# nwihardjo/SpaghettiSearch

Measured on AMD Instinct MI355X. Metric: pagerank_iters_per_sec, higher is better.
Workload: dtype f64

## Files before the change

include/spaghetti_rank.h:

```cpp
#ifndef SPAGHETTI_RANK_H
#define SPAGHETTI_RANK_H

#include <stdint.h>

#ifdef __cplusplus
extern "C" {
#endif

#define SS_ABI_VERSION 4

enum {
    SS_OK = 0,
    SS_ERR_INVALID = 1,
    SS_ERR_NO_DEVICE = 2,
    SS_ERR_HIP = 3,
    SS_ERR_OOM = 4,
    SS_ERR_UNSORTED = 5,
    SS_ERR_STATE = 6,
    SS_ERR_UNSUPPORTED = 7,
    SS_ERR_COMM = 8
};

#define SS_MAX_TOPK 1024
#define SS_MAX_TOPICS 64
#define SS_MAX_QUERY_TERMS 64
#define SS_MAX_CONSTRAINT_TERMS 16
#define SS_UNKNOWN_TERM 0xFFFFFFFFu

typedef struct ss_ctx ss_ctx;
typedef struct ss_graph ss_graph;
typedef struct ss_pr ss_pr;
typedef struct ss_index ss_index;
typedef struct ss_scorer ss_scorer;

typedef struct ss_hit {
    uint32_t doc;
    uint32_t _pad;
    double title;
    double body;
    double pagerank;
    double final;
} ss_hit;

typedef struct ss_graph_info {
    uint64_t n_nodes, n_edges;
    uint64_t n_nondangling;
    uint64_t n_rows_local;
    uint64_t n_edges_local;
    uint32_t max_indeg;
    int32_t rank, world;
} ss_graph_info;

int32_t ss_abi_version(void);
int32_t ss_init(int32_t device_id, ss_ctx** out);
int32_t ss_shutdown(ss_ctx* ctx);
int32_t ss_set_stream(ss_ctx* ctx, void* hip_stream);
int32_t ss_synchronize(ss_ctx* ctx);
#define SS_OPTION_DEFAULT INT64_MIN
int32_t ss_set_option(ss_ctx* ctx, const char* name, int64_t value);
const char* ss_last_error(ss_ctx* ctx);

#define SS_COMM_ID_BYTES 128
int32_t ss_comm_unique_id(void* id_out );
int32_t ss_comm_init(ss_ctx* ctx, const void* id , int32_t rank, int32_t world);
int32_t ss_comm_split(ss_ctx* ctx, int32_t color, int32_t key);
int32_t ss_comm_destroy(ss_ctx* ctx);
int32_t ss_comm_info(ss_ctx* ctx, int32_t* rank_out , int32_t* world_out);
int32_t ss_comm_allreduce_u64(ss_ctx* ctx, uint64_t* buf, uint64_t n);
int32_t ss_comm_allgather(ss_ctx* ctx, const void* send, void* recv, uint64_t bytes_per_rank);

int32_t ss_graph_create(ss_ctx* ctx, uint64_t n_nodes, uint64_t n_edges,
                        const uint64_t* out_ptr , const uint32_t* out_dst ,
                        int32_t rank, int32_t world, ss_graph** out);
int32_t ss_graph_apply_delta(ss_graph* g, uint64_t n_nodes_new, uint64_t n_changed, const uint32_t* changed ,
                             const uint64_t* new_ptr , const uint32_t* new_children);
int32_t ss_graph_get_info(const ss_graph* g, ss_graph_info* info);
int32_t ss_graph_destroy(ss_graph* g);

#define SS_MAX_LINKS      64
#define SS_LINKS_PARENTS  0
#define SS_LINKS_CHILDREN 1
int32_t ss_graph_set_link_key(ss_graph* g, const double* key );
int32_t ss_graph_top_links(ss_graph* g, int32_t dir, uint64_t n, const uint32_t* nodes , int32_t m,
                           uint32_t* links_out , int32_t* n_out , uint32_t* degree_out );
int32_t ss_graph_hit_links(ss_graph* g, int32_t dir, int32_t n_q, int32_t k,
                           const ss_hit* hits , const int32_t* n_hits , int32_t m,
                           uint32_t* links_out , int32_t* n_out ,
                           uint32_t* degree_out );

int32_t ss_pagerank_run(ss_graph* g, double damping, double eps, int32_t max_iter,
                        int32_t k_topics, const int32_t* n_topic,
                        double* rank_out, int32_t* iters_out);

int32_t ss_pr_create(ss_graph* g, double damping, double eps, int32_t max_iter,
                     int32_t k_topics, const int32_t* n_topic, ss_pr** out);
int32_t ss_pr_destroy(ss_pr* pr);
int32_t ss_pr_set_teleport(ss_pr* pr, const uint64_t* set_ptr , const uint32_t* set_nodes);
int32_t ss_pr_begin(ss_pr* pr);
int32_t ss_pr_step(ss_pr* pr, int32_t n_steps);
int32_t ss_pr_finalize(ss_pr* pr);
int32_t ss_pr_exchange_buffers(ss_pr* pr, void** send_dev, uint64_t* send_bytes,
                               void** recv_dev, uint64_t* recv_bytes);
int32_t ss_pr_exchange(ss_pr* pr, int32_t allreduce);
int32_t ss_pagerank_run_sharded(ss_graph* g, double damping, double eps, int32_t max_iter, int32_t k_topics,
                                const int32_t* n_topic, int32_t allreduce, uint32_t* ids_out, double* rank_out, int32_t* iters_out);
int32_t ss_pagerank_run_group(ss_graph* const* shards, int32_t world, double damping, double eps, int32_t max_iter, int32_t k_topics,
                              const int32_t* n_topic, double* rank_out, int32_t* iters_out);
int32_t ss_pr_status(ss_pr* pr, int32_t* iters_out, int32_t* n_active, int32_t* sweeps,
                     double* last_delta_out , double* last_total_out );
int32_t ss_pr_read_local(ss_pr* pr, uint32_t* ids_out, double* rank_out);
int32_t ss_pr_read(ss_pr* pr, double* rank_out);

int32_t ss_pr_probe(ss_pr* pr, int32_t mode, int32_t n_reps, float* ms_out);

int32_t ss_index_create(ss_ctx* ctx, uint64_t n_docs, uint64_t n_terms,
                        const uint64_t* term_ptr , const uint32_t* post_doc,
                        const float* post_tf, ss_index** out);
int32_t ss_index_destroy(ss_index* idx);
int32_t ss_tfidf_build(ss_index* idx, uint64_t total_docs,
                       float* w_out, double* mag_out, float* idf_out);
int32_t ss_index_set_doc_freq(ss_index* idx, const uint64_t* df );
int32_t ss_index_set_weighted(ss_index* idx, const double* mag );
int32_t ss_index_set_positions(ss_index* idx, const uint64_t* pos_ptr, const float* pos);

int32_t ss_index_apply_delta(ss_index* idx, uint64_t n_del_docs, const uint32_t* del_docs,
                             uint64_t n_del, const uint32_t* del_term, const uint32_t* del_doc,
                             uint64_t n_add, const uint32_t* add_term, const uint32_t* add_doc, const float* add_w);
int32_t ss_index_apply_delta_pos(ss_index* idx, uint64_t n_del_docs, const uint32_t* del_docs,
                                 uint64_t n_del, const uint32_t* del_term, const uint32_t* del_doc,
                                 uint64_t n_add, const uint32_t* add_term, const uint32_t* add_doc, const float* add_w,
                                 const uint64_t* add_pos_ptr , const float* add_pos);
int32_t ss_index_resize(ss_index* idx, uint64_t n_docs_new, uint64_t n_terms_new);
int32_t ss_index_read_magnitudes(ss_index* idx, uint64_t n, const uint32_t* docs, double* mag_out);
int32_t ss_index_refresh_magnitudes(ss_index* idx, double* mag_out);
int32_t ss_index_get_info(const ss_index* idx, uint64_t* n_docs, uint64_t* n_terms, uint64_t* n_post);
int32_t ss_index_read(ss_index* idx, uint64_t* term_ptr_out , uint32_t* post_doc_out, float* post_w_out);
int32_t ss_index_read_positions(ss_index* idx, uint64_t* pos_ptr_out, float* pos_out);

int32_t ss_index_build_doc_view(ss_index* idx);
int32_t ss_index_drop_doc_view(ss_index* idx);
int32_t ss_index_read_doc_view(ss_index* idx, uint64_t* doc_ptr_out, uint32_t* doc_term_out, float* doc_w_out);
int32_t ss_index_doc_top_terms(ss_index* idx, uint64_t n, const uint32_t* docs , int32_t m,
                               uint32_t* terms_out , float* w_out , int32_t* n_out );

int32_t ss_scorer_create(ss_ctx* ctx, ss_index* title, ss_index* body, ss_scorer** out);
int32_t ss_scorer_destroy(ss_scorer* s);
int32_t ss_scorer_set_prior(ss_scorer* s, int32_t k_topics, const double* rank);
int32_t ss_score_topk(ss_scorer* s, int32_t n_q, const uint32_t* q_ptr, const uint32_t* q_terms,
                      const int32_t* query_len, const double* topic_probs, int32_t k,
                      ss_hit* hits_out, int32_t* n_hits_out);

#define SS_SCORE_INFLIGHT 3
int32_t ss_score_topk_submit(ss_scorer* s, int32_t n_q, const uint32_t* q_ptr, const uint32_t* q_terms,
                             const uint32_t* p_ptr ,
                             const uint32_t* p_terms, const int32_t* query_len, const double* topic_probs, int32_t k,
                             uint64_t* ticket_out);
int32_t ss_score_topk_collect(ss_scorer* s, uint64_t ticket, ss_hit* hits_out, int32_t* n_hits_out);

#define SS_MAX_PHRASE_TERMS 16
int32_t ss_score_topk_phrase(ss_scorer* s, int32_t n_q, const uint32_t* q_ptr, const uint32_t* q_terms,
                             const uint32_t* p_ptr, const uint32_t* p_terms, const int32_t* query_len,
                             const double* topic_probs, int32_t k, ss_hit* hits_out, int32_t* n_hits_out);

int32_t ss_scorer_set_doc_masks(ss_scorer* s, int32_t n_masks, const uint32_t* words);

int32_t ss_score_topk_masked(ss_scorer* s, int32_t n_q, const uint32_t* q_ptr, const uint32_t* q_terms,
                             const uint32_t* p_ptr, const uint32_t* p_terms, const int32_t* query_len,
                             const double* topic_probs, const int32_t* mask_id, int32_t k,
                             ss_hit* hits_out, int32_t* n_hits_out);

int32_t ss_score_topk_constrained(ss_scorer* s, int32_t n_q, const uint32_t* q_ptr, const uint32_t* q_terms,
                                  const uint32_t* p_ptr, const uint32_t* p_terms, const int32_t* query_len,
                                  const double* topic_probs, const int32_t* mask_id,
                                  const uint32_t* req_ptr , const uint32_t* req_terms,
                                  const uint32_t* exc_ptr , const uint32_t* exc_terms,
                                  int32_t k, ss_hit* hits_out, int32_t* n_hits_out);

int32_t ss_similar_topk(ss_scorer* s, int32_t n_q, const uint32_t* seeds , int32_t m,
                        const double* topic_probs, const int32_t* mask_id , int32_t k,
                        ss_hit* hits_out, int32_t* n_hits_out);

#define SS_MAX_FEEDBACK_DOCS 64
int32_t ss_related_terms(ss_scorer* s, int32_t n_q, const uint32_t* q_ptr, const uint32_t* q_terms,
                         const int32_t* query_len, const double* topic_probs, const int32_t* mask_id ,
                         int32_t k_fb, int32_t m_doc, int32_t m,
                         uint32_t* terms_out , double* score_out , int32_t* n_out );

typedef struct ss_term_match {
    float    title_w;
    float    body_w;
    uint32_t flags;
    float    body_pos;
} ss_term_match;
int32_t ss_explain_hits(ss_scorer* s, int32_t n_q, const uint32_t* q_ptr, const uint32_t* q_terms,
                        int32_t k, const ss_hit* hits , const int32_t* n_hits ,
                        int32_t t_stride, ss_term_match* out );

typedef struct ss_passage {
    float    start;
    float    last;
    uint32_t n_distinct;
    uint32_t n_occ;
    uint64_t token_mask;
} ss_passage;
int32_t ss_best_passages(ss_scorer* s, int32_t n_q, const uint32_t* q_ptr, const uint32_t* q_terms,
                         int32_t k, const ss_hit* hits , const int32_t* n_hits ,
                         int32_t width, ss_passage* out );

#define SS_NO_GROUP 0xFFFFFFFFu
int32_t ss_scorer_set_doc_groups(ss_scorer* s, const uint32_t* group );

int32_t ss_collapse_hits(ss_scorer* s, int32_t n_q, int32_t k_in, const ss_hit* hits ,
                         const int32_t* n_hits , int32_t g, int32_t first, int32_t k,
                         ss_hit* hits_out , int32_t* n_hits_out ,
                         uint32_t* same_out , int32_t* n_kept_out );

int32_t ss_score_topk_collapsed(ss_scorer* s, int32_t n_q, const uint32_t* q_ptr, const uint32_t* q_terms,
                                const int32_t* query_len, const double* topic_probs, const int32_t* mask_id ,
                                int32_t k_window, int32_t g, int32_t first, int32_t k,
                                ss_hit* hits_out , int32_t* n_hits_out ,
                                uint32_t* same_out , int32_t* n_kept_out );

#define SS_MAX_SIG_SLOTS 32
#define SS_SIG_EMPTY 0xFFFFFFFFu
int32_t ss_index_build_signatures(ss_index* idx, int32_t n_slots);
int32_t ss_index_drop_signatures(ss_index* idx);
int32_t ss_index_read_signatures(ss_index* idx, uint64_t n, const uint32_t* docs ,
                                 uint32_t* sig_out , int32_t* n_slots_out );

int32_t ss_dedup_hits(ss_scorer* s, int32_t n_q, int32_t k_in, const ss_hit* hits , const int32_t* n_hits ,
                      int32_t min_match, int32_t first, int32_t k,
                      ss_hit* hits_out , int32_t* n_hits_out ,
                      uint32_t* similar_out , int32_t* n_kept_out );

#define SS_MAX_DOC_FIELDS 4
#define SS_MAX_RANGE_CLAUSES 4
#define SS_NO_FIELD_VALUE INT64_MIN
typedef struct ss_doc_range {
    int32_t field;
    int32_t _pad;
    int64_t lo, hi;
} ss_doc_range;
int32_t ss_scorer_set_doc_fields(ss_scorer* s, int32_t n_fields, const int64_t* values );

int32_t ss_doc_field_masks(ss_scorer* s, int32_t n_sets, const uint32_t* rng_ptr , const ss_doc_range* rng,
                           const int32_t* mask_id ,
                           uint32_t* words_out );

int32_t ss_score_topk_filtered(ss_scorer* s, int32_t n_q, const uint32_t* q_ptr, const uint32_t* q_terms,
                               const uint32_t* p_ptr, const uint32_t* p_terms, const int32_t* query_len,
                               const double* topic_probs, const int32_t* mask_id,
                               const uint32_t* req_ptr , const uint32_t* req_terms,
                               const uint32_t* exc_ptr , const uint32_t* exc_terms,
                               const uint32_t* rng_ptr , const ss_doc_range* rng,
                               int32_t k, ss_hit* hits_out, int32_t* n_hits_out);

int32_t ss_sort_hits_by_field(ss_scorer* s, int32_t n_q, int32_t k_in, const ss_hit* hits ,
                              const int32_t* n_hits , int32_t field, int32_t descending, int32_t first, int32_t k,
                              ss_hit* hits_out , int32_t* n_hits_out , int64_t* values_out );
int32_t ss_hit_fields(ss_scorer* s, int32_t n_q, int32_t k_in, const ss_hit* hits , const int32_t* n_hits ,
                      int64_t* values_out );

#define SS_MAX_VEC_DIM   1024
#define SS_NO_VEC_SCORE  INT32_MIN
typedef struct ss_vec_hit { uint32_t doc; int32_t score; } ss_vec_hit;
int32_t ss_scorer_set_doc_vectors(ss_scorer* s, int32_t dim, const int8_t* vec );

int32_t ss_vector_topk(ss_scorer* s, int32_t n_q, const int8_t* qvec , const int32_t* mask_id ,
                       int32_t k, ss_vec_hit* hits_out , int32_t* n_hits_out );

int32_t ss_hit_vector_scores(ss_scorer* s, int32_t n_q, const int8_t* qvec , int32_t k_in, const ss_hit* hits ,
                             const int32_t* n_hits , int32_t* scores_out );
int32_t ss_rerank_hits_by_vector(ss_scorer* s, int32_t n_q, const int8_t* qvec , int32_t k_in,
                                 const ss_hit* hits , const int32_t* n_hits , int32_t first, int32_t k,
                                 ss_hit* hits_out , int32_t* n_hits_out , int32_t* scores_out );

#define SS_MAX_VEC_LISTS 65536
#define SS_NO_LIST       0xFFFFFFFFu
int32_t ss_scorer_set_vector_lists(ss_scorer* s, int32_t n_lists, const int8_t* centroids ,
                                   const uint32_t* list_of_doc );
int32_t ss_vector_assign_lists(ss_scorer* s, int32_t n_lists, const int8_t* centroids , uint32_t* list_out ,
                               int32_t* score_out );
int32_t ss_vector_topk_probed(ss_scorer* s, int32_t n_q, const int8_t* qvec , const int32_t* mask_id ,
                              int32_t k, int32_t n_probe, ss_vec_hit* hits_out , int32_t* n_hits_out ,
                              uint32_t* probes_out );

int32_t ss_score_docs(ss_scorer* s, int32_t n_q, const uint32_t* q_ptr, const uint32_t* q_terms, const int32_t* query_len,
                      const double* topic_probs, int32_t k_in, const uint32_t* docs , const int32_t* n_in ,
                      ss_hit* hits_out );

#define SS_FUSE_RRF      0
#define SS_FUSE_WEIGHTED 1
typedef struct ss_fuse_params { int32_t mode; int32_t rrf_c; double w_lex; double w_vec; } ss_fuse_params;
typedef struct ss_fused { double score; int32_t vec_score; uint16_t lex_rank; uint16_t vec_rank; } ss_fused;
int32_t ss_fuse_hits(ss_scorer* s, int32_t n_q, const uint32_t* q_ptr, const uint32_t* q_terms, const int32_t* query_len,
                     const double* topic_probs, const int8_t* qvec ,
                     int32_t k_lex, const ss_hit* lex , const int32_t* n_lex ,
                     int32_t k_vec, const ss_vec_hit* vec , const int32_t* n_vec ,
                     const ss_fuse_params* fp, int32_t first, int32_t k,
                     ss_hit* hits_out , int32_t* n_hits_out ,
                     ss_fused* fused_out , int32_t* n_union_out );
int32_t ss_hybrid_topk(ss_scorer* s, int32_t n_q, const uint32_t* q_ptr, const uint32_t* q_terms, const int32_t* query_len,
                       const double* topic_probs, const int8_t* qvec , const int32_t* mask_id ,
                       int32_t k_window, const ss_fuse_params* fp, int32_t first, int32_t k,
                       ss_hit* hits_out , int32_t* n_hits_out ,
                       ss_fused* fused_out , int32_t* n_union_out );

#define SS_MAX_WORD_BYTES 64
#define SS_MAX_EDIT_DIST  3
#define SS_MAX_SUGGEST    64
typedef struct ss_lexicon ss_lexicon;

int32_t ss_lexicon_create(ss_ctx* ctx, uint64_t n_terms, const uint64_t* word_ptr , const uint8_t* bytes,
                          const uint32_t* freq , ss_lexicon** out);
int32_t ss_lexicon_set_freq(ss_lexicon* lx, const uint32_t* freq );
int32_t ss_lexicon_get_info(const ss_lexicon* lx, uint64_t* n_terms, uint64_t* n_bytes);
int32_t ss_lexicon_read_order(ss_lexicon* lx, uint32_t* order_out );
int32_t ss_lexicon_destroy(ss_lexicon* lx);

int32_t ss_lexicon_prefix(ss_lexicon* lx, int32_t n_q, const uint32_t* p_ptr , const uint8_t* p_bytes,
                          int64_t first, int32_t k, uint32_t* terms_out , int32_t* n_out ,
                          uint64_t* n_match_out );

int32_t ss_lexicon_suggest(ss_lexicon* lx, int32_t n_q, const uint32_t* w_ptr , const uint8_t* w_bytes,
                           int32_t max_dist, uint32_t min_freq, int32_t m,
                           uint32_t* terms_out , int32_t* dist_out , int32_t* n_out );

#define SS_MAX_SHARDS 64
int32_t ss_merge_hits(ss_ctx* ctx, int32_t n_q, int32_t n_parts, int32_t k, const ss_hit* parts,
                      const int32_t* n_hits, const uint32_t* doc_base, ss_hit* hits_out, int32_t* n_hits_out);

int32_t ss_last_kernel_ms(ss_ctx* ctx, int32_t kind, float* ms_out);

#ifdef __cplusplus
}
#endif
#endif
```

spaghettisearch_amd/_lib.py:

```python
from __future__ import annotations

import ctypes as C
import os

_HERE = os.path.dirname(os.path.abspath(__file__))
LIB_PATH = os.environ.get("SS_LIB_PATH") or os.path.join(_HERE, "libspaghetti_rank.so")

SS_OK = 0
SS_MAX_TOPK = 1024
SS_MAX_TOPICS = 64
SS_MAX_QUERY_TERMS = 64
SS_MAX_FEEDBACK_DOCS = 64
SS_UNKNOWN_TERM = 0xFFFFFFFF
SS_NO_GROUP = 0xFFFFFFFF
SS_MAX_WORD_BYTES = 64
SS_MAX_EDIT_DIST = 3
SS_MAX_SUGGEST = 64
SS_MAX_SIG_SLOTS = 32
SS_SIG_EMPTY = 0xFFFFFFFF
SS_MAX_LINKS = 64
SS_LINKS_PARENTS = 0
SS_LINKS_CHILDREN = 1
SS_MAX_DOC_FIELDS = 4
SS_MAX_RANGE_CLAUSES = 4
SS_NO_FIELD_VALUE = -(2 ** 63)
SS_MAX_VEC_DIM = 1024
SS_NO_VEC_SCORE = -(2 ** 31)
SS_MAX_VEC_LISTS = 65536
SS_NO_LIST = 0xFFFFFFFF
SS_FUSE_RRF = 0
SS_FUSE_WEIGHTED = 1

ERR_NAMES = {0: "SS_OK", 1: "SS_ERR_INVALID", 2: "SS_ERR_NO_DEVICE", 3: "SS_ERR_HIP", 4: "SS_ERR_OOM",
             5: "SS_ERR_UNSORTED", 6: "SS_ERR_STATE", 7: "SS_ERR_UNSUPPORTED", 8: "SS_ERR_COMM"}
SS_COMM_ID_BYTES = 128


class SpaghettiError(RuntimeError):
    def __init__(self, code: int, msg: str):
        super().__init__(f"{ERR_NAMES.get(code, code)}: {msg}")
        self.code = code


class SsHit(C.Structure):
    _fields_ = [("doc", C.c_uint32), ("_pad", C.c_uint32), ("title", C.c_double), ("body", C.c_double),
                ("pagerank", C.c_double), ("final", C.c_double)]


class SsTermMatch(C.Structure):
    _fields_ = [("title_w", C.c_float), ("body_w", C.c_float), ("flags", C.c_uint32), ("body_pos", C.c_float)]


class SsPassage(C.Structure):
    _fields_ = [("start", C.c_float), ("last", C.c_float), ("n_distinct", C.c_uint32), ("n_occ", C.c_uint32), ("token_mask", C.c_uint64)]


class SsDocRange(C.Structure):
    _fields_ = [("field", C.c_int32), ("_pad", C.c_int32), ("lo", C.c_int64), ("hi", C.c_int64)]


class SsVecHit(C.Structure):
    _fields_ = [("doc", C.c_uint32), ("score", C.c_int32)]


class SsFuseParams(C.Structure):
    _fields_ = [("mode", C.c_int32), ("rrf_c", C.c_int32), ("w_lex", C.c_double), ("w_vec", C.c_double)]


class SsFused(C.Structure):
    _fields_ = [("score", C.c_double), ("vec_score", C.c_int32), ("lex_rank", C.c_uint16), ("vec_rank", C.c_uint16)]


class SsGraphInfo(C.Structure):
    _fields_ = [("n_nodes", C.c_uint64), ("n_edges", C.c_uint64), ("n_nondangling", C.c_uint64),
                ("n_rows_local", C.c_uint64), ("n_edges_local", C.c_uint64), ("max_indeg", C.c_uint32),
                ("rank", C.c_int32), ("world", C.c_int32)]


_vp = C.c_void_p
_i32 = C.c_int32
_u64 = C.c_uint64
_f64 = C.c_double

PROTOTYPES = {
    "ss_abi_version": (_i32, []),
    "ss_init": (_i32, [_i32, C.POINTER(_vp)]),
    "ss_shutdown": (_i32, [_vp]),
    "ss_set_stream": (_i32, [_vp, _vp]),
    "ss_synchronize": (_i32, [_vp]),
    "ss_set_option": (_i32, [_vp, C.c_char_p, C.c_int64]),
    "ss_last_error": (C.c_char_p, [_vp]),
    "ss_comm_unique_id": (_i32, [_vp]),
    "ss_comm_init": (_i32, [_vp, _vp, _i32, _i32]),
    "ss_comm_split": (_i32, [_vp, _i32, _i32]),
    "ss_comm_destroy": (_i32, [_vp]),
    "ss_comm_info": (_i32, [_vp, C.POINTER(_i32), C.POINTER(_i32)]),
    "ss_comm_allreduce_u64": (_i32, [_vp, _vp, _u64]),
    "ss_comm_allgather": (_i32, [_vp, _vp, _vp, _u64]),
    "ss_graph_create": (_i32, [_vp, _u64, _u64, _vp, _vp, _i32, _i32, C.POINTER(_vp)]),
    "ss_graph_apply_delta": (_i32, [_vp, _u64, _u64, _vp, _vp, _vp]),
    "ss_graph_get_info": (_i32, [_vp, C.POINTER(SsGraphInfo)]),
    "ss_graph_destroy": (_i32, [_vp]),
    "ss_graph_set_link_key": (_i32, [_vp, _vp]),
    "ss_graph_top_links": (_i32, [_vp, _i32, _u64, _vp, _i32, _vp, _vp, _vp]),
    "ss_graph_hit_links": (_i32, [_vp, _i32, _i32, _i32, _vp, _vp, _i32, _vp, _vp, _vp]),
    "ss_pagerank_run": (_i32, [_vp, _f64, _f64, _i32, _i32, _vp, _vp, _vp]),
    "ss_pr_create": (_i32, [_vp, _f64, _f64, _i32, _i32, _vp, C.POINTER(_vp)]),
    "ss_pr_destroy": (_i32, [_vp]),
    "ss_pr_set_teleport": (_i32, [_vp, _vp, _vp]),
    "ss_pr_begin": (_i32, [_vp]),
    "ss_pr_step": (_i32, [_vp, _i32]),
    "ss_pr_finalize": (_i32, [_vp]),
    "ss_pr_exchange_buffers": (_i32, [_vp, C.POINTER(_vp), C.POINTER(_u64), C.POINTER(_vp), C.POINTER(_u64)]),
    "ss_pr_exchange": (_i32, [_vp, _i32]),
    "ss_pagerank_run_sharded": (_i32, [_vp, _f64, _f64, _i32, _i32, _vp, _i32, _vp, _vp, _vp]),
    "ss_pagerank_run_group": (_i32, [_vp, _i32, _f64, _f64, _i32, _i32, _vp, _vp, _vp]),
    "ss_pr_status": (_i32, [_vp, _vp, C.POINTER(_i32), C.POINTER(_i32), _vp, _vp]),
    "ss_pr_read_local": (_i32, [_vp, _vp, _vp]),
    "ss_pr_read": (_i32, [_vp, _vp]),
    "ss_pr_probe": (_i32, [_vp, _i32, _i32, C.POINTER(C.c_float)]),
    "ss_index_create": (_i32, [_vp, _u64, _u64, _vp, _vp, _vp, C.POINTER(_vp)]),
    "ss_index_destroy": (_i32, [_vp]),
    "ss_tfidf_build": (_i32, [_vp, _u64, _vp, _vp, _vp]),
    "ss_index_apply_delta": (_i32, [_vp, _u64, _vp, _u64, _vp, _vp, _u64, _vp, _vp, _vp]),
    "ss_index_apply_delta_pos": (_i32, [_vp, _u64, _vp, _u64, _vp, _vp, _u64, _vp, _vp, _vp, _vp, _vp]),
    "ss_index_resize": (_i32, [_vp, _u64, _u64]),
    "ss_index_read_magnitudes": (_i32, [_vp, _u64, _vp, _vp]),
    "ss_index_refresh_magnitudes": (_i32, [_vp, _vp]),
    "ss_index_get_info": (_i32, [_vp, C.POINTER(_u64), C.POINTER(_u64), C.POINTER(_u64)]),
    "ss_index_read": (_i32, [_vp, _vp, _vp, _vp]),
    "ss_index_read_positions": (_i32, [_vp, _vp, _vp]),
    "ss_index_set_doc_freq": (_i32, [_vp, _vp]),
    "ss_index_set_weighted": (_i32, [_vp, _vp]),
    "ss_index_set_positions": (_i32, [_vp, _vp, _vp]),
    "ss_index_build_doc_view": (_i32, [_vp]),
    "ss_index_drop_doc_view": (_i32, [_vp]),
    "ss_index_read_doc_view": (_i32, [_vp, _vp, _vp, _vp]),
    "ss_index_doc_top_terms": (_i32, [_vp, _u64, _vp, _i32, _vp, _vp, _vp]),
    "ss_scorer_create": (_i32, [_vp, _vp, _vp, C.POINTER(_vp)]),
    "ss_scorer_destroy": (_i32, [_vp]),
    "ss_scorer_set_prior": (_i32, [_vp, _i32, _vp]),
    "ss_score_topk": (_i32, [_vp, _i32, _vp, _vp, _vp, _vp, _i32, _vp, _vp]),
    "ss_score_topk_phrase": (_i32, [_vp, _i32, _vp, _vp, _vp, _vp, _vp, _vp, _i32, _vp, _vp]),
    "ss_score_topk_submit": (_i32, [_vp, _i32, _vp, _vp, _vp, _vp, _vp, _vp, _i32, _vp]),
    "ss_score_topk_collect": (_i32, [_vp, C.c_uint64, _vp, _vp]),
    "ss_scorer_set_doc_masks": (_i32, [_vp, _i32, _vp]),
    "ss_score_topk_masked": (_i32, [_vp, _i32, _vp, _vp, _vp, _vp, _vp, _vp, _vp, _i32, _vp, _vp]),
    "ss_score_topk_constrained": (_i32, [_vp, _i32, _vp, _vp, _vp, _vp, _vp, _vp, _vp, _vp, _vp, _vp, _vp, _i32, _vp, _vp]),
    "ss_similar_topk": (_i32, [_vp, _i32, _vp, _i32, _vp, _vp, _i32, _vp, _vp]),
    "ss_related_terms": (_i32, [_vp, _i32, _vp, _vp, _vp, _vp, _vp, _i32, _i32, _i32, _vp, _vp, _vp]),
    "ss_explain_hits": (_i32, [_vp, _i32, _vp, _vp, _i32, _vp, _vp, _i32, _vp]),
    "ss_best_passages": (_i32, [_vp, _i32, _vp, _vp, _i32, _vp, _vp, _i32, _vp]),
    "ss_scorer_set_doc_groups": (_i32, [_vp, _vp]),
    "ss_collapse_hits": (_i32, [_vp, _i32, _i32, _vp, _vp, _i32, _i32, _i32, _vp, _vp, _vp, _vp]),
    "ss_score_topk_collapsed": (_i32, [_vp, _i32, _vp, _vp, _vp, _vp, _vp, _i32, _i32, _i32, _i32, _vp, _vp, _vp, _vp]),
    "ss_index_build_signatures": (_i32, [_vp, _i32]),
    "ss_index_drop_signatures": (_i32, [_vp]),
    "ss_index_read_signatures": (_i32, [_vp, _u64, _vp, _vp, C.POINTER(_i32)]),
    "ss_dedup_hits": (_i32, [_vp, _i32, _i32, _vp, _vp, _i32, _i32, _i32, _vp, _vp, _vp, _vp]),
    "ss_scorer_set_doc_fields": (_i32, [_vp, _i32, _vp]),
    "ss_doc_field_masks": (_i32, [_vp, _i32, _vp, _vp, _vp, _vp]),
    "ss_score_topk_filtered": (_i32, [_vp, _i32, _vp, _vp, _vp, _vp, _vp, _vp, _vp, _vp, _vp, _vp, _vp, _vp, _vp, _i32, _vp, _vp]),
    "ss_sort_hits_by_field": (_i32, [_vp, _i32, _i32, _vp, _vp, _i32, _i32, _i32, _i32, _vp, _vp, _vp]),
    "ss_hit_fields": (_i32, [_vp, _i32, _i32, _vp, _vp, _vp]),
    "ss_scorer_set_doc_vectors": (_i32, [_vp, _i32, _vp]),
    "ss_vector_topk": (_i32, [_vp, _i32, _vp, _vp, _i32, _vp, _vp]),
    "ss_hit_vector_scores": (_i32, [_vp, _i32, _vp, _i32, _vp, _vp, _vp]),
    "ss_rerank_hits_by_vector": (_i32, [_vp, _i32, _vp, _i32, _vp, _vp, _i32, _i32, _vp, _vp, _vp]),
    "ss_scorer_set_vector_lists": (_i32, [_vp, _i32, _vp, _vp]),
    "ss_vector_assign_lists": (_i32, [_vp, _i32, _vp, _vp, _vp]),
    "ss_vector_topk_probed": (_i32, [_vp, _i32, _vp, _vp, _i32, _i32, _vp, _vp, _vp]),
    "ss_score_docs": (_i32, [_vp, _i32, _vp, _vp, _vp, _vp, _i32, _vp, _vp, _vp]),
    "ss_fuse_hits": (_i32, [_vp, _i32, _vp, _vp, _vp, _vp, _vp, _i32, _vp, _vp, _i32, _vp, _vp, _vp, _i32, _i32, _vp, _vp, _vp, _vp]),
    "ss_hybrid_topk": (_i32, [_vp, _i32, _vp, _vp, _vp, _vp, _vp, _vp, _i32, _vp, _i32, _i32, _vp, _vp, _vp, _vp]),
    "ss_lexicon_create": (_i32, [_vp, _u64, _vp, _vp, _vp, C.POINTER(_vp)]),
    "ss_lexicon_set_freq": (_i32, [_vp, _vp]),
    "ss_lexicon_get_info": (_i32, [_vp, C.POINTER(_u64), C.POINTER(_u64)]),
    "ss_lexicon_read_order": (_i32, [_vp, _vp]),
    "ss_lexicon_destroy": (_i32, [_vp]),
    "ss_lexicon_prefix": (_i32, [_vp, _i32, _vp, _vp, C.c_int64, _i32, _vp, _vp, _vp]),
    "ss_lexicon_suggest": (_i32, [_vp, _i32, _vp, _vp, _i32, C.c_uint32, _i32, _vp, _vp, _vp]),
    "ss_merge_hits": (_i32, [_vp, _i32, _i32, _i32, _vp, _vp, _vp, _vp, _vp]),
    "ss_last_kernel_ms": (_i32, [_vp, _i32, C.POINTER(C.c_float)]),
}

ABI_VERSION = 4
_lib = None


def load() -> C.CDLL:
    global _lib
    if _lib is not None:
        return _lib
    if not os.path.exists(LIB_PATH):
        raise ImportError(
            f"{LIB_PATH} not found: build it with `python -c 'import __graft_entry__ as g; g.build()'` "
            "(make -C spaghettisearch_amd/csrc). There is no CPU fallback.")
    try:
        import torch
    except ImportError:
        pass
    lib = C.CDLL(LIB_PATH)
    for name, (res, args) in PROTOTYPES.items():
        fn = getattr(lib, name)
        fn.restype = res
        fn.argtypes = args
    if lib.ss_abi_version() != ABI_VERSION:
        raise ImportError(f"{LIB_PATH}: ABI version {lib.ss_abi_version()}, this binding was written for {ABI_VERSION} "
                          "(include/spaghetti_rank.h: SS_ABI_VERSION) - rebuild the library")
    _lib = lib
    return lib


def check(rc: int, ctx=None) -> None:
    if rc != SS_OK:
        msg = load().ss_last_error(ctx)
        raise SpaghettiError(rc, msg.decode("utf-8", "replace") if msg else "")
```

spaghettisearch_amd/csrc/ctx.hip:

```cpp
#include "common.hpp"
#include <chrono>

#include <unordered_map>

namespace ss {

namespace {
struct Pool {
    std::mutex mu;
    std::multimap<std::pair<int, size_t>, void*> free_blocks;
    std::unordered_map<void*, std::pair<int, size_t>> live;
    size_t held = 0, limit = (size_t)64 << 30;
    double miss_ms = 0.0;
    uint64_t misses = 0;
    int contexts = 0;
};
Pool& pool() { static Pool* p = new Pool(); return *p; }
size_t size_class(size_t b) {
    if (b <= 4096) return 4096;
    size_t p2 = 4096;
    while (p2 < b) p2 <<= 1;
    if (p2 <= ((size_t)1 << 20)) return p2;
    const size_t step = p2 >> 4;
    return (b + step - 1) / step * step;
}
}

hipError_t pool_alloc(void** out, size_t bytes) {
    Pool& P = pool();
    const size_t cls = size_class(bytes);
    int dev = 0;
    (void)hipGetDevice(&dev);
    {
        std::lock_guard<std::mutex> lk(P.mu);
        auto it = P.free_blocks.find({dev, cls});
        if (it != P.free_blocks.end()) {
            *out = it->second;
            P.free_blocks.erase(it);
            P.held -= cls;
            P.live[*out] = {dev, cls};
            return hipSuccess;
        }
    }
    const auto tm0 = std::chrono::steady_clock::now();
    hipError_t e = hipMalloc(out, cls);
    {
        std::lock_guard<std::mutex> lk(P.mu);
        P.miss_ms += std::chrono::duration<double, std::milli>(std::chrono::steady_clock::now() - tm0).count();
        P.misses++;
    }
    if (e != hipSuccess) {
        (void)hipGetLastError();
        pool_trim();
        e = hipMalloc(out, cls);
    }
    if (e == hipSuccess) {
        std::lock_guard<std::mutex> lk(P.mu);
        P.live[*out] = {dev, cls};
    }
    return e;
}

static thread_local bool t_device_idle = false;

void pool_free_batch(void* const* blocks, size_t count) {
    if (!count) return;
    {
        int cur = 0;
        (void)hipGetDevice(&cur);
        if (device_wedged(cur)) return;
    }
    (void)hipDeviceSynchronize();
    t_device_idle = true;
    for (size_t i = 0; i < count; i++) pool_free(blocks[i]);
    t_device_idle = false;
}

void pool_free(void* p) {
    if (!p) return;
    Pool& P = pool();
    size_t cls = 0, limit = 0;
    int dev = 0;
    {
        std::lock_guard<std::mutex> lk(P.mu);
        auto it = P.live.find(p);
        if (it != P.live.end()) { dev = it->second.first; cls = it->second.second; P.live.erase(it); }
        limit = P.limit;
    }
    if (device_wedged(dev)) return;
    if (cls && cls <= limit / 2) {
        int cur = 0;
        (void)hipGetDevice(&cur);
        if (cur != dev || !t_device_idle) {
            if (cur != dev) (void)hipSetDevice(dev);
            (void)hipDeviceSynchronize();
            if (cur != dev) (void)hipSetDevice(cur);
        }
        std::vector<void*> evict;
        {
            std::lock_guard<std::mutex> lk(P.mu);
            while (P.held + cls > P.limit && !P.free_blocks.empty()) {
                auto last = std::prev(P.free_blocks.end());
                if (last->first.second <= cls) break;
                evict.push_back(last->second);
                P.held -= last->first.second;
                P.free_blocks.erase(last);
            }
            if (P.held + cls <= P.limit) {
                P.free_blocks.emplace(std::make_pair(dev, cls), p);
                P.held += cls;
                p = nullptr;
            }
        }
        for (void* q : evict) (void)hipFree(q);
        if (!p) return;
    }
    (void)hipFree(p);
}

void pool_stats(uint64_t* misses, double* miss_ms) {
    std::lock_guard<std::mutex> lk(pool().mu);
    *misses = pool().misses;
    *miss_ms = pool().miss_ms;
}
void pool_context_count(int delta) {
    bool last = false;
    {
        std::lock_guard<std::mutex> lk(pool().mu);
        pool().contexts += delta;
        last = delta < 0 && pool().contexts <= 0;
    }
    if (last) pool_trim();
}

void pool_trim() {
    Pool& P = pool();
    std::multimap<std::pair<int, size_t>, void*> take;
    {
        std::lock_guard<std::mutex> lk(P.mu);
        take.swap(P.free_blocks);
        P.held = 0;
    }
    for (auto& kv : take) (void)hipFree(kv.second);
}

void pool_set_limit(size_t bytes) {
    {
        std::lock_guard<std::mutex> lk(pool().mu);
        pool().limit = bytes;
    }
    pool_trim();
}

static std::mutex g_err_mu;
static std::string g_err;
void set_global_error(const std::string& msg) {
    std::lock_guard<std::mutex> lk(g_err_mu);
    g_err = msg;
}
}

extern "C" {

int32_t ss_abi_version(void) { return SS_ABI_VERSION; }

int32_t ss_init(int32_t device_id, ss_ctx** out) {
    if (!out) {
        ss::set_global_error("ss_init: out is NULL");
        return SS_ERR_INVALID;
    }
    *out = nullptr;
    int n_dev = 0;
    hipError_t e = hipGetDeviceCount(&n_dev);
    if (e != hipSuccess || n_dev <= 0) {
        ss::set_global_error(std::string("ss_init: no HIP device (") + hipGetErrorString(e) + ")");
        return SS_ERR_NO_DEVICE;
    }
    if (device_id < 0 || device_id >= n_dev) {
        ss::set_global_error("ss_init: device_id out of range");
        return SS_ERR_INVALID;
    }
    ss_ctx* ctx = new (std::nothrow) ss_ctx();
    if (!ctx) return SS_ERR_OOM;
    ctx->device = device_id;
    if ((e = hipSetDevice(device_id)) != hipSuccess) {
        ss::set_global_error(std::string("ss_init: hipSetDevice: ") + hipGetErrorString(e));
        delete ctx;
        return SS_ERR_NO_DEVICE;
    }
    hipDeviceProp_t prop;
    if ((e = hipGetDeviceProperties(&prop, device_id)) != hipSuccess) {
        ss::set_global_error(std::string("ss_init: hipGetDeviceProperties: ") + hipGetErrorString(e));
        delete ctx;
        return SS_ERR_NO_DEVICE;
    }
    if (std::strncmp(prop.gcnArchName, "gfx950", 6) != 0) {
        ss::set_global_error(std::string("ss_init: device is ") + prop.gcnArchName +
                             ", this library is built for gfx950 (MI355X) only");
        delete ctx;
        return SS_ERR_NO_DEVICE;
    }
    ctx->cu_count = prop.multiProcessorCount;
    ctx->total_mem = prop.totalGlobalMem;
    if ((e = hipStreamCreateWithFlags(&ctx->own_stream, hipStreamNonBlocking)) != hipSuccess) {
        ss::set_global_error(std::string("ss_init: hipStreamCreate: ") + hipGetErrorString(e));
        delete ctx;
        return SS_ERR_HIP;
    }
    ctx->stream = ctx->own_stream;
    int prio_lo = 0, prio_hi = 0;
    (void)hipDeviceGetStreamPriorityRange(&prio_lo, &prio_hi);
    if ((e = hipStreamCreateWithPriority(&ctx->comm_stream, hipStreamNonBlocking, prio_hi)) != hipSuccess) {
        ss::set_global_error(std::string("ss_init: hipStreamCreate (comm): ") + hipGetErrorString(e));
        (void)hipStreamDestroy(ctx->own_stream);
        delete ctx;
        return SS_ERR_HIP;
    }
    for (int k = 0; k < 3; k++)
        for (int j = 0; j < 2; j++)
            if ((e = hipEventCreate(&ctx->ev[k][j])) != hipSuccess) {
                ss::set_global_error(std::string("ss_init: hipEventCreate: ") + hipGetErrorString(e));
                delete ctx;
                return SS_ERR_HIP;
            }
    if ((e = hipHostMalloc(reinterpret_cast<void**>(&ctx->h_pin), ss_ctx::PIN_SCRATCH, hipHostMallocDefault)) != hipSuccess) {
        ss::set_global_error(std::string("ss_init: hipHostMalloc: ") + hipGetErrorString(e));
        delete ctx;
        return SS_ERR_HIP;
    }
    ss::pool_context_count(+1);
    *out = ctx;
    return SS_OK;
}

int32_t ss_shutdown(ss_ctx* ctx) {
    if (!ctx) return SS_ERR_INVALID;
    (void)hipSetDevice(ctx->device);
    const bool stuck = !ss::try_unwedge(ctx);
    (void)ss_comm_destroy(ctx);
    if (!stuck) (void)hipStreamSynchronize(ctx->stream);
    for (int k = 0; k < 3; k++)
        for (int j = 0; j < 2; j++)
            if (ctx->ev[k][j]) (void)hipEventDestroy(ctx->ev[k][j]);
    if (ctx->comm_stream && !stuck) { (void)hipStreamSynchronize(ctx->comm_stream); (void)hipStreamDestroy(ctx->comm_stream); }
    for (hipStream_t ws : ctx->wave_stream)
        if (ws && !stuck) { (void)hipStreamSynchronize(ws); (void)hipStreamDestroy(ws); }
    if (ctx->own_stream && !stuck) (void)hipStreamDestroy(ctx->own_stream);
    if (ctx->h_pin) (void)hipHostFree(ctx->h_pin);
    for (auto& b : ctx->pin_cache) (void)hipHostFree(b.p);
    delete ctx;
    ss::pool_context_count(-1);
    return SS_OK;
}

int32_t ss_set_stream(ss_ctx* ctx, void* hip_stream) {
    if (!ctx) return SS_ERR_INVALID;
    std::lock_guard<std::recursive_mutex> lk(ctx->mu);
    SS_HIP(ctx, hipStreamSynchronize(ctx->stream));
    ctx->stream = hip_stream ? reinterpret_cast<hipStream_t>(hip_stream) : ctx->own_stream;
    return SS_OK;
}

static const char* const k_option_names[] = {
    "comm.timeout_ms",
    "pr.force_narrow",
    "pr.wire_f32",
    "pr.narrow_wave",
    "pr.t_quad",
    "pr.blocks_per_cu",
    "mem.pool_mb",
    "pr.deal_snake",
    "pr.affine_lag",
    "pr.affine",
    "pr.items_per_wave",
    "pr.persistent",
    "pr.persistent_blocks",
    "pr.n_class_order",
    "pr.class_order",
    "pr.stagger",
    "pr.deal_global",
    "pr.share_zero_rows",
    "pr.item_turns",
    "graph.late_free",
    "graph.readback_runs",
    "pr.trace",
    "score.collect_pinned",
    "score.pipeline_slices",
    "score.timing",
    "score.trace",
    "pr.probe_hot",
    "pr.topic_blocks",
    "tfidf.blocks",
    "tfidf.bucket_shift",
    "tfidf.head_min_run",
    "tfidf.bucket_min",
    "score.wave",
    "score.wave_max_terms",
    "score.wave_min_list",
    "score.wave_share_pct",
    "score.wave_slice_target",
    "score.wave_big_pct",
    "score.wave_big_x100",
    "score.small",
    "score.small_max_batch",
    "score.small_batch",
    "score.small_cap",
    "score.pipeline",
    "score.grade_slices",
    "score.wave_small_x100",
    "score.exact_all",
    "score.slice_target",
    "score.separate_merge",
    "passage.lds_events",
    "lexicon.chunk_terms",
    "links.wave_max",
    "links.chunk_edges",
    "vec.chunk_docs",
    "vec.list_seg_rows",
    "vec.list_batch_q",
    "vec.assign_batch",
};

int32_t ss_set_option(ss_ctx* ctx, const char* name, int64_t value) {
    if (!ctx || !name) return SS_ERR_INVALID;
    std::lock_guard<std::recursive_mutex> lk(ctx->mu);
    for (const char* n : k_option_names)
        if (std::strcmp(n, name) == 0) {
            if (value == SS_OPTION_DEFAULT) ctx->options.erase(name);
            else ctx->options[name] = value;
            if (std::strcmp(name, "mem.pool_mb") == 0) ss::pool_set_limit(value == SS_OPTION_DEFAULT ? (size_t)64 << 30 : (size_t)std::max<int64_t>(0, value) << 20);
            return SS_OK;
        }
    return ctx->fail(SS_ERR_INVALID, "ss_set_option: unknown option '%s'", name);
}

int32_t ss_synchronize(ss_ctx* ctx) {
    if (!ctx) return SS_ERR_INVALID;
    std::lock_guard<std::recursive_mutex> lk(ctx->mu);
    SS_HIP(ctx, hipSetDevice(ctx->device));
    SS_TRY(ss::sync_bounded(ctx, ctx->stream, "ss_synchronize"));
    return SS_OK;
}

const char* ss_last_error(ss_ctx* ctx) {
    if (ctx) return ctx->last_error.c_str();
    static thread_local std::string tl;
    {
        std::lock_guard<std::mutex> lk(ss::g_err_mu);
        tl = ss::g_err;
    }
    return tl.c_str();
}

int32_t ss_last_kernel_ms(ss_ctx* ctx, int32_t kind, float* ms_out) {
    if (!ctx || !ms_out || kind < 0 || kind > 2) return SS_ERR_INVALID;
    std::lock_guard<std::recursive_mutex> lk(ctx->mu);
    if (!ctx->ev_valid[kind]) return ctx->fail(SS_ERR_STATE, "ss_last_kernel_ms: no timed call of kind %d yet", kind);
    SS_HIP(ctx, hipEventSynchronize(ctx->ev[kind][1]));
    SS_HIP(ctx, hipEventElapsedTime(ms_out, ctx->ev[kind][0], ctx->ev[kind][1]));
    return SS_OK;
}

}
```

spaghettisearch_amd/csrc/pagerank.hip:

```cpp
#include "pr_device.hpp"

#include <algorithm>
#include <chrono>
#include <cmath>
#include <memory>

namespace {

__global__ void k_pr_item_ranges(WorkItem* __restrict__ work, uint32_t n_items, const uint32_t* __restrict__ in_ptr) {
    const uint32_t i = blockIdx.x * blockDim.x + threadIdx.x;
    if (i >= n_items) return;
    WorkItem w = work[i];
    switch (w.kind) {
        case V_ROWW: w.beg = in_ptr[w.row]; w.end = in_ptr[w.row + 1]; break;
        case V_SEG:
            w.beg = in_ptr[w.row] + w.count * SEGW;
            w.end = min(in_ptr[w.row + 1], w.beg + SEGW);
            break;
        case V_QUAD:
        case V_DEG: w.beg = in_ptr[w.row]; w.end = in_ptr[w.row + w.count]; break;
        default: return;
    }
    work[i] = w;
}

__global__ __launch_bounds__(TPB) void k_pr_remap_src(const uint32_t* __restrict__ in_src, uint32_t* __restrict__ out, size_t n_edges, uint32_t pos_nd,
                                                      uint32_t cnt_nd, const uint32_t* __restrict__ outdeg, const uint32_t* __restrict__ sh_deg,
                                                      uint32_t n_shared, uint32_t zrow) {
    for (size_t e = (size_t)blockIdx.x * TPB + threadIdx.x; e < n_edges; e += (size_t)gridDim.x * TPB) {
        uint32_t w = NT_LOAD(&in_src[e]);
        const uint32_t s = w & SRC_MASK;
        if (s >= pos_nd) {
            uint32_t row = zrow;
            if (s < cnt_nd && n_shared) {
                const uint32_t od = outdeg[s];
                uint32_t lo = 0, hi = n_shared;
                while (lo < hi) {
                    const uint32_t mid = (lo + hi) >> 1;
                    if (sh_deg[mid] < od) lo = mid + 1; else hi = mid;
                }
                if (lo < n_shared && sh_deg[lo] == od) row = zrow + 1 + lo;
            }
            w = (w & ~SRC_MASK) | row;
        }
        NT_STORE(w, &out[e]);
    }
}

template <int GW>
__global__ __launch_bounds__(TPB) void k_pr_begin(PrParams p) {
    const int lane = threadIdx.x & 63;
    const int t = lane % GW;
    const double x0 = p.x0[t];
    double* __restrict__ Tw = p.tab_wr[1];
    double csum = 0.0;
    for (uint32_t i = blockIdx.x * TPB + threadIdx.x; i < p.n_shared * (uint32_t)GW; i += gridDim.x * TPB)
        Tw[(size_t)(p.zrow + 1) * GW + i] = p.d * x0 / (double)p.sh_deg[i / GW];
    const size_t n_el = ((size_t)p.sl_nd + p.sl_d) * GW;
    for (size_t i = (size_t)blockIdx.x * TPB + threadIdx.x; i < n_el; i += (size_t)gridDim.x * TPB) {
        const uint32_t lrow = (uint32_t)(i / GW);
        const bool real = lrow < p.sl_nd ? lrow < p.cnt_nd : (lrow - p.sl_nd) < p.cnt_d;
        p.x[i] = real ? x0 : 0.0;
        if (lrow < p.sl_nd) {
            double c = 0.0;
            if (real) c = p.d * x0 / (double)p.outdeg[lrow];
            if ((p.world == 1 || lrow + 2 < p.sl_nd) && lrow < p.tab_rows) Tw[i] = c;
            csum += c;
        }
    }
    block_reduce_and_publish<GW>(p, 0.0, csum, Tw, true);
}

template <int GW>
__global__ void k_pr_finalize(PrParams p, const double* __restrict__ table, int is_begin) {
    if (threadIdx.x != 0 || blockIdx.x != 0) return;
    if (!is_begin && p.ctl->n_active == 0) return;
    double dl[MAXK], cs[MAXK];
    for (int k = 0; k < MAXK; k++) { dl[k] = 0.0; cs[k] = 0.0; }
    for (int r = 0; r < p.world; r++) {
        const size_t base = ((size_t)r * p.sl_nd + (p.sl_nd - 2)) * GW;
        for (int k = 0; k < GW; k++) {
            cs[k] += table[base + k];
            dl[k] += table[base + GW + k];
        }
    }
    finalize_ctl(p, dl, cs, is_begin != 0);
}

template <int GW>
__global__ void k_pr_read(const double* __restrict__ x, const PrCtl* __restrict__ ctl, const uint32_t* __restrict__ old_id,
                          uint32_t sl_nd, uint32_t cnt_nd, uint32_t pos_nd, uint32_t sl_d, uint32_t cnt_d, uint32_t pos_d,
                          uint64_t id0_nd, uint64_t id0_d, int k_topics, uint64_t out_stride,
                          int by_original_id, uint32_t* __restrict__ ids_out, double* __restrict__ out,
                          const uint32_t* __restrict__ memb, uint32_t ts_mask) {
    const size_t n_rows = (size_t)cnt_nd + cnt_d;
    size_t i = (size_t)blockIdx.x * blockDim.x + threadIdx.x;
    if (i >= n_rows) return;
    const uint32_t lrow = i < cnt_nd ? (uint32_t)i : sl_nd + (uint32_t)(i - cnt_nd);
    const uint64_t iid = lrow < sl_nd ? id0_nd + lrow : id0_d + (lrow - sl_nd);
    const uint32_t orig = old_id[iid];
    const size_t o = by_original_id ? (size_t)orig : i;
    if (ids_out) ids_out[i] = orig;
    const bool zero = lrow < sl_nd ? lrow >= pos_nd : (lrow - sl_nd) >= pos_d;
    const uint32_t mb = memb ? memb[lrow] & ts_mask : 0u;
    for (int k = 0; k < k_topics; k++)
        out[(size_t)k * out_stride + o] = zero ? (((mb >> k) & 1u) ? ctl->xz_in[k] : ctl->xz[k]) : x[(size_t)lrow * GW + k];
}

__global__ void k_pr_memb(const uint64_t* __restrict__ set_ptr, const uint32_t* __restrict__ set_nodes, int k_topics, uint64_t n_nodes,
                          const uint32_t* __restrict__ new_id, uint64_t nd_int, uint32_t sl_nd, uint32_t sl_d, int rank,
                          uint32_t* __restrict__ memb, uint32_t* __restrict__ seen, uint32_t* __restrict__ err) {
    const uint64_t total = set_ptr[k_topics];
    for (uint64_t i = (uint64_t)blockIdx.x * blockDim.x + threadIdx.x; i < total; i += (uint64_t)gridDim.x * blockDim.x) {
        int k = 0;
        while (k + 1 < k_topics && set_ptr[k + 1] <= i) k++;
        const uint32_t v = set_nodes[i];
        if ((uint64_t)v >= n_nodes) { atomicOr(err, 1u); continue; }
        if (atomicOr(&seen[v], 1u << k) & (1u << k)) { atomicOr(err, 2u); continue; }
        const uint64_t iid = new_id[v];
        uint32_t lrow;
        int owner;
        if (iid < nd_int) { owner = (int)(iid / sl_nd); lrow = (uint32_t)(iid % sl_nd); }
        else { owner = (int)((iid - nd_int) / sl_d); lrow = sl_nd + (uint32_t)((iid - nd_int) % sl_d); }
        if (owner == rank) atomicOr(&memb[lrow], 1u << k);
    }
}
__global__ void k_pr_memb_zero_count(const uint32_t* __restrict__ memb, uint32_t sl_nd, uint32_t cnt_nd, uint32_t pos_nd, uint32_t cnt_d,
                                     uint32_t pos_d, int k_topics, unsigned long long* __restrict__ cnt) {
    const uint32_t z_nd = cnt_nd - pos_nd, n_zero = z_nd + (cnt_d - pos_d);
    for (uint32_t i = blockIdx.x * blockDim.x + threadIdx.x; i < n_zero; i += gridDim.x * blockDim.x) {
        const uint32_t lrow = i < z_nd ? pos_nd + i : sl_nd + pos_d + (i - z_nd);
        const uint32_t mb = memb[lrow];
        for (int k = 0; k < k_topics; k++)
            if ((mb >> k) & 1u) atomicAdd(&cnt[k], 1ull);
    }
}

template <int GW, int POL>
__global__ __launch_bounds__(TPB) void k_pr_probe(const double* __restrict__ T, const uint32_t* __restrict__ in_src, size_t n_edges,
                                                  uint32_t n_rows, int mode, double* __restrict__ sink, uint32_t hot) {
    if constexpr (GW >= 8) {
        constexpr int NSLOT = 64 / GW;
        const int lane = threadIdx.x & 63, wave = threadIdx.x >> 6;
        const int t = lane % GW, slot = lane / GW, gbase = lane - t;
        const size_t groups = (size_t)gridDim.x * WAVES * NSLOT;
        const size_t gi = ((size_t)blockIdx.x * WAVES + wave) * NSLOT + slot;
        const size_t n_chunks = n_edges / CH;
        const size_t per = (n_chunks + groups - 1) / groups;
        size_t c = min(gi * per, n_chunks);
        const size_t c_hi = min(c + per, n_chunks);
        double acc = 0.0;
        for (; c < c_hi; c++) {
            constexpr int R = CH / GW;
            uint32_t src[R];
#pragma unroll
            for (int r = 0; r < R; r++) {
                const size_t e = c * CH + (size_t)(r * GW + t);
                uint32_t v = NT_LOAD(&in_src[e]) & SRC_MASK;
                if (mode == 1) v = (uint32_t)(((uint64_t)(v * 2654435761u + (uint32_t)e * 40503u) * n_rows) >> 32);
                if (mode == 2) v = (uint32_t)(e % n_rows);
                src[r] = v;
            }
            double v[CH];
#pragma unroll
            for (int j = 0; j < CH; j++) {
                const uint32_t sj = (uint32_t)__shfl((int)src[j / GW], gbase + (j % GW), 64);
                const double* a = &T[(size_t)sj * GW + t];
                if constexpr (POL == 0) v[j] = *a;
                else if constexpr (POL == 1) v[j] = __builtin_nontemporal_load(a);
                else if constexpr (POL == 2) v[j] = __hip_atomic_load(a, __ATOMIC_RELAXED, __HIP_MEMORY_SCOPE_AGENT);
                else if constexpr (POL == 3) v[j] = sj < hot ? *a : __builtin_nontemporal_load(a);
                else v[j] = sj < hot ? *a : __hip_atomic_load(a, __ATOMIC_RELAXED, __HIP_MEMORY_SCOPE_AGENT);
            }
#pragma unroll
            for (int j = 0; j < CH; j++) acc += v[j];
        }
        sink[((size_t)blockIdx.x * TPB + threadIdx.x)] = acc;
    }
}

}

namespace {

void pick_kernel(const ss_ctx* ctx, ss_pr* pr, int k, uint64_t table_rows) {
    const bool force_narrow = ctx->opt("pr.force_narrow", 0) != 0, narrow_wave = ctx->opt("pr.narrow_wave", 1) != 0;
    if (k > 2) {
        pr->kernel = PR_SWEEP;
        pr->gw = k <= 8 ? 8 : 16;
    } else if (force_narrow) {
        pr->kernel = PR_STEP;
        pr->gw = k;
    } else if (narrow_wave) {
        pr->kernel = PR_SWEEP_N;
        pr->gw = k;
    } else if (table_rows * 64 <= (64ull << 20)) {
        pr->kernel = PR_SWEEP;
        pr->gw = 8;
    } else {
        pr->kernel = PR_STEP;
        pr->gw = k;
    }
    pr->nwave = pr->kernel == PR_SWEEP_N;
    const int64_t want = ctx->opt("pr.persistent", 0);
    pr->persist_mode = want == 2 ? 2 : 1;
    pr->persist = pr->nwave && pr->g->world == 1 && !ctx->opt("pr.affine", 0) && want > 0;
}

template <int GW>
void launch_begin(ss_pr* pr, hipStream_t st, unsigned nb) {
    hipLaunchKernelGGL(k_pr_begin<GW>, dim3(nb), dim3(TPB), 0, st, pr->prm);
}
template <int GW>
void launch_finalize(ss_pr* pr, hipStream_t st, int is_begin) {
    hipLaunchKernelGGL(k_pr_finalize<GW>, dim3(1), dim3(64), 0, st, pr->prm, (const double*)pr->tab0.p, is_begin);
}
template <int GW>
__global__ __launch_bounds__(TPB) void k_pr_read_orig(const double* __restrict__ x, const PrCtl* __restrict__ ctl, const uint32_t* __restrict__ new_id,
                                                      uint64_t n, uint32_t sl_nd, uint32_t pos_nd, uint32_t pos_d, int k_topics,
                                                      double* __restrict__ out, const uint32_t* __restrict__ memb, uint32_t ts_mask) {
    const uint64_t v = (uint64_t)blockIdx.x * blockDim.x + threadIdx.x;
    if (v >= n) return;
    const uint32_t lrow = new_id[v];
    const bool zero = lrow < sl_nd ? lrow >= pos_nd : (lrow - sl_nd) >= pos_d;
    double r[GW];
    if (!zero) {
        if constexpr (GW >= 2) {
            const double2* const row = reinterpret_cast<const double2*>(x + (size_t)lrow * GW);
#pragma unroll
            for (int j = 0; j < GW / 2; j++) { const double2 t = row[j]; r[2 * j] = t.x; r[2 * j + 1] = t.y; }
        } else {
            r[0] = x[lrow];
        }
    } else {
        const uint32_t mb = memb ? memb[lrow] & ts_mask : 0u;
#pragma unroll
        for (int k = 0; k < GW; k++) r[k] = ((mb >> k) & 1u) ? ctl->xz_in[k] : ctl->xz[k];
    }
#pragma unroll
    for (int k = 0; k < GW; k++)
        if (k < k_topics) out[(size_t)k * n + v] = r[k];
}

template <int GW>
void launch_read(ss_pr* pr, hipStream_t st, int by_orig, uint64_t stride, uint32_t* ids, double* out) {
    const ss_graph* g = pr->g;
    const size_t n_rows = (size_t)g->cnt_nd + g->cnt_d;
    if (!n_rows) return;
    if (by_orig && g->world == 1 && !ids && stride == g->n) {
        hipLaunchKernelGGL(k_pr_read_orig<GW>, dim3(ss::div_up(g->n, TPB)), dim3(TPB), 0, st, (const double*)pr->x.p, (const PrCtl*)pr->ctl.p,
                           (const uint32_t*)g->new_id.p, g->n, g->sl_nd, pr->prm.pos_nd, pr->prm.pos_d, pr->k, out, pr->prm.memb, pr->prm.ts_mask);
        return;
    }
    hipLaunchKernelGGL(k_pr_read<GW>, dim3(ss::div_up(n_rows, TPB)), dim3(TPB), 0, st, (const double*)pr->x.p,
                       (const PrCtl*)pr->ctl.p, (const uint32_t*)g->old_id.p, g->sl_nd, g->cnt_nd, pr->prm.pos_nd, g->sl_d, g->cnt_d,
                       pr->prm.pos_d,
                       (uint64_t)g->rank * g->sl_nd, g->nd_int + (uint64_t)g->rank * g->sl_d, pr->k, stride, by_orig, ids, out,
                       pr->prm.memb, pr->prm.ts_mask);
}

#define SS_GW_DISPATCH(gw, fn, ...)          \
    switch (gw) {                            \
        case 1: fn<1>(__VA_ARGS__); break;   \
        case 2: fn<2>(__VA_ARGS__); break;   \
        case 8: fn<8>(__VA_ARGS__); break;   \
        default: fn<16>(__VA_ARGS__); break; \
    }

}

namespace ss {
unsigned begin_blocks(const ss_pr* pr) { return std::max(1u, std::min(2048u, ss::div_up((size_t)pr->g->n_local() * pr->gw, TPB))); }
void pr_launch_begin(ss_pr* pr, hipStream_t st, unsigned nb) { SS_GW_DISPATCH(pr->gw, launch_begin, pr, st, nb); }
void pr_launch_step(ss_pr* pr, hipStream_t st) {
    switch (pr->kernel) {
        case PR_STEP: pr_step_launch(pr, st); break;
        case PR_SWEEP: pr_sweep_launch(pr, st); break;
        case PR_SWEEP_N: pr_sweep_n_launch(pr, st); break;
    }
}
void pr_launch_finalize(ss_pr* pr, hipStream_t st, int is_begin) { SS_GW_DISPATCH(pr->gw, launch_finalize, pr, st, is_begin); }
}

namespace {

PlanOptions plan_options(const ss_ctx* ctx, const ss_pr* pr, size_t n_local) {
    const bool small = n_local <= ((size_t)4 << 20);
    PlanOptions o;
    o.t_quad = (uint32_t)ctx->opt("pr.t_quad", pr->nwave ? 256 : 128);
    o.item_turns = (uint32_t)std::max<int64_t>(1, std::min<int64_t>(64, ctx->opt("pr.item_turns", pr->nwave ? (small ? 1 : 4) : (small ? 4 : 8))));
    o.items_per_wave = pr->nwave ? (size_t)std::max<int64_t>(1, ctx->opt("pr.items_per_wave", 4)) : 1;
    o.deal_snake = ctx->opt("pr.deal_snake", PlanOptions::AUTO);
    o.deal_global = ctx->opt("pr.deal_global", pr->nwave && pr->gw == 1 ? 1 : 2);
    o.blocks_per_cu = ctx->opt("pr.blocks_per_cu", PlanOptions::AUTO);
    o.class_order = ctx->opt("pr.class_order", 235401);
    o.n_class_order = ctx->opt("pr.n_class_order", small ? 2310 : 123);
    o.stagger = ctx->opt("pr.stagger", 0);
    return o;
}

constexpr int OCC_MULTI_N = 3;
int blocks_per_cu(int row, int gw) {
    static std::mutex occ_mu;
    static int occ_cache[4][MAXK + 1] = {};
    std::lock_guard<std::mutex> lk_occ(occ_mu);
    int& occ = occ_cache[row][gw];
    if (!occ) {
        int per_cu = 0;
        switch (row) {
            case PR_STEP: per_cu = ss::pr_step_occupancy(gw); break;
            case PR_SWEEP: per_cu = ss::pr_sweep_occupancy(gw); break;
            case PR_SWEEP_N: per_cu = ss::pr_sweep_n_occupancy(gw); break;
            default: per_cu = ss::pr_multi_n_occupancy(gw); break;
        }
        occ = std::max(per_cu, 1);
    }
    return occ;
}
unsigned grid_for(const ss_ctx* ctx, const ss_pr* pr, const PlanOptions& opt, int per_cu, size_t n_items) {
    per_cu = (int)std::max<int64_t>(1, opt.blocks_per_cu == PlanOptions::AUTO ? per_cu : opt.blocks_per_cu);
    if (pr->persist) {
        const int admit = std::max(1, blocks_per_cu(OCC_MULTI_N, pr->gw) - 2);
        per_cu = (int)std::max<int64_t>(1, std::min<int64_t>(std::min(admit, std::max(1, per_cu / 2)), ctx->opt("pr.persistent_blocks", 4)));
    }
    return pr->kernel != PR_STEP ? (unsigned)std::min<size_t>(std::max<size_t>(1, ss::div_up(n_items, (size_t)WAVES * opt.items_per_wave)), (size_t)ctx->cu_count * per_cu)
                                 : (unsigned)std::min<size_t>(n_items, (size_t)ctx->cu_count * 8);
}

void fill_params(ss_pr* pr, const Cut& cut, const PlanOptions& opt, double damping, double eps, int32_t max_iter, int32_t k_topics) {
    const ss_graph* g = pr->g;
    PrParams& p = pr->prm;
    p.in_ptr = g->in_ptr.p;
    p.in_src = g->in_src.p;
    p.outdeg = g->outdeg.p;
    p.x = pr->x.p;
    if (g->world == 1) {
        p.tab_rd[0] = pr->tab0.p; p.tab_wr[0] = pr->tab1.p;
        p.tab_rd[1] = pr->tab1.p; p.tab_wr[1] = pr->tab0.p;
    } else {
        p.tab_rd[0] = p.tab_rd[1] = pr->tab0.p;
        p.tab_wr[0] = p.tab_wr[1] = pr->send.p;
    }
    p.work = pr->work.p;
    p.partials = pr->partials.p;
    p.segpart = pr->segpart.p;
    p.rowticket = pr->rowticket.p;
    p.hubsum = pr->hubsum.p;
    p.nmulti = cut.nmulti;
    p.ctl = pr->ctl.p;
    p.x0 = pr->x0.p;
    p.d = damping;
    p.teleport = 1.0 - damping;
    p.eps = eps;
    p.tele_n = p.teleport * (double)g->n;
    p.max_iter = max_iter;
    p.k_topics = k_topics;
    p.world = g->world;
    p.sl_nd = g->sl_nd;
    p.cnt_nd = g->cnt_nd;
    p.sl_d = g->sl_d;
    p.cnt_d = g->cnt_d;
    p.seg_edges = cut.seg_edges;
    p.n_items = (uint32_t)cut.items.size();
    p.pos_nd = cut.pos_nd;
    p.pos_d = cut.pos_d;
    p.zrow = (uint32_t)g->nd_int;
    p.tab_rows = g->sl_nd;
    p.woff = pr->woff.p;
    p.stagger_div = opt.stagger != 0 ? (uint32_t)std::max(g->ctx->cu_count, 1) : 0u;
    p.stagger_code = opt.stagger >= 10 ? (uint32_t)(opt.stagger - 10) : 0u;
    p.class_order = pack_class_order(opt.class_order);
    p.n_order = pack_n_order(opt.n_class_order);
}

uint64_t fnv1a(const void* q, size_t n, uint64_t h = 0xcbf29ce484222325ull) {
    const unsigned char* b = static_cast<const unsigned char*>(q);
    for (size_t i = 0; i < n; i++) { h ^= b[i]; h *= 0x100000001b3ull; }
    return h;
}
void trace_plan(const ss_pr* pr, const std::vector<WorkItem>& work, const std::vector<uint32_t>& woff) {
    const PrParams& p = pr->prm;
    const double sd[] = {p.d, p.teleport, p.eps, p.tele_n};
    const uint32_t su[] = {(uint32_t)p.max_iter, (uint32_t)p.k_topics, (uint32_t)p.world, p.sl_nd, p.cnt_nd, p.sl_d, p.cnt_d, p.seg_edges, p.n_items,
                           p.pos_nd, p.pos_d, p.ts_mask, p.zrow, p.stagger_div, p.stagger_code, p.class_order, p.n_order};
    fprintf(stderr, "[pr trace] plan: work %016llx (%zu items)  woff %016llx  params %016llx  nblocks %u\n",
            (unsigned long long)fnv1a(work.data(), work.size() * sizeof(WorkItem)), work.size(),
            (unsigned long long)fnv1a(woff.data(), woff.size() * sizeof(uint32_t)),
            (unsigned long long)fnv1a(su, sizeof(su), fnv1a(sd, sizeof(sd))), pr->nblocks);
}

int32_t alloc_tables(ss_pr* pr, hipStream_t st, size_t rows) {
    const ss_graph* g = pr->g;
    ss_ctx* ctx = g->ctx;
    const size_t GW = (size_t)pr->gw;
    SS_HIP(ctx, pr->tab0.alloc(rows * GW));
    SS_HIP(ctx, hipMemsetAsync(pr->tab0.p, 0, std::max<size_t>(pr->tab0.bytes(), 8), st));
    if (g->world == 1) {
        SS_HIP(ctx, pr->tab1.alloc(rows * GW));
        SS_HIP(ctx, hipMemsetAsync(pr->tab1.p, 0, std::max<size_t>(pr->tab1.bytes(), 8), st));
    } else {
        SS_HIP(ctx, pr->send.alloc((size_t)g->sl_nd * GW));
        SS_HIP(ctx, hipMemsetAsync(pr->send.p, 0, std::max<size_t>(pr->send.bytes(), 8), st));
    }
    return SS_OK;
}
int32_t unshare_rows(ss_pr* pr, hipStream_t st) {
    if (!pr->prm.share) return SS_OK;
    const ss_graph* g = pr->g;
    SS_HIP(g->ctx, hipStreamSynchronize(st));
    SS_TRY(alloc_tables(pr, st, (size_t)g->nd_int + 1));
    pr->src_shared.release();
    pr->sh_deg.release();
    PrParams& p = pr->prm;
    p.tab_rd[0] = pr->tab0.p; p.tab_wr[0] = pr->tab1.p;
    p.tab_rd[1] = pr->tab1.p; p.tab_wr[1] = pr->tab0.p;
    p.in_src = g->in_src.p;
    p.sh_deg = nullptr;
    p.n_shared = 0;
    p.share = 0;
    p.zrow = (uint32_t)g->nd_int;
    p.tab_rows = g->sl_nd;
    return SS_OK;
}

#ifdef SS_PR_WAVETIME
void dump_wave_loads(const Cut& cut, const std::vector<double>& cost, const std::vector<uint32_t>& owner, uint32_t nw) {
    FILE* f = open_dump("pr_load.csv");
    if (!f) return;
    std::vector<double> wl(nw, 0.0), wcls((size_t)nw * 6, 0.0);
    for (size_t i = 0; i < cut.items.size(); i++) {
        int kc = 0; while (kc < 5 && i >= cut.vbeg[kc + 1]) kc++;
        wl[owner[i]] += cost[i]; wcls[(size_t)owner[i] * 6 + kc] += cost[i];
    }
    fprintf(f, "wave,load,c0,c1,c2,c3,c4,c5\n");
    for (uint32_t w = 0; w < nw; w++) fprintf(f, "%u,%.2f,%.2f,%.2f,%.2f,%.2f,%.2f,%.2f\n", w, wl[w], wcls[(size_t)w * 6], wcls[(size_t)w * 6 + 1], wcls[(size_t)w * 6 + 2], wcls[(size_t)w * 6 + 3], wcls[(size_t)w * 6 + 4], wcls[(size_t)w * 6 + 5]);
    fclose(f);
}
#endif

}

extern "C" {

int32_t ss_pr_create(ss_graph* g, double damping, double eps, int32_t max_iter, int32_t k_topics,
                     const int32_t* n_topic, ss_pr** out) {
    if (!g) return SS_ERR_INVALID;
    ss_ctx* ctx = g->ctx;
    std::lock_guard<std::recursive_mutex> lk(ctx->mu);
    if (!out) return ctx->fail(SS_ERR_INVALID, "ss_pr_create: out is NULL");
    *out = nullptr;
    if (k_topics < 1 || !n_topic) return ctx->fail(SS_ERR_INVALID, "ss_pr_create: k_topics < 1 or n_topic NULL");
    if (k_topics > MAXK) return ctx->fail(SS_ERR_UNSUPPORTED, "ss_pr_create: k_topics %d > %d per state (ss_pagerank_run splits larger K)", k_topics, MAXK);
    SS_HIP(ctx, hipSetDevice(ctx->device));
    hipStream_t st = ctx->stream;

    ss_pr* pr = new (std::nothrow) ss_pr();
    if (!pr) return ctx->fail(SS_ERR_OOM, "ss_pr_create: host OOM");
    std::unique_ptr<ss_pr> guard(pr);
    pr->g = g;
    pr->k = k_topics;
    pick_kernel(ctx, pr, k_topics, g->nd_int);
    const int GW = pr->gw;
    const bool vitems = pr->kernel != PR_STEP;
    const int GI = pr->nwave ? 8 : GW;
    const size_t n_local = g->n_local();
    if (((uint64_t)g->nd_int + 1) * GW * 8 >= (1ull << 32))
        return ctx->fail(SS_ERR_UNSUPPORTED, "ss_pr_create: contribution table of %llu rows x %d topics exceeds 4 GiB (shard the graph over more ranks)",
                         (unsigned long long)g->nd_int, GW);

    const bool trace = ctx->opt("pr.trace", 0) != 0;
    auto t_now = [] { return std::chrono::steady_clock::now(); };
    auto t_ms = [](std::chrono::steady_clock::time_point a, std::chrono::steady_clock::time_point b) { return std::chrono::duration<double, std::milli>(b - a).count(); };
    SS_HIP(ctx, pr->x.alloc(n_local * GW));
    bool share = GW >= 8 && g->world == 1 && ctx->opt("pr.affine", 0) == 0 && ctx->opt("pr.share_zero_rows", 1) != 0;
    if (!share) SS_TRY(alloc_tables(pr, st, (size_t)g->nd_int + 1));

    const auto tc0 = t_now();
    const PlanOptions opt = plan_options(ctx, pr, n_local);
    Cut cut = cut_items(g->h_indeg_nd, g->h_indeg_d, g->sl_nd, GI, pr->nwave, opt);
    const uint32_t n_tail = g->cnt_nd - cut.pos_nd;
    struct PinGuard { ss_ctx* c; void* p = nullptr; size_t cap = 0; ~PinGuard() { c->pin_free(p, cap); } } tail_od{ctx};
    if (share && n_tail == 0) {
        share = false;
        SS_TRY(alloc_tables(pr, st, (size_t)g->nd_int + 1));
    }
    if (share) {
        tail_od.p = ctx->pin_alloc((size_t)n_tail * sizeof(uint32_t), &tail_od.cap);
        if (!tail_od.p) return ctx->fail(SS_ERR_OOM, "ss_pr_create: no pinned host memory for %u out-degrees", n_tail);
        SS_HIP(ctx, hipMemcpyAsync(tail_od.p, g->outdeg.p + cut.pos_nd, (size_t)n_tail * sizeof(uint32_t), hipMemcpyDeviceToHost, st));
    }
    const auto tc1 = t_now();
    const int per_cu = blocks_per_cu(pr->kernel, GW);
    const auto tc1a = t_now();
    pr->nblocks = grid_for(ctx, pr, opt, per_cu, cut.items.size());
    static const std::vector<uint32_t> no_woff;
    const std::vector<uint32_t>* woff = &no_woff;
    if (vitems) {
        const uint32_t nw = pr->nblocks * WAVES;
        const auto td0 = t_now();
        const std::vector<double>& cost = item_costs(cut, g->h_indeg_nd, g->h_indeg_d, g->sl_nd, GI, pr->nwave);
        const auto td0a = t_now();
        std::vector<uint32_t>& owner = deal_items(cut, cost, nw, pr->nwave, opt);
#ifdef SS_PR_WAVETIME
        dump_wave_loads(cut, cost, owner, nw);
#endif
        const auto td1 = t_now();
        if (trace) fprintf(stderr, "[pr trace]   deal: occupancy query %.2f ms, costs %.3f ms, owners %.3f ms\n", t_ms(tc1, tc1a), t_ms(td0, td0a), t_ms(td0a, td1));
        woff = &place_items(cut, owner, nw);
        if (trace) fprintf(stderr, "[pr trace]   deal: placement %.3f ms\n", t_ms(td1, t_now()));
    }
    const std::vector<WorkItem>& items = cut.items;

    g->settle();
    const auto tc2 = t_now();
    SharedRows sh;
    if (share) {
        SS_HIP(ctx, hipStreamSynchronize(st));
        const auto ts0 = t_now();
        sh = plan_shared_rows(static_cast<const uint32_t*>(tail_od.p), n_tail, cut.pos_nd);
        const auto ts1 = t_now();
        SS_TRY(alloc_tables(pr, st, (size_t)sh.table_rows));
        SS_HIP(ctx, pr->sh_deg.alloc(sh.deg.size()));
        SS_HIP(ctx, hipMemcpyAsync(pr->sh_deg.p, sh.deg.data(), sh.deg.size() * sizeof(uint32_t), hipMemcpyHostToDevice, st));
        SS_HIP(ctx, pr->src_shared.alloc(g->e_local));
        if (g->e_local)
            hipLaunchKernelGGL(k_pr_remap_src, dim3((unsigned)std::min<uint64_t>(ss::div_up(g->e_local, TPB), (uint64_t)ctx->cu_count * 16)), dim3(TPB), 0, st,
                               (const uint32_t*)g->in_src.p, pr->src_shared.p, (size_t)g->e_local, cut.pos_nd, g->cnt_nd, (const uint32_t*)g->outdeg.p,
                               (const uint32_t*)pr->sh_deg.p, (uint32_t)sh.deg.size(), sh.zrow);
        if (trace) fprintf(stderr, "[pr trace]   shared rows: %u rows without in-edges -> %zu shared rows (host %.3f ms), table %llu rows\n", n_tail, sh.deg.size(),
                           t_ms(ts0, ts1), (unsigned long long)sh.table_rows);
    }
    SS_HIP(ctx, pr->partials.alloc(((size_t)std::max(pr->nblocks, ss::begin_blocks(pr)) + 8) * 2 * GW));
    SS_HIP(ctx, pr->segpart.alloc((size_t)std::max(cut.nsegs, 1u) * GW));
    SS_HIP(ctx, pr->rowticket.alloc(std::max(cut.nmulti, 1u)));
    SS_HIP(ctx, pr->hubsum.alloc((size_t)std::max(cut.nmulti, 1u) * 2 * GW));
    SS_HIP(ctx, hipMemsetAsync(pr->hubsum.p, 0, pr->hubsum.bytes(), st));
    SS_HIP(ctx, hipMemsetAsync(pr->rowticket.p, 0, pr->rowticket.bytes(), st));
    SS_HIP(ctx, pr->woff.alloc(std::max<size_t>(woff->size(), 8)));
    if (!woff->empty()) SS_HIP(ctx, hipMemcpyAsync(pr->woff.p, woff->data(), woff->size() * sizeof(uint32_t), hipMemcpyHostToDevice, st));
    SS_HIP(ctx, pr->work.alloc(items.size()));
    SS_HIP(ctx, hipMemcpyAsync(pr->work.p, items.data(), items.size() * sizeof(WorkItem), hipMemcpyHostToDevice, st));
    if (vitems)
        hipLaunchKernelGGL(k_pr_item_ranges, dim3(ss::div_up(items.size(), TPB)), dim3(TPB), 0, st, pr->work.p, (uint32_t)items.size(), (const uint32_t*)g->in_ptr.p);
    SS_HIP(ctx, pr->ctl.alloc(1));
    SS_HIP(ctx, hipMemsetAsync(pr->ctl.p, 0, sizeof(PrCtl), st));
    double h_x0[MAXK];
    for (int k = 0; k < MAXK; k++) h_x0[k] = k < k_topics ? 1.0 / (double)n_topic[k] : 0.0;
    SS_HIP(ctx, pr->x0.alloc(MAXK));
    SS_HIP(ctx, hipMemcpyAsync(pr->x0.p, h_x0, sizeof(h_x0), hipMemcpyHostToDevice, st));
    SS_HIP(ctx, hipStreamSynchronize(st));
    if (trace) fprintf(stderr, "[pr trace] ss_pr_create: build_work %.2f ms (%zu items), edge ranges + deal %.2f ms, alloc + upload %.2f ms\n", t_ms(tc0, tc1), items.size(), t_ms(tc1, tc2), t_ms(tc2, t_now()));
    if (trace) fprintf(stderr, "[pr trace] where the state lives: x %p  tab0 %p  tab1 %p  in_src %p  in_ptr %p  outdeg %p  work %p  woff %p\n", (void*)pr->x.p, (void*)pr->tab0.p,
                       (void*)pr->tab1.p, (void*)g->in_src.p, (void*)g->in_ptr.p, (void*)g->outdeg.p, (void*)pr->work.p, (void*)pr->woff.p);

    fill_params(pr, cut, opt, damping, eps, max_iter, k_topics);
    if (share) {
        PrParams& p = pr->prm;
        p.in_src = pr->src_shared.p;
        p.sh_deg = pr->sh_deg.p;
        p.n_shared = (uint32_t)sh.deg.size();
        p.share = 1;
        p.zrow = sh.zrow;
        p.tab_rows = cut.pos_nd;
    }
    if (trace) trace_plan(pr, items, *woff);
    g->users++;
    *out = guard.release();
    return SS_OK;
}

int32_t ss_pr_set_teleport(ss_pr* pr, const uint64_t* set_ptr, const uint32_t* set_nodes) {
    if (!pr) return SS_ERR_INVALID;
    ss_ctx* ctx = pr->g->ctx;
    std::lock_guard<std::recursive_mutex> lk(ctx->mu);
    SS_HIP(ctx, hipSetDevice(ctx->device));
    if (pr->begun) return ctx->fail(SS_ERR_STATE, "ss_pr_set_teleport: call before ss_pr_begin");
    hipStream_t st = ctx->stream;
    PrParams& p = pr->prm;
    if (!set_ptr) {
        p.memb = nullptr; p.tin = nullptr; p.nz_in = nullptr; p.ts_mask = 0;
        return SS_OK;
    }
    const ss_graph* g = pr->g;
    const int K = pr->k;
    SS_TRY(unshare_rows(pr, st));
    std::vector<uint64_t> h_ptr(K + 1);
    SS_HIP(ctx, ss::copy_in(ctx->stream, h_ptr.data(), set_ptr, (K + 1) * sizeof(uint64_t)));
    if (h_ptr[0] != 0) return ctx->fail(SS_ERR_INVALID, "ss_pr_set_teleport: set_ptr[0] != 0");
    for (int k = 0; k < K; k++)
        if (h_ptr[k + 1] < h_ptr[k]) return ctx->fail(SS_ERR_INVALID, "ss_pr_set_teleport: set_ptr not non-decreasing");
    const uint64_t total = h_ptr[K];
    if (total && !set_nodes) return ctx->fail(SS_ERR_INVALID, "ss_pr_set_teleport: set_nodes is NULL");
    double h_tin[MAXK];
    uint32_t mask = 0;
    for (int k = 0; k < MAXK; k++) {
        h_tin[k] = 0.0;
        if (k < K && h_ptr[k + 1] > h_ptr[k]) {
            mask |= 1u << k;
            h_tin[k] = p.teleport * (double)g->n / (double)(h_ptr[k + 1] - h_ptr[k]);
        }
    }
    const size_t n_local = g->n_local();
    ss::DevBuf<uint64_t> d_ptr;
    ss::DevBuf<uint32_t> d_nodes, d_err, d_seen;
    ss::DevBuf<unsigned long long> d_cnt;
    SS_HIP(ctx, d_ptr.alloc(K + 1));
    SS_HIP(ctx, d_seen.alloc(g->n));
    SS_HIP(ctx, hipMemsetAsync(d_seen.p, 0, std::max<size_t>(d_seen.bytes(), 4), st));
    SS_HIP(ctx, d_nodes.alloc(total));
    SS_HIP(ctx, d_err.alloc(1));
    SS_HIP(ctx, d_cnt.alloc(MAXK));
    SS_HIP(ctx, pr->memb.alloc(n_local));
    SS_HIP(ctx, pr->tin.alloc(MAXK));
    SS_HIP(ctx, pr->nz_in.alloc(MAXK));
    SS_HIP(ctx, hipMemcpyAsync(d_ptr.p, h_ptr.data(), (K + 1) * sizeof(uint64_t), hipMemcpyHostToDevice, st));
    if (total) SS_HIP(ctx, hipMemcpyAsync(d_nodes.p, set_nodes, total * sizeof(uint32_t), hipMemcpyDefault, st));
    SS_HIP(ctx, hipMemsetAsync(pr->memb.p, 0, std::max<size_t>(pr->memb.bytes(), 4), st));
    SS_HIP(ctx, hipMemsetAsync(d_err.p, 0, sizeof(uint32_t), st));
    SS_HIP(ctx, hipMemsetAsync(d_cnt.p, 0, MAXK * sizeof(unsigned long long), st));
    if (total)
        hipLaunchKernelGGL(k_pr_memb, dim3(std::min<unsigned>(ss::div_up(total, TPB), 4096u)), dim3(TPB), 0, st, (const uint64_t*)d_ptr.p,
                           (const uint32_t*)d_nodes.p, K, g->n, (const uint32_t*)g->new_id.p, g->nd_int, std::max(g->sl_nd, 1u), std::max(g->sl_d, 1u),
                           g->rank, pr->memb.p, d_seen.p, d_err.p);
    const uint32_t n_zero = (g->cnt_nd - p.pos_nd) + (g->cnt_d - p.pos_d);
    if (n_zero)
        hipLaunchKernelGGL(k_pr_memb_zero_count, dim3(std::min<unsigned>(ss::div_up(n_zero, TPB), 4096u)), dim3(TPB), 0, st,
                           (const uint32_t*)pr->memb.p, g->sl_nd, g->cnt_nd, p.pos_nd, g->cnt_d, p.pos_d, K, d_cnt.p);
    SS_HIP(ctx, hipGetLastError());
    uint32_t h_err = 0;
    unsigned long long h_cnt[MAXK];
    SS_HIP(ctx, ss::fetch(ctx, st, &h_err, d_err.p, sizeof(h_err), h_cnt, d_cnt.p, sizeof(h_cnt)));
    if (h_err & 1u) return ctx->fail(SS_ERR_INVALID, "ss_pr_set_teleport: a teleport set holds a node id >= n_nodes");
    if (h_err & 2u) return ctx->fail(SS_ERR_INVALID, "ss_pr_set_teleport: a teleport set lists a node twice (the ids of a set must be distinct)");
    double h_nz[MAXK];
    for (int k = 0; k < MAXK; k++) h_nz[k] = (double)h_cnt[k];
    SS_HIP(ctx, hipMemcpyAsync(pr->tin.p, h_tin, sizeof(h_tin), hipMemcpyHostToDevice, st));
    SS_HIP(ctx, hipMemcpyAsync(pr->nz_in.p, h_nz, sizeof(h_nz), hipMemcpyHostToDevice, st));
    SS_HIP(ctx, hipStreamSynchronize(st));
    p.memb = pr->memb.p;
    p.tin = pr->tin.p;
    p.nz_in = pr->nz_in.p;
    p.ts_mask = mask;
    return SS_OK;
}

int32_t ss_pr_destroy(ss_pr* pr) {
#ifdef SS_PR_WAVETIME
    if (pr) ss::pr_dump_wave_times(pr);
#endif

    if (!pr) return SS_ERR_INVALID;
    ss_ctx* ctx = pr->g->ctx;
    std::lock_guard<std::recursive_mutex> lk(ctx->mu);
    (void)hipSetDevice(ctx->device);
    if (!ss::device_wedged(ctx->device)) {
        (void)hipStreamSynchronize(ctx->stream);
        (void)hipStreamSynchronize(ctx->comm_stream);
    }
    pr->g->users--;
    delete pr;
    return SS_OK;
}

int32_t ss_pr_begin(ss_pr* pr) {
    if (!pr) return SS_ERR_INVALID;
    ss_ctx* ctx = pr->g->ctx;
    std::lock_guard<std::recursive_mutex> lk(ctx->mu);
    SS_HIP(ctx, hipSetDevice(ctx->device));
    if (pr->need_finalize) return ctx->fail(SS_ERR_STATE, "ss_pr_begin: pending exchange/finalize");
    SS_HIP(ctx, hipMemsetAsync(&pr->ctl.p->ticket, 0, sizeof(uint32_t), ctx->stream));
    ss::pr_launch_begin(pr, ctx->stream, ss::begin_blocks(pr));
    SS_HIP(ctx, hipGetLastError());
    pr->begun = true;
    if (pr->g->world > 1) {
        pr->need_finalize = true;
        pr->finalize_is_begin = true;
    }
    return SS_OK;
}

int32_t ss_pr_step(ss_pr* pr, int32_t n_steps) {
    if (!pr) return SS_ERR_INVALID;
    ss_ctx* ctx = pr->g->ctx;
    std::lock_guard<std::recursive_mutex> lk(ctx->mu);
    SS_HIP(ctx, hipSetDevice(ctx->device));
    if (!pr->begun) return ctx->fail(SS_ERR_STATE, "ss_pr_step: ss_pr_begin not called");
    if (pr->need_finalize) return ctx->fail(SS_ERR_STATE, "ss_pr_step: pending exchange/finalize");
    if (n_steps < 1) return ctx->fail(SS_ERR_INVALID, "ss_pr_step: n_steps < 1");
    if (pr->g->world > 1 && n_steps != 1) return ctx->fail(SS_ERR_INVALID, "ss_pr_step: world>1 needs an exchange after every step");
    SS_HIP(ctx, hipEventRecord(ctx->ev[0][0], ctx->stream));
    if (pr->persist && !pr->prm.memb && !pr->prm.aff) {
        ss::pr_multi_n_launch(pr, ctx->stream, (int)n_steps);
    } else {
        for (int i = 0; i < n_steps; i++) ss::pr_launch_step(pr, ctx->stream);
    }
    SS_HIP(ctx, hipEventRecord(ctx->ev[0][1], ctx->stream));
    ctx->ev_valid[0] = true;
    SS_HIP(ctx, hipGetLastError());
    if (pr->g->world > 1) {
        pr->need_finalize = true;
        pr->finalize_is_begin = false;
    }
    return SS_OK;
}

int32_t ss_pr_finalize(ss_pr* pr) {
    if (!pr) return SS_ERR_INVALID;
    ss_ctx* ctx = pr->g->ctx;
    std::lock_guard<std::recursive_mutex> lk(ctx->mu);
    SS_HIP(ctx, hipSetDevice(ctx->device));
    if (pr->g->world == 1) return ctx->fail(SS_ERR_STATE, "ss_pr_finalize: world==1 folds the finalize into the sweep");
    if (!pr->need_finalize) return ctx->fail(SS_ERR_STATE, "ss_pr_finalize: nothing to finalize");
    ss::pr_launch_finalize(pr, ctx->stream, pr->finalize_is_begin ? 1 : 0);
    SS_HIP(ctx, hipGetLastError());
    pr->need_finalize = false;
    return SS_OK;
}

int32_t ss_pr_exchange_buffers(ss_pr* pr, void** send_dev, uint64_t* send_bytes, void** recv_dev, uint64_t* recv_bytes) {
    if (!pr) return SS_ERR_INVALID;
    ss_ctx* ctx = pr->g->ctx;
    if (pr->g->world == 1) return ctx->fail(SS_ERR_STATE, "ss_pr_exchange_buffers: world==1 has no exchange");
    if (send_dev) *send_dev = pr->send.p;
    if (send_bytes) *send_bytes = pr->send.bytes();
    if (recv_dev) *recv_dev = pr->tab0.p;
    if (recv_bytes) *recv_bytes = (uint64_t)pr->g->nd_int * pr->gw * sizeof(double);
    return SS_OK;
}

int32_t ss_pr_exchange(ss_pr* pr, int32_t allreduce) {
    if (!pr) return SS_ERR_INVALID;
    ss_ctx* ctx = pr->g->ctx;
    std::lock_guard<std::recursive_mutex> lk(ctx->mu);
    SS_HIP(ctx, hipSetDevice(ctx->device));
    const ss_graph* g = pr->g;
    if (g->world == 1) return ctx->fail(SS_ERR_STATE, "ss_pr_exchange: world==1 has no exchange");
    if (!pr->need_finalize) return ctx->fail(SS_ERR_STATE, "ss_pr_exchange: nothing to exchange (call after ss_pr_begin / ss_pr_step)");
    if (!ctx->comm || ctx->comm_world != g->world || ctx->comm_rank != g->rank)
        return ctx->fail(SS_ERR_STATE, "ss_pr_exchange: the context's communicator (rank %d of %d) does not match the graph's shard (rank %d of %d)",
                         ctx->comm ? ctx->comm_rank : -1, ctx->comm ? ctx->comm_world : 0, g->rank, g->world);
    const size_t slice = (size_t)g->sl_nd * pr->gw;
    if (!allreduce && ctx->opt("pr.wire_f32", 0) != 0) {
        SS_HIP(ctx, ss::pr_wire_alloc(pr));
        ss::pr_wire_pack(pr, ctx->stream);
        SS_TRY(ss::comm_allgather(ctx, pr->wire_send.p, pr->wire_recv.p, ss::pr_wire_floats(pr) * sizeof(float)));
        ss::pr_wire_unpack(pr, ctx->stream);
        return SS_OK;
    }
    if (!allreduce) return ss::comm_allgather(ctx, pr->send.p, pr->tab0.p, slice * sizeof(double));
    SS_HIP(ctx, hipMemsetAsync(pr->tab0.p, 0, pr->tab0.bytes(), ctx->stream));
    SS_HIP(ctx, hipMemcpyAsync(pr->tab0.p + (size_t)g->rank * slice, pr->send.p, slice * sizeof(double), hipMemcpyDeviceToDevice, ctx->stream));
    return ss::comm_allreduce_f64(ctx, pr->tab0.p, pr->tab0.p, slice * (size_t)g->world);
}

int32_t ss_pr_status(ss_pr* pr, int32_t* iters_out, int32_t* n_active, int32_t* sweeps, double* last_delta_out,
                     double* last_total_out) {
    if (!pr) return SS_ERR_INVALID;
    ss_ctx* ctx = pr->g->ctx;
    std::lock_guard<std::recursive_mutex> lk(ctx->mu);
    SS_HIP(ctx, hipSetDevice(ctx->device));
    const PrCtl* hp = nullptr;
    SS_TRY(read_ctl(ctx, pr, ctx->stream, "ss_pr_status", &hp));
    const PrCtl h = *hp;
    if (h.stuck) return ctx->fail(SS_ERR_STATE, "ss_pr_status: the multi-sweep kernel gave up waiting between two sweeps (its grid of %u blocks was not resident: "
                                  "other kernels held the CUs for seconds); the state is void — set option pr.persistent = 0 and run again", pr->nblocks);
    for (int k = 0; k < pr->k; k++) {
        if (iters_out) iters_out[k] = h.iters[k];
        if (last_delta_out) last_delta_out[k] = h.delta[k];
        if (last_total_out) last_total_out[k] = h.S[k];
    }
    if (n_active) *n_active = h.n_active;
    if (sweeps) *sweeps = h.sweep;
    return SS_OK;
}

int32_t ss_pr_read_local(ss_pr* pr, uint32_t* ids_out, double* rank_out) {
    if (!pr || !rank_out) return SS_ERR_INVALID;
    ss_ctx* ctx = pr->g->ctx;
    std::lock_guard<std::recursive_mutex> lk(ctx->mu);
    SS_HIP(ctx, hipSetDevice(ctx->device));
    const ss_graph* g = pr->g;
    const size_t n_rows = (size_t)g->cnt_nd + g->cnt_d;
    ss::DevBuf<uint32_t> d_ids;
    ss::DevBuf<double> d_out;
    SS_HIP(ctx, d_ids.alloc(n_rows));
    SS_HIP(ctx, d_out.alloc(n_rows * pr->k));
    SS_GW_DISPATCH(pr->gw, launch_read, pr, ctx->stream, 0, (uint64_t)n_rows, d_ids.p, d_out.p);
    SS_HIP(ctx, hipGetLastError());
    if (ids_out && n_rows) SS_HIP(ctx, hipMemcpyAsync(ids_out, d_ids.p, n_rows * sizeof(uint32_t), hipMemcpyDefault, ctx->stream));
    if (n_rows) SS_HIP(ctx, hipMemcpyAsync(rank_out, d_out.p, n_rows * pr->k * sizeof(double), hipMemcpyDefault, ctx->stream));
    SS_HIP(ctx, hipStreamSynchronize(ctx->stream));
    return SS_OK;
}

int32_t ss_pr_read(ss_pr* pr, double* rank_out) {
    if (!pr || !rank_out) return SS_ERR_INVALID;
    ss_ctx* ctx = pr->g->ctx;
    std::lock_guard<std::recursive_mutex> lk(ctx->mu);
    SS_HIP(ctx, hipSetDevice(ctx->device));
    const ss_graph* g = pr->g;
    if (g->world != 1) return ctx->fail(SS_ERR_STATE, "ss_pr_read: world>1, use ss_pr_read_local");
    hipPointerAttribute_t pa{};
    const bool dev_out = hipPointerGetAttributes(&pa, rank_out) == hipSuccess && pa.type == hipMemoryTypeDevice;
    (void)hipGetLastError();
    ss::DevBuf<double> d_out;
    if (!dev_out) SS_HIP(ctx, d_out.alloc((size_t)g->n * pr->k));
    SS_GW_DISPATCH(pr->gw, launch_read, pr, ctx->stream, 1, (uint64_t)g->n, (uint32_t*)nullptr, dev_out ? rank_out : d_out.p);
    SS_HIP(ctx, hipGetLastError());
    if (!dev_out) SS_HIP(ctx, hipMemcpyAsync(rank_out, d_out.p, (size_t)g->n * pr->k * sizeof(double), hipMemcpyDefault, ctx->stream));
    SS_HIP(ctx, hipStreamSynchronize(ctx->stream));
    return SS_OK;
}

int32_t ss_pr_probe(ss_pr* pr, int32_t mode, int32_t n_reps, float* ms_out) {
    if (!pr || !ms_out) return SS_ERR_INVALID;
    ss_ctx* ctx = pr->g->ctx;
    std::lock_guard<std::recursive_mutex> lk(ctx->mu);
    SS_HIP(ctx, hipSetDevice(ctx->device));
    if (pr->gw < 8) return ctx->fail(SS_ERR_UNSUPPORTED, "ss_pr_probe: the probe mirrors the chunked gather of the K >= 5 kernels");
    if (mode < 0 || (mode & 7) > 2 || (mode >> 3) > 4 || n_reps < 1) return ctx->fail(SS_ERR_INVALID, "ss_pr_probe: mode 0..2 (+ 8 * gather cache policy 0..4), n_reps >= 1");
    const int pol = mode >> 3;
    mode &= 7;
    const uint32_t hot = (uint32_t)ctx->opt("pr.probe_hot", 24576);
    const ss_graph* g = pr->g;
    const unsigned nb = (unsigned)ctx->cu_count * 8;
    ss::DevBuf<double> sink;
    SS_HIP(ctx, sink.alloc((size_t)nb * TPB));
    hipEvent_t e0, e1;
    SS_HIP(ctx, hipEventCreate(&e0));
    SS_HIP(ctx, hipEventCreate(&e1));
    hipStream_t st = ctx->stream;
    ss::DevBuf<double> full;
    if (pr->prm.share) {
        SS_HIP(ctx, full.alloc(((size_t)g->nd_int + 1) * pr->gw));
        SS_HIP(ctx, hipMemsetAsync(full.p, 0, full.bytes(), ctx->stream));
    }
    const double* T = pr->prm.share ? full.p : pr->tab0.p;
    for (int r = 0; r < n_reps + 1; r++) {
        if (r == 1) SS_HIP(ctx, hipEventRecord(e0, st));
#define SS_PROBE_LAUNCH(GWV, POLV) hipLaunchKernelGGL((k_pr_probe<GWV, POLV>), dim3(nb), dim3(TPB), 0, st, T, (const uint32_t*)g->in_src.p, (size_t)g->e_local, (uint32_t)g->nd_int, mode, sink.p, hot)
        if (pr->gw == 8) SS_PROBE_LAUNCH(8, 0);
        else switch (pol) {
            case 0: SS_PROBE_LAUNCH(16, 0); break;
            case 1: SS_PROBE_LAUNCH(16, 1); break;
            case 2: SS_PROBE_LAUNCH(16, 2); break;
            case 3: SS_PROBE_LAUNCH(16, 3); break;
            default: SS_PROBE_LAUNCH(16, 4); break;
        }
    }
    SS_HIP(ctx, hipEventRecord(e1, st));
    SS_HIP(ctx, hipEventSynchronize(e1));
    float ms = 0.f;
    SS_HIP(ctx, hipEventElapsedTime(&ms, e0, e1));
    (void)hipEventDestroy(e0);
    (void)hipEventDestroy(e1);
    SS_HIP(ctx, hipGetLastError());
    *ms_out = ms / (float)n_reps;
    return SS_OK;
}

}
```

spaghettisearch_amd/csrc/pagerank_run.hip:

```cpp
#include "pr_state.hpp"

#include <algorithm>

namespace {

constexpr int AFF_KC = 16;
__global__ __launch_bounds__(TPB) void k_aff_delta(const double2* __restrict__ xp, const double2* __restrict__ xn, const AffCtl* __restrict__ a,
                                                   uint32_t sl_nd, uint32_t pos_nd, uint32_t pos_d, double* __restrict__ partials) {
    __shared__ double red[WAVES][AFF_KC];
    if (a->n_active == 0) return;
    const int k_real = a->k_real;
    const double r_old = a->r_prev, r_new = a->r_x, s_old = a->s_prev, s_new = a->s_x;
    const uint32_t n_rows = pos_nd + pos_d;
    const int lane = threadIdx.x & 63, wave = threadIdx.x >> 6;
    for (int k0 = 0; k0 < k_real; k0 += AFF_KC) {
        double u[AFF_KC], d_old[AFF_KC], d_new[AFF_KC], acc[AFF_KC];
        bool any = false;
#pragma unroll
        for (int j = 0; j < AFF_KC; j++) {
            const bool on = k0 + j < k_real && a->active[k0 + j] != 0;
            any = any || on;
            u[j] = on ? a->u[k0 + j] : 0.0;
            d_old[j] = on ? r_old * u[j] + s_old : 1.0;
            d_new[j] = on ? r_new * u[j] + s_new : 1.0;
// ... 366 lines not shown
                for (int s = 0; s < S; s++) ctl_and_emit(s, A[s].gath.p, (size_t)AFF_MAXK, 0);
            }
            it++;
            if (max_iter > 0 && it >= max_iter) break;
        }
        SS_HIP(ctx, hipGetLastError());
        ctx->pin_used = 0;
        int32_t* const hn = ctx->pin<int32_t>();
        SS_HIP(ctx, hipMemcpyAsync(hn, &A[0].aff.p->n_active, sizeof(int32_t), hipMemcpyDeviceToHost, st));
        SS_TRY(ss::sync_bounded(ctx, st, "sharded two-vector sweep (waiting for the exchange)"));
        n_active = *hn;
        if (max_iter > 0 && it >= max_iter) break;
    }
    if (lag && max_iter > 0 && it >= max_iter && n_active > 0) {
        it--;
        for (int s = 0; s < S; s++) {
            ss_pr* pr = sh[s].blk[0];
            hipLaunchKernelGGL(k_aff_local, dim3(1), dim3(AFF_MAXK), 0, st, (const AffCtl*)A[s].aff.p, (const PrCtl*)pr->ctl.p, (const double*)A[s].partials.p,
                               AFF_NB, A[s].n_zero, A[s].loc.p);
        }
        SS_TRY(exchange_sums(st));
        for (int s = 0; s < S; s++) ctl_and_emit(s, A[s].gath.p, (size_t)AFF_MAXK, 0);
        it++;
        SS_HIP(ctx, hipGetLastError());
    }
    for (int s = 0; s < S; s++) sh[s].blk[0]->need_finalize = false;
    if (iters_out) {
        std::vector<AffCtl> h(1);
        SS_HIP(ctx, hipMemcpyAsync(h.data(), A[0].aff.p, sizeof(AffCtl), hipMemcpyDeviceToHost, st));
        SS_TRY(ss::sync_bounded(ctx, st, "sharded two-vector sweep (status)"));
        for (int k = 0; k < k_topics; k++) iters_out[k] = h[0].iters[k];
    }
    return SS_OK;
}
int32_t local_ids(ss_pr* pr, uint32_t* ids_out) {
    const size_t n_rows = (size_t)pr->g->cnt_nd + pr->g->cnt_d;
    std::vector<double> scratch(std::max<size_t>(1, n_rows * (size_t)pr->k));
    return ss_pr_read_local(pr, ids_out, scratch.data());
}

int32_t check_eps(ss_ctx* ctx, const char* who, double eps, int32_t max_iter) {
    if (!(eps >= 0.0) && max_iter <= 0 && !(eps != eps)) return ctx->fail(SS_ERR_INVALID, "%s: eps < 0 (never converges) needs max_iter > 0", who);
    return SS_OK;
}

int32_t make_topic_blocks(ss_ctx* ctx, const char* who, ss_graph* const* shards, int n_shards, bool affine, bool check_first, double damping, double eps,
                          int32_t max_iter, int32_t k_topics, const int32_t* n_topic, std::vector<ShardBlocks>& sh, std::vector<AffShard>& aff, std::vector<int>& k0) {
    const int B = affine ? 1 : topic_blocks_for(ctx, k_topics);
    sh.resize(n_shards);
    aff.resize(affine ? n_shards : 0);
    k0.resize(B + 1);
    for (int b = 0; b <= B; b++) k0[b] = (int)((int64_t)k_topics * b / B);
    auto check_sizes = [&]() -> int32_t {
        for (int k = 0; k < k_topics; k++)
            if (n_topic[k] < 1) return ctx->fail(SS_ERR_INVALID, "%s: n_topic[%d] < 1", who, k);
        return SS_OK;
    };
    if (affine && check_first) SS_TRY(check_sizes());
    const int32_t two[2] = {1, 1};
    for (int s = 0; s < n_shards; s++) {
        for (int b = 0; b < B; b++) {
            ss_pr* pr = nullptr;
            SS_TRY(affine ? ss_pr_create(shards[s], damping, -1.0, 0, 2, two, &pr)
                          : ss_pr_create(shards[s], damping, eps, max_iter, k0[b + 1] - k0[b], n_topic + k0[b], &pr));
            sh[s].blk.push_back(pr);
        }
        if (affine && !check_first && s == 0) SS_TRY(check_sizes());
        if (affine) SS_TRY(aff_attach(sh[s].blk[0], aff[s], k_topics, n_topic, shards[s]->world));
    }
    return SS_OK;
}

int32_t run_affine(ss_graph* g, double damping, double eps, int32_t max_iter, int32_t k_topics, const int32_t* n_topic,
                   double* rank_out, int32_t* iters_out) {
    ss_ctx* ctx = g->ctx;
    hipStream_t st = ctx->stream;
    if (k_topics > AFF_MAXK) return ctx->fail(SS_ERR_UNSUPPORTED, "ss_pagerank_run (pr.affine): at most %d topics", AFF_MAXK);
    for (int k = 0; k < k_topics; k++)
        if (n_topic[k] < 1) return ctx->fail(SS_ERR_INVALID, "ss_pagerank_run: n_topic[%d] < 1", k);
    const int32_t two[2] = {1, 1};
    ss_pr* pr = nullptr;
    SS_TRY(ss_pr_create(g, damping, -1.0, 0, 2, two, &pr));
    struct Guard { ss_pr* p; ~Guard() { ss_pr_destroy(p); } } guard{pr};
    if (!pr->nwave || pr->gw != 2) return ctx->fail(SS_ERR_UNSUPPORTED, "ss_pagerank_run (pr.affine): needs the wave-item K = 2 sweep (pr.narrow_wave / pr.force_narrow at their defaults)");
    const uint32_t n_local = g->n_local();
    ss::DevBuf<AffCtl> aff;
    ss::DevBuf<double> x_prev, partials, d_out;
    SS_HIP(ctx, aff.alloc(1));
    SS_HIP(ctx, x_prev.alloc((size_t)n_local * 2));
    SS_HIP(ctx, partials.alloc((size_t)AFF_NB * AFF_MAXK));
    SS_TRY(aff_init(pr, k_topics, n_topic, aff.p, x_prev.p));
    hipPointerAttribute_t at{};
    const bool dev_out = hipPointerGetAttributes(&at, rank_out) == hipSuccess && at.type == hipMemoryTypeDevice;
    (void)hipGetLastError();
    double* out = rank_out;
    if (!dev_out) {
        SS_HIP(ctx, d_out.alloc((size_t)k_topics * g->n));
        out = d_out.p;
    }
    SS_TRY(ss_pr_begin(pr));
    const double n_zero = (double)((g->cnt_nd - pr->prm.pos_nd) + (g->cnt_d - pr->prm.pos_d));
    int32_t n_active = k_topics, it = 0;
    const int BATCH = 4;
    while (n_active > 0) {
        for (int b = 0; b < BATCH; b++) {
            const double2* const x_old = reinterpret_cast<const double2*>((it & 1) ? x_prev.p : pr->x.p);
            const double2* const x_new = reinterpret_cast<const double2*>((it & 1) ? pr->x.p : x_prev.p);
            ss::pr_launch_step(pr, st);
            hipLaunchKernelGGL(k_aff_delta, dim3(AFF_NB), dim3(TPB), 0, st, x_old, x_new, (const AffCtl*)aff.p, g->sl_nd, pr->prm.pos_nd, pr->prm.pos_d, partials.p);
            hipLaunchKernelGGL(k_aff_ctl, dim3(1), dim3(AFF_MAXK), 0, st, aff.p, pr->ctl.p, (const double*)partials.p, AFF_NB, n_zero, eps, max_iter, (size_t)AFF_MAXK);
            hipLaunchKernelGGL(k_aff_emit, dim3((unsigned)std::min<uint64_t>(4096, ss::div_up(g->n, TPB))), dim3(TPB), 0, st, x_new, (const PrCtl*)pr->ctl.p,
                               (const AffCtl*)aff.p, (const uint32_t*)g->new_id.p, g->n, g->sl_nd, pr->prm.pos_nd, pr->prm.pos_d, out);
            it++;
            if (max_iter > 0 && it >= max_iter) break;
        }
        SS_HIP(ctx, hipGetLastError());
        SS_HIP(ctx, ss::fetch(ctx, st, &n_active, &aff.p->n_active, sizeof(int32_t)));
        if (max_iter > 0 && it >= max_iter) break;
    }
    std::vector<AffCtl> h(1);
    SS_HIP(ctx, hipMemcpyAsync(h.data(), aff.p, sizeof(AffCtl), hipMemcpyDeviceToHost, st));
    if (!dev_out) SS_HIP(ctx, hipMemcpyAsync(rank_out, d_out.p, (size_t)k_topics * g->n * sizeof(double), hipMemcpyDeviceToHost, st));
    SS_HIP(ctx, hipStreamSynchronize(st));
    if (iters_out)
        for (int k = 0; k < k_topics; k++) iters_out[k] = h[0].iters[k];
    return SS_OK;
}

}

extern "C" {

int32_t ss_pagerank_run_sharded(ss_graph* g, double damping, double eps, int32_t max_iter, int32_t k_topics,
                                const int32_t* n_topic, int32_t allreduce, uint32_t* ids_out, double* rank_out, int32_t* iters_out) {
    if (!g) return SS_ERR_INVALID;
    ss_ctx* ctx = g->ctx;
    std::lock_guard<std::recursive_mutex> lk(ctx->mu);
    if (g->world < 2) return ctx->fail(SS_ERR_STATE, "ss_pagerank_run_sharded: needs a sharded graph (world > 1); use ss_pagerank_run");
    const bool affine = ctx->opt("pr.affine", 0) != 0 && !allreduce;
    const int k_max = affine ? AFF_MAXK : MAXK;
    if (k_topics < 1 || k_topics > k_max || !n_topic || !rank_out)
        return ctx->fail(SS_ERR_INVALID, "ss_pagerank_run_sharded: k_topics must be 1..%d, n_topic/rank_out not NULL", k_max);
    SS_TRY(check_eps(ctx, "ss_pagerank_run_sharded", eps, max_iter));
    if (!ctx->comm || ctx->comm_world != g->world || ctx->comm_rank != g->rank)
        return ctx->fail(SS_ERR_STATE, "ss_pagerank_run_sharded: the context's communicator (rank %d of %d) does not match the graph's shard (rank %d of %d)",
                         ctx->comm ? ctx->comm_rank : -1, ctx->comm ? ctx->comm_world : 0, g->rank, g->world);
    SS_HIP(ctx, hipSetDevice(ctx->device));
    std::vector<ShardBlocks> sh;
    std::vector<AffShard> aff;
    std::vector<int> k0;
    int32_t rc = make_topic_blocks(ctx, "ss_pagerank_run_sharded", &g, 1, affine, false, damping, eps, max_iter, k_topics, n_topic, sh, aff, k0);
    const bool wire_f32 = ctx->opt("pr.wire_f32", 0) != 0;
    if (rc == SS_OK) {
        auto exchange = [&](int b, hipStream_t xs) -> int32_t {
            ss_pr* pr = sh[0].blk[b];
            const size_t slice = (size_t)g->sl_nd * pr->gw;
            if (!allreduce && wire_f32) {
                SS_HIP(ctx, ss::pr_wire_alloc(pr));
                ss::pr_wire_pack(pr, xs);
                SS_TRY(ss::comm_allgather_on(ctx, pr->wire_send.p, pr->wire_recv.p, ss::pr_wire_floats(pr) * sizeof(float), xs));
                ss::pr_wire_unpack(pr, xs);
                return SS_OK;
            }
            if (!allreduce) return ss::comm_allgather_on(ctx, pr->send.p, pr->tab0.p, slice * sizeof(double), xs);
            SS_HIP(ctx, hipMemsetAsync(pr->tab0.p, 0, pr->tab0.bytes(), xs));
            SS_HIP(ctx, hipMemcpyAsync(pr->tab0.p + (size_t)g->rank * slice, pr->send.p, slice * sizeof(double), hipMemcpyDeviceToDevice, xs));
            return ss::comm_allreduce_f64_on(ctx, pr->tab0.p, pr->tab0.p, slice * (size_t)g->world, xs);
        };
        if (affine) {
            auto exchange_sums = [&](hipStream_t xs) -> int32_t {
                return ss::comm_allgather_on(ctx, aff[0].loc.p, aff[0].gath.p, (size_t)AFF_MAXK * sizeof(double), xs);
            };
            rc = run_affine_sharded(ctx, sh, aff, g->world, eps, max_iter, k_topics, exchange, exchange_sums, iters_out);
        } else {
            rc = run_pipelined(ctx, sh, max_iter, exchange, iters_out, k0);
        }
    }
    const size_t n_rows = (size_t)g->cnt_nd + g->cnt_d;
    if (affine) {
        if (rc == SS_OK && ids_out) rc = local_ids(sh[0].blk[0], ids_out);
        if (rc == SS_OK && n_rows) {
            if (hipMemcpyAsync(rank_out, aff[0].out.p, (size_t)k_topics * n_rows * sizeof(double), hipMemcpyDefault, ctx->stream) != hipSuccess ||
                hipStreamSynchronize(ctx->stream) != hipSuccess)
                rc = ctx->fail(SS_ERR_HIP, "ss_pagerank_run_sharded: copy of the ranks failed");
        }
    } else
    for (int b = 0; b < (int)sh[0].blk.size() && rc == SS_OK; b++)
        rc = ss_pr_read_local(sh[0].blk[b], b == 0 ? ids_out : nullptr, rank_out + (size_t)k0[b] * n_rows);
    for (ss_pr* pr : sh[0].blk) ss_pr_destroy(pr);
    return rc;
}

int32_t ss_pagerank_run_group(ss_graph* const* shards, int32_t world, double damping, double eps, int32_t max_iter, int32_t k_topics,
                              const int32_t* n_topic, double* rank_out, int32_t* iters_out) {
    if (!shards || world < 2 || !shards[0]) return SS_ERR_INVALID;
    ss_ctx* ctx = shards[0]->ctx;
    std::lock_guard<std::recursive_mutex> lk(ctx->mu);
    const bool affine = ctx->opt("pr.affine", 0) != 0;
    const int k_max = affine ? AFF_MAXK : MAXK;
    if (k_topics < 1 || k_topics > k_max || !n_topic || !rank_out)
        return ctx->fail(SS_ERR_INVALID, "ss_pagerank_run_group: k_topics must be 1..%d, n_topic/rank_out not NULL", k_max);
    SS_TRY(check_eps(ctx, "ss_pagerank_run_group", eps, max_iter));
    for (int s = 0; s < world; s++)
        if (!shards[s] || shards[s]->ctx != ctx || shards[s]->world != world || shards[s]->rank != s || shards[s]->n != shards[0]->n)
            return ctx->fail(SS_ERR_INVALID, "ss_pagerank_run_group: shards[%d] is not shard %d of %d of the same graph on this context", s, s, world);
    SS_HIP(ctx, hipSetDevice(ctx->device));
    std::vector<ShardBlocks> sh;
    std::vector<AffShard> aff;
    std::vector<int> k0;
    int32_t rc = make_topic_blocks(ctx, "ss_pagerank_run_group", shards, world, affine, true, damping, eps, max_iter, k_topics, n_topic, sh, aff, k0);
    const int B = (int)k0.size() - 1;
    if (rc == SS_OK) {
        const bool wire_f32 = ctx->opt("pr.wire_f32", 0) != 0;
        auto exchange = [&](int b, hipStream_t xs) -> int32_t {
            if (wire_f32) {
                for (int src = 0; src < world; src++) {
                    SS_HIP(ctx, ss::pr_wire_alloc(sh[src].blk[b]));
                    ss::pr_wire_pack(sh[src].blk[b], xs);
                }
                for (int dst = 0; dst < world; dst++) {
                    ss_pr* to = sh[dst].blk[b];
                    for (int src = 0; src < world; src++) {
                        ss_pr* from = sh[src].blk[b];
                        SS_HIP(ctx, hipMemcpyAsync(to->wire_recv.p + (size_t)src * ss::pr_wire_floats(from), from->wire_send.p, ss::pr_wire_floats(from) * sizeof(float),
                                                   hipMemcpyDeviceToDevice, xs));
                    }
                    ss::pr_wire_unpack(to, xs);
                }
                return SS_OK;
            }
            for (int dst = 0; dst < world; dst++)
                for (int src = 0; src < world; src++) {
                    ss_pr* from = sh[src].blk[b];
                    ss_pr* to = sh[dst].blk[b];
                    const size_t slice = (size_t)shards[src]->sl_nd * from->gw;
                    SS_HIP(ctx, hipMemcpyAsync(to->tab0.p + (size_t)src * slice, from->send.p, slice * sizeof(double), hipMemcpyDeviceToDevice, xs));
                }
            return SS_OK;
        };
        if (affine) {
            auto exchange_sums = [&](hipStream_t xs) -> int32_t {
                for (int dst = 0; dst < world; dst++)
                    for (int src = 0; src < world; src++)
                        SS_HIP(ctx, hipMemcpyAsync(aff[dst].gath.p + (size_t)src * AFF_MAXK, aff[src].loc.p, (size_t)AFF_MAXK * sizeof(double),
                                                   hipMemcpyDeviceToDevice, xs));
                return SS_OK;
            };
            rc = run_affine_sharded(ctx, sh, aff, world, eps, max_iter, k_topics, exchange, exchange_sums, iters_out);
        } else {
            rc = run_pipelined(ctx, sh, max_iter, exchange, iters_out, k0);
        }
    }
    const uint64_t n = shards[0]->n;
    for (int s = 0; s < world && rc == SS_OK && affine; s++) {
        const size_t n_rows = (size_t)shards[s]->cnt_nd + shards[s]->cnt_d;
        std::vector<uint32_t> ids(n_rows);
        std::vector<double> part((size_t)k_topics * n_rows);
        rc = local_ids(sh[s].blk[0], ids.data());
        if (rc == SS_OK && n_rows) {
            if (hipMemcpyAsync(part.data(), aff[s].out.p, part.size() * sizeof(double), hipMemcpyDeviceToHost, ctx->stream) != hipSuccess ||
                hipStreamSynchronize(ctx->stream) != hipSuccess)
                rc = ctx->fail(SS_ERR_HIP, "ss_pagerank_run_group: copy of the ranks failed");
        }
        for (int k = 0; k < k_topics && rc == SS_OK; k++)
            for (size_t i = 0; i < n_rows; i++) rank_out[(size_t)k * n + ids[i]] = part[(size_t)k * n_rows + i];
    }
    for (int s = 0; s < world && rc == SS_OK && !affine; s++) {
        const size_t n_rows = (size_t)shards[s]->cnt_nd + shards[s]->cnt_d;
        std::vector<uint32_t> ids(n_rows);
        for (int b = 0; b < B && rc == SS_OK; b++) {
            const int kb = k0[b + 1] - k0[b];
            std::vector<double> part((size_t)kb * n_rows);
            rc = ss_pr_read_local(sh[s].blk[b], ids.data(), part.data());
            if (rc != SS_OK) break;
            for (int k = 0; k < kb; k++)
                for (size_t i = 0; i < n_rows; i++) rank_out[(size_t)(k0[b] + k) * n + ids[i]] = part[(size_t)k * n_rows + i];
        }
    }
    for (auto& s : sh)
        for (ss_pr* pr : s.blk) ss_pr_destroy(pr);
    return rc;
}

int32_t ss_pagerank_run(ss_graph* g, double damping, double eps, int32_t max_iter, int32_t k_topics,
                        const int32_t* n_topic, double* rank_out, int32_t* iters_out) {
    if (!g) return SS_ERR_INVALID;
    ss_ctx* ctx = g->ctx;
    std::lock_guard<std::recursive_mutex> lk(ctx->mu);
    if (g->world != 1) return ctx->fail(SS_ERR_STATE, "ss_pagerank_run: needs a (rank 0, world 1) graph");
    if (k_topics < 1 || k_topics > SS_MAX_TOPICS || !n_topic || !rank_out)
        return ctx->fail(SS_ERR_INVALID, "ss_pagerank_run: bad k_topics / NULL argument");
    SS_TRY(check_eps(ctx, "ss_pagerank_run", eps, max_iter));
    if (ctx->opt("pr.affine", 0) != 0) return run_affine(g, damping, eps, max_iter, k_topics, n_topic, rank_out, iters_out);
    for (int k0 = 0; k0 < k_topics; k0 += MAXK) {
        const int kk = std::min(MAXK, k_topics - k0);
        ss_pr* pr = nullptr;
        SS_TRY(ss_pr_create(g, damping, eps, max_iter, kk, n_topic + k0, &pr));
        int32_t rc = ss_pr_begin(pr);
        int32_t n_active = kk, sweeps = 0;
        const int BATCH = 8;
        while (rc == SS_OK && n_active > 0) {
            int todo = BATCH;
            if (max_iter > 0) todo = std::min(BATCH, std::max(1, max_iter - sweeps));
            rc = ss_pr_step(pr, todo);
            if (rc == SS_OK) rc = ss_pr_status(pr, iters_out ? iters_out + k0 : nullptr, &n_active, &sweeps, nullptr, nullptr);
        }
        if (rc == SS_OK) rc = ss_pr_read(pr, rank_out + (size_t)k0 * g->n);
        ss_pr_destroy(pr);
        if (rc != SS_OK) return rc;
    }
    return SS_OK;
}

}
```

spaghettisearch_amd/csrc/pr_plan.hpp:

```cpp
#pragma once
#include "sorted_degrees.hpp"

#include <algorithm>
#include <cstdint>
#include <utility>
#include <vector>

namespace {

constexpr int TPB = 256;
constexpr int WAVES = TPB / 64;
constexpr int CH = 16;
constexpr uint32_t SEGW = 2048;

enum : uint32_t { W_SEG = 0, W_WAVE = 1, W_GROUP = 2, W_ZERO = 3,
                  V_SEG = 8,
                  V_ROWW = 9,
                  V_QUAD = 10,
                  V_DEG = 11,
                  V_ZERO = 12 };

struct WorkItem {
    uint32_t kind;
    uint32_t row;
    uint32_t count;
    uint32_t nseg;
    uint32_t sbase;
    uint32_t tix;
    uint32_t beg, end;
};

constexpr uint32_t plan_div_up(uint64_t a, uint64_t b) { return (uint32_t)((a + b - 1) / b); }

struct PlanOptions {
    static constexpr int64_t AUTO = INT64_MIN;
    uint32_t t_quad = 128;
    uint32_t item_turns = 4;
    size_t items_per_wave = 1;
    int64_t deal_snake = AUTO;
    int64_t deal_global = 2;
    int64_t blocks_per_cu = AUTO;
    int64_t class_order = 235401;
    int64_t n_class_order = 2310;
    int64_t stagger = 0;
};

struct PlanScratch {
    std::vector<WorkItem> seg, rwg, wav, grp, zer;
    std::vector<WorkItem> vseg, vroww, vquad, vdeg[3], vzero;
    std::vector<WorkItem> items, dealt;
    std::vector<double> cost, load;
    std::vector<uint32_t> owner, by_load, idx, order, bucket, woff, cnt;
    std::vector<std::pair<double, uint32_t>> key;
};
inline PlanScratch& plan_scratch() {
    static thread_local PlanScratch s;
    return s;
}

struct Cut {
    std::vector<WorkItem>& items;
    uint32_t nsegs = 0, nmulti = 0;
    uint32_t seg_edges = 0;
    uint32_t pos_nd = 0, pos_d = 0;
    uint32_t vbeg[7] = {0};
};

inline Cut cut_items(const ss::SortedDegrees& nd, const ss::SortedDegrees& d, uint32_t sl_nd, int gw, bool lane_rows, const PlanOptions& opt) {
    PlanScratch& s = plan_scratch();
    Cut cut{s.items};
    uint32_t& nsegs = cut.nsegs;
    uint32_t& nmulti = cut.nmulti;
    const uint32_t NSLOT = 64 / gw;
    const uint32_t T_SEG = 32 * NSLOT;
    const uint32_t T_WAVE = 2 * NSLOT;
    const uint32_t seg_edges = cut.seg_edges = 128 * NSLOT;
    auto &seg = s.seg, &rwg = s.rwg, &wav = s.wav, &grp = s.grp, &zer = s.zer;
    auto &vseg = s.vseg, &vroww = s.vroww, &vquad = s.vquad, &vzero = s.vzero;
    auto& vdeg = s.vdeg;
    for (auto* v : {&seg, &rwg, &wav, &grp, &zer, &vseg, &vroww, &vquad, &vdeg[0], &vdeg[1], &vdeg[2], &vzero}) v->clear();
    auto emit_v = [&](const ss::SortedDegrees& deg, uint32_t row0, bool non_dangling, uint32_t& n_pos) {
        const uint32_t cnt = (uint32_t)deg.size();
        const uint32_t T_MULTI = 4096, T_DEG = 8;
        const uint32_t T_QUAD = opt.t_quad;
        const uint32_t item_turns = opt.item_turns;
        size_t j_at = 0, j_lim = 0;
        const size_t n_run = deg.val.size();
        auto deg_at = [&](uint32_t r) -> uint32_t {
            while (deg.start[j_at + 1] <= r) j_at++;
            return deg.val[j_at];
        };
        auto end_above = [&](uint32_t lim) -> uint32_t {
            while (j_lim < n_run && deg.val[j_lim] > lim) j_lim++;
            return deg.start[j_lim];
        };
        uint32_t r = 0;
        for (; r < cnt && deg_at(r) > T_MULTI; r++) {
            const uint32_t ns = (deg_at(r) + SEGW - 1) / SEGW;
            const uint32_t tix = nmulti++;
            for (uint32_t sg = 0; sg < ns; sg++) vseg.push_back({V_SEG, row0 + r, sg, ns, nsegs, tix});
            nsegs += ns;
        }
        {
            const uint32_t end = std::min(cnt, end_above(T_QUAD));
            for (; r < end; r++) vroww.push_back({V_ROWW, row0 + r, 0, 0, 0, 0});
        }
        while (r < cnt && deg_at(r) > T_DEG) {
            const uint32_t nch = (deg_at(r) + CH - 1) / CH;
            const uint32_t max_groups = std::min<uint32_t>((uint32_t)gw, std::max<uint32_t>(1u, 2u * item_turns / nch));
            const uint32_t lim = std::max<uint32_t>(T_DEG, (nch - 1) * CH);
            const uint32_t end = end_above(lim);
            const uint32_t same = end > r ? end - r : 0u;
            const uint32_t rows = std::min<uint32_t>(same, max_groups * NSLOT);
            vquad.push_back({V_QUAD, row0 + r, rows, nch, 0, 0});
            r += rows;
        }
        while (r < cnt && deg_at(r) > 0) {
            const uint32_t D = deg_at(r);
            const uint32_t run = deg.start[j_at + 1] - r;
            const uint32_t R = D <= 2 ? 8 : D <= 4 ? 4 : 2;
            const uint32_t per_item = lane_rows ? 64u * item_turns : NSLOT * R * item_turns;
            auto& out = vdeg[R == 2 ? 0 : R == 4 ? 1 : 2];
            for (uint32_t o = 0; o < run; o += per_item) out.push_back({V_DEG, row0 + r + o, std::min(per_item, run - o), D, 0, 0});
            r += run;
        }
        n_pos = r;
        const uint32_t ZERO_ROWS = 16 * NSLOT;
        if (non_dangling)
            for (uint32_t o = r; o < cnt; o += ZERO_ROWS) vzero.push_back({V_ZERO, row0 + o, std::min<uint32_t>(ZERO_ROWS, cnt - o), 0, 0, 0});
    };
    auto emit = [&](const ss::SortedDegrees& deg, uint32_t row0, bool non_dangling, uint32_t& n_pos) {
        if (gw >= 8) { emit_v(deg, row0, non_dangling, n_pos); return; }
        const uint32_t cnt = (uint32_t)deg.size();
        const uint32_t a = deg.first_at_most(T_SEG);
        const uint32_t c = std::max(a, deg.first_at_most(0));
        for (uint32_t r = 0; r < a; r++) {
            const uint32_t ns = (deg[r] + seg_edges - 1) / seg_edges;
            const uint32_t tix = ns > 1 ? nmulti++ : 0;
            for (uint32_t sg = 0; sg < ns; sg++) seg.push_back({W_SEG, row0 + r, sg, ns, nsegs, tix});
            nsegs += ns;
        }
        {
            const uint32_t b = std::min(c, std::max(a, deg.first_at_most(T_WAVE)));
            for (uint32_t r = a; r < b; r += WAVES) wav.push_back({W_WAVE, row0 + r, std::min<uint32_t>(WAVES, b - r), 0, 0, 0});
            const uint32_t GROUP_ROWS = WAVES * NSLOT * 4;
            for (uint32_t r = b; r < c; r += GROUP_ROWS) grp.push_back({W_GROUP, row0 + r, std::min<uint32_t>(GROUP_ROWS, c - r), 0, 0, 0});
        }
        n_pos = c;
        const uint32_t ZERO_ROWS = (TPB * 8) / gw;
        if (non_dangling)
            for (uint32_t r = c; r < cnt; r += ZERO_ROWS) zer.push_back({W_ZERO, row0 + r, std::min<uint32_t>(ZERO_ROWS, cnt - r), 0, 0, 0});
    };
    emit(nd, 0, true, cut.pos_nd);
    const size_t vquad_split = vquad.size();
    emit(d, sl_nd, false, cut.pos_d);
    auto& items = cut.items;
    auto& vbeg = cut.vbeg;
    items.clear();
    items.reserve(seg.size() + rwg.size() + wav.size() + grp.size() + zer.size());
    items.insert(items.end(), seg.begin(), seg.end());
    items.insert(items.end(), rwg.begin(), rwg.end());
    items.insert(items.end(), wav.begin(), wav.end());
    items.insert(items.end(), grp.begin(), grp.end());
    items.insert(items.end(), zer.begin(), zer.end());
    vbeg[0] = (uint32_t)items.size();
    items.insert(items.end(), vseg.begin(), vseg.end());
    items.insert(items.end(), vroww.begin(), vroww.end());
    vbeg[1] = (uint32_t)items.size();
    std::inplace_merge(vquad.begin(), vquad.begin() + (ptrdiff_t)vquad_split, vquad.end(),
                       [](const WorkItem& a, const WorkItem& b) { return a.nseg > b.nseg; });
    items.insert(items.end(), vquad.begin(), vquad.end());
    for (int k = 0; k < 3; k++) {
        vbeg[2 + k] = (uint32_t)items.size();
        items.insert(items.end(), vdeg[k].begin(), vdeg[k].end());
    }
    vbeg[5] = (uint32_t)items.size();
    items.insert(items.end(), vzero.begin(), vzero.end());
    vbeg[6] = (uint32_t)items.size();
    if (items.empty()) items.push_back({W_ZERO, 0, 0, 0, 0, 0});
    return cut;
}

inline const std::vector<double>& item_costs(const Cut& cut, const ss::SortedDegrees& nd, const ss::SortedDegrees& d, uint32_t sl_nd, int gw, bool lane_rows) {
    const std::vector<WorkItem>& items = cut.items;
    std::vector<double>& cost = plan_scratch().cost;
    const uint32_t NS = 64 / gw;
    struct DegCursor {
        const ss::SortedDegrees* d;
        size_t j = 0;
        uint32_t at(uint32_t r) {
            if (r >= d->size()) return 0u;
            if (d->start[j] > r) j = d->run_of(r);
            while (d->start[j + 1] <= r) j++;
            return d->val[j];
        }
    } cur_nd{&nd}, cur_d{&d};
    auto deg_of = [&](uint32_t lrow) -> uint32_t { return lrow < sl_nd ? cur_nd.at(lrow) : cur_d.at(lrow - sl_nd); };
    cost.assign(items.size(), 0.0);
    for (size_t i = 0; i < items.size(); i++) {
        const WorkItem& w = items[i];
        double turns = 1.0;
        switch (w.kind) {
            case V_ROWW: turns = plan_div_up(deg_of(w.row), NS * CH); break;
            case V_SEG: turns = plan_div_up(std::min<uint32_t>(SEGW, deg_of(w.row) - w.count * SEGW), NS * CH) + 2.0; break;
            case V_QUAD: turns = (double)plan_div_up(w.count, NS) * w.nseg; break;
            case V_DEG: {
                if (lane_rows) { turns = (double)plan_div_up(w.count, 64u) * (0.6 + 0.2 * (w.nseg <= 2 ? 2 : w.nseg <= 4 ? 4 : 8)); break; }
                const uint32_t R = w.nseg <= 2 ? 8 : w.nseg <= 4 ? 4 : 2;
                turns = (double)plan_div_up(w.count, NS * R) * (R == 8 ? 2.5 : R == 4 ? 1.7 : 1.3);
                break;
            }
            default: turns = 0.5; break;
        }
        cost[i] = turns + 1.0;
    }
    return cost;
}

inline std::vector<uint32_t>& deal_items(const Cut& cut, const std::vector<double>& cost, uint32_t nw, bool lane_rows, const PlanOptions& opt) {
    PlanScratch& s = plan_scratch();
    const size_t n_items = cut.items.size();
    auto &owner = s.owner, &by_load = s.by_load, &idx = s.idx, &order = s.order, &bucket = s.bucket;
    auto& load = s.load;
    auto& key = s.key;
    owner.assign(n_items, 0u);
    load.assign(nw, 0.0);
    by_load.resize(nw);
    for (uint32_t w = 0; w < nw; w++) by_load[w] = w;
    const bool snake = (opt.deal_snake == PlanOptions::AUTO ? (n_items >= (size_t)8 * nw || lane_rows ? 1 : 0) : opt.deal_snake) != 0;
    const int64_t deal_mode = opt.deal_global;
    const bool global_order = deal_mode != 0;
    if (global_order) {
        constexpr uint32_t NB = 1u << 14;
        const auto bkey = [&](size_t i) { return NB - 1 - (uint32_t)std::min<double>(cost[i] * 16.0, (double)(NB - 1)); };
        bucket.assign(NB + 1, 0u);
        order.resize(n_items);
        size_t c0 = 0;
        for (int kcls = 0; kcls < (deal_mode == 2 ? 6 : 1); kcls++) {
            const size_t c1 = deal_mode == 2 ? (kcls < 5 ? std::min<size_t>(cut.vbeg[kcls + 1], n_items) : n_items) : n_items;
            if (kcls) std::fill(bucket.begin(), bucket.end(), 0u);
            for (size_t i = c0; i < c1; i++) bucket[bkey(i) + 1]++;
            for (uint32_t b = 0; b < NB; b++) bucket[b + 1] += bucket[b];
            for (size_t i = c0; i < c1; i++) order[c0 + bucket[bkey(i)]++] = (uint32_t)i;
            c0 = c1;
        }
    }
    for (size_t i0 = 0; i0 < n_items; i0 += nw) {
        const size_t n_chunk = std::min<size_t>(nw, n_items - i0);
        if (i0 && snake) {
            std::reverse(by_load.begin(), by_load.end());
        } else if (i0) {
            key.resize(nw);
            for (uint32_t w = 0; w < nw; w++) key[w] = {load[w], w};
            std::sort(key.begin(), key.end());
            for (uint32_t w = 0; w < nw; w++) by_load[w] = key[w].second;
        }
        idx.resize(n_chunk);
        for (size_t j = 0; j < n_chunk; j++) idx[j] = global_order ? order[i0 + j] : (uint32_t)(i0 + j);
        const auto falling = [&](uint32_t a, uint32_t b) { return cost[a] > cost[b]; };
        size_t run_end = 0, n_merge = 0;
        for (size_t j = 1; j <= n_chunk && !global_order; j++) {
            if (j < n_chunk && !(cost[i0 + j] > cost[i0 + j - 1])) continue;
            if (run_end) {
                if (++n_merge > 8) { std::stable_sort(idx.begin(), idx.end(), falling); break; }
                std::inplace_merge(idx.begin(), idx.begin() + (ptrdiff_t)run_end, idx.begin() + (ptrdiff_t)j, falling);
            }
            run_end = j;
        }
        for (size_t j = 0; j < n_chunk; j++) {
            owner[idx[j]] = by_load[j];
            load[by_load[j]] += cost[idx[j]];
        }
    }
    return owner;
}

inline const std::vector<uint32_t>& place_items(Cut& cut, std::vector<uint32_t>& owner, uint32_t nw) {
    PlanScratch& s = plan_scratch();
    auto& items = cut.items;
    auto &woff = s.woff, &cnt = s.cnt;
    woff.assign((size_t)nw * 8, 0);
    cnt.assign((size_t)nw * 8, 0);
    for (int k = 0; k < 6; k++) {
        const size_t i1 = k < 5 ? std::min<size_t>(cut.vbeg[k + 1], items.size()) : items.size();
        for (size_t i = std::min<size_t>(cut.vbeg[k], i1); i < i1; i++) { owner[i] = owner[i] * 8 + (uint32_t)k; cnt[owner[i]]++; }
    }
    uint32_t run_off = 0;
    for (uint32_t w = 0; w < nw; w++) {
        for (int k = 0; k < 8; k++) {
            woff[(size_t)w * 8 + k] = run_off;
            run_off += cnt[(size_t)w * 8 + k];
            cnt[(size_t)w * 8 + k] = woff[(size_t)w * 8 + k];
        }
    }
    s.dealt.resize(items.size());
    for (size_t i = 0; i < items.size(); i++) s.dealt[cnt[owner[i]]++] = items[i];
    s.dealt.push_back({V_ZERO, 0, 0, 0, 0, 0, 0, 0});
    s.dealt.push_back({V_ZERO, 0, 0, 0, 0, 0, 0, 0});
    items.swap(s.dealt);
    return woff;
}

inline uint32_t pack_class_order(int64_t code) {
    uint32_t packed = 0, seen = 0;
    for (int pos = 5; pos >= 0; pos--) {
        const uint32_t c = (uint32_t)(code % 10);
        code /= 10;
        packed |= (c & 7u) << (3 * pos);
        if (c < 6) seen |= 1u << c;
    }
    return seen == 0x3Fu ? packed : (0u | 1u << 3 | 2u << 6 | 3u << 9 | 4u << 12 | 5u << 15);
}
inline uint32_t pack_n_order(int64_t code) {
    uint32_t packed = 0, seen = 0;
    for (int pos = 3; pos >= 0; pos--) {
        const uint32_t c = (uint32_t)(code % 10);
        code /= 10;
        packed |= (c & 3u) << (2 * pos);
        if (c < 4) seen |= 1u << c;
    }
    return seen == 0xFu ? packed : (0u | 1u << 2 | 2u << 4 | 3u << 6);
}

struct SharedRows {
    std::vector<uint32_t> deg;
    uint32_t zrow = 0;
    uint32_t base = 0;
    uint64_t table_rows = 0;
    uint32_t row_of(uint32_t od) const {
        const auto it = std::lower_bound(deg.begin(), deg.end(), od);
        return it != deg.end() && *it == od ? base + (uint32_t)(it - deg.begin()) : zrow;
    }
};
inline SharedRows plan_shared_rows(const uint32_t* od, size_t n, uint32_t pos_nd) {
    SharedRows sh;
    uint32_t hi = 0;
    for (size_t i = 0; i < n; i++) hi = std::max(hi, od[i]);
    if (n && (uint64_t)hi <= 4 * (uint64_t)n + 65536) {
        std::vector<unsigned char> seen((size_t)hi + 1, 0);
        for (size_t i = 0; i < n; i++) seen[od[i]] = 1;
        for (size_t v = 0; v <= hi; v++)
            if (seen[v]) sh.deg.push_back((uint32_t)v);
    } else if (n) {
        sh.deg.assign(od, od + n);
        std::sort(sh.deg.begin(), sh.deg.end());
        sh.deg.erase(std::unique(sh.deg.begin(), sh.deg.end()), sh.deg.end());
    }
    sh.zrow = pos_nd;
    sh.base = pos_nd + 1;
    sh.table_rows = (uint64_t)pos_nd + 1 + sh.deg.size();
    return sh;
}

}
```

spaghettisearch_amd/csrc/pr_state.hpp:

```cpp
#pragma once
#include "graph.hpp"
#include "pr_plan.hpp"

#ifdef SS_PR_WAVETIME
#include <cstdio>
#include <cstdlib>
#include <string>
#endif

namespace {

constexpr int MAXK = 16;

struct PrCtl {
    double S[MAXK];
    double delta[MAXK];
    double csum[MAXK];
    double xz[MAXK];
    double xz_in[MAXK];
    double tele[MAXK];
    int32_t active[MAXK];
    int32_t iters[MAXK];
    int32_t sweep;
    int32_t n_active;
    uint32_t ticket;
    uint32_t stuck;
    uint32_t gticket[8];
};

constexpr int AFF_MAXK = 256;
constexpr unsigned AFF_NB = 512;
struct AffCtl {
    double u[AFF_MAXK];
    double delta[AFF_MAXK];
    int32_t active[AFF_MAXK], iters[AFF_MAXK], just[AFF_MAXK];
    double r_x, r_prev, r_next;
    double s_x, s_prev, s_next;
    double xz_prev[2];
    int32_t n_active, n_just, k_real, it;
};

struct PrParams {
    const uint32_t* in_ptr;
    const uint32_t* in_src;
    const uint32_t* outdeg;
    double* x;
    const double* tab_rd[2];
    double* tab_wr[2];
    const WorkItem* work;
    double* partials;
    double* segpart;
    uint32_t* rowticket;
    double* hubsum;
    uint32_t nmulti;
    PrCtl* ctl;
    const double* x0;
    double d, teleport, eps, tele_n;
    int32_t max_iter, k_topics, world;
    uint32_t sl_nd, cnt_nd, sl_d, cnt_d, seg_edges, n_items;
    uint32_t pos_nd, pos_d;
    const uint32_t* memb;
    const double* tin;
    const double* nz_in;
    uint32_t ts_mask;
    uint32_t zrow;
    const uint32_t* woff;
    uint32_t stagger_div;
    uint32_t stagger_code;
    uint32_t class_order;
    uint32_t n_order;
    double* x_alt;
    AffCtl* aff;
    const double* tele_col;
    const uint32_t* sh_deg;
    uint32_t n_shared;
    uint32_t share;
    uint32_t tab_rows;
};

}

enum PrKernel : int {
    PR_STEP = 0,
    PR_SWEEP = 1,
    PR_SWEEP_N = 2,
};

struct ss_pr {
    ss_graph* g = nullptr;
    PrKernel kernel = PR_SWEEP;
    int gw = 1;
    ss::DevBuf<float> wire_send, wire_recv;
    bool nwave = false;
    int persist_mode = 1;
    bool persist = false;
    int k = 1;
    PrParams prm{};
    unsigned nblocks = 0;
    ss::DevBuf<double> x, tab0, tab1, send, partials, segpart, hubsum, x0;
    ss::DevBuf<uint32_t> rowticket;
    ss::DevBuf<uint32_t> memb;
    ss::DevBuf<double> tin, nz_in;
    ss::DevBuf<WorkItem> work;
    ss::DevBuf<uint32_t> woff;
    ss::DevBuf<uint32_t> src_shared;
    ss::DevBuf<uint32_t> sh_deg;
    ss::DevBuf<PrCtl> ctl;
    bool begun = false;
    bool need_finalize = false;
    bool finalize_is_begin = false;
};

#pragma GCC visibility push(hidden)
namespace ss {
unsigned begin_blocks(const ss_pr* pr);
void pr_launch_begin(ss_pr* pr, hipStream_t st, unsigned nb);
void pr_launch_step(ss_pr* pr, hipStream_t st);
void pr_launch_finalize(ss_pr* pr, hipStream_t st, int is_begin);
void pr_sweep_launch(ss_pr* pr, hipStream_t st);
int pr_sweep_occupancy(int gw);
void pr_sweep_n_launch(ss_pr* pr, hipStream_t st);
int pr_sweep_n_occupancy(int gw);
void pr_multi_n_launch(ss_pr* pr, hipStream_t st, int n_steps);
int pr_multi_n_occupancy(int gw);
void pr_step_launch(ss_pr* pr, hipStream_t st);
int pr_step_occupancy(int gw);
#ifdef SS_PR_WAVETIME
void pr_dump_wave_times(const ss_pr* pr);
#endif
size_t pr_wire_floats(const ss_pr* pr);
hipError_t pr_wire_alloc(ss_pr* pr);
void pr_wire_pack(ss_pr* pr, hipStream_t st);
void pr_wire_unpack(ss_pr* pr, hipStream_t st);
}
#pragma GCC visibility pop

namespace {
#ifdef SS_PR_WAVETIME
inline FILE* open_dump(const char* name) {
    const char* dir = getenv("SS_PR_WAVETIME_DIR");
    return fopen((std::string(dir && *dir ? dir : ".") + "/" + name).c_str(), "w");
}
#endif
inline int32_t read_ctl(ss_ctx* ctx, const ss_pr* pr, hipStream_t st, const char* what, const PrCtl** out) {
    ctx->pin_used = 0;
    PrCtl* const hp = ctx->pin<PrCtl>();
    if (hipMemcpyAsync(hp, pr->ctl.p, sizeof(PrCtl), hipMemcpyDeviceToHost, st) != hipSuccess) return ctx->fail(SS_ERR_HIP, "%s: status read failed", what);
    SS_TRY(ss::sync_bounded(ctx, st, what));
    *out = hp;
    return SS_OK;
}
}
```

spaghettisearch_amd/csrc/pr_sweep.hip:

```cpp
#include "pr_device.hpp"

#include <algorithm>

namespace {

template <int GW>
__device__ __forceinline__ double tab_at(const double* __restrict__ T, uint32_t row, int t) {
    return *reinterpret_cast<const double*>(reinterpret_cast<const char*>(T) + (size_t)((row * (uint32_t)GW + (uint32_t)t) * 8u));
}


template <int GW, bool TS>
struct SweepCtx {
    const PrParams& p;
    const double* __restrict__ T;
    double* __restrict__ Tw;
    double S, x0;
    bool act;
    int t, gbase, slot;
    double dsum, csum;
};

__device__ __forceinline__ uint32_t turn_fill(uint32_t epos, uint32_t lim) {
    return min((uint32_t)CH, __builtin_elementwise_sub_sat(lim, epos));
}

template <int GW>
__device__ __forceinline__ void idx_turn(const uint32_t* __restrict__ in_src, uint32_t epos, uint32_t n, uint32_t zrow, int t, uint32_t (&src)[CH / GW]) {
#pragma unroll
    for (int r = 0; r < CH / GW; r++) {
        const uint32_t j = (uint32_t)(r * GW + t);
        const uint32_t raw = NT_LOAD(&in_src[j < n ? epos + j : 0u]);
        src[r] = j < n ? (raw & SRC_MASK) : zrow;
    }
}
template <int GW>
__device__ __forceinline__ void gather_turn(const double* __restrict__ T, const uint32_t (&src)[CH / GW], int t, int gbase, double (&v)[CH]) {
#pragma unroll
    for (int j = 0; j < CH; j++) {
        const uint32_t sj = (uint32_t)__shfl((int)src[j / GW], gbase + (j % GW), 64);
        v[j] = tab_at<GW>(T, sj, t);
    }
}

template <int GW, bool TS>
__device__ __forceinline__ void finish_row(SweepCtx<GW, TS>& c, uint32_t lrow, double y, double xo, uint32_t od, double* hub = nullptr) {
    const PrParams& p = c.p;
    y += c.x0;
    const size_t xi = (size_t)lrow * GW + c.t;
    double tele = p.teleport;
    if constexpr (TS) tele = teleport_of(p, lrow, c.t);
    double xn = (y + tele) / c.S;
    if (c.act) {
        NT_STORE(xn, &p.x[xi]);
        if (!hub) c.dsum += fabs(xn - xo);
    } else {
        xn = xo;
    }
    double cc = 0.0;
    if (lrow < p.sl_nd) {
        cc = p.d * xn / (double)od;
        NT_STORE(cc, &c.Tw[xi]);
        if (!hub) c.csum += cc;
    }
    if (hub) {
        __hip_atomic_store(&hub[c.t], fabs(xn - xo), __ATOMIC_RELAXED, __HIP_MEMORY_SCOPE_AGENT);
        __hip_atomic_store(&hub[GW + c.t], cc, __ATOMIC_RELAXED, __HIP_MEMORY_SCOPE_AGENT);
    }
}

template <int GW, bool TS>
__device__ __forceinline__ void long_rows(SweepCtx<GW, TS>& c, const WorkItem* __restrict__ work, uint32_t i0, uint32_t i1, int lane) {
    constexpr int NS = 64 / GW;
    constexpr uint32_t TW = NS * CH;
    const PrParams& p = c.p;
    if (i0 >= i1) return;
    WorkItem cur = work[i0], nxt = work[i0 + 1];
    uint32_t src_n[CH / GW];
    {
        const uint32_t e0 = cur.beg + (uint32_t)c.slot * CH;
        idx_turn<GW>(p.in_src, e0, turn_fill(e0, cur.end), p.zrow, c.t, src_n);
    }
    for (uint32_t it = i0; it < i1; it++) {
        const WorkItem nn = work[it + 2];
        const uint32_t lrow = cur.row;
        const double xo = NT_LOAD(&p.x[(size_t)lrow * GW + c.t]);
        const uint32_t od = lrow < p.sl_nd ? NT_LOAD(&p.outdeg[lrow]) : 1u;
        const uint32_t turns = (cur.end - cur.beg + TW - 1) / TW;
        const bool more = it + 1 < i1;
        double acc = 0.0;
        for (uint32_t i = 0; i < turns; i++) {
            uint32_t src[CH / GW];
#pragma unroll
            for (int r = 0; r < CH / GW; r++) src[r] = src_n[r];
            const bool last = i + 1 == turns;
            const uint32_t e1 = (last ? nxt.beg : cur.beg + (i + 1) * TW) + (uint32_t)c.slot * CH;
            const uint32_t lim = last ? (more ? nxt.end : 0u) : cur.end;
            idx_turn<GW>(p.in_src, e1, turn_fill(e1, lim), p.zrow, c.t, src_n);
            double v[CH];
            gather_turn<GW>(c.T, src, c.t, c.gbase, v);
#pragma unroll
            for (int j = 0; j < CH; j++) acc += v[j];
        }
        const double y = wave_sum_topic<GW>(acc);
        if (cur.kind == V_ROWW) {
            if (lane < GW) finish_row<GW>(c, lrow, y, xo, od);
        } else {
            if (lane < GW) __hip_atomic_store(&p.segpart[(size_t)(cur.sbase + cur.count) * GW + c.t], y, __ATOMIC_RELAXED, __HIP_MEMORY_SCOPE_AGENT);
            asm volatile("s_waitcnt vmcnt(0)" ::: "memory");
            unsigned prev = 0;
            if (lane == 0) prev = __hip_atomic_fetch_add(&p.rowticket[cur.tix], 1u, __ATOMIC_RELAXED, __HIP_MEMORY_SCOPE_AGENT);
            prev = (unsigned)__builtin_amdgcn_readfirstlane((int)prev);
            if (prev == cur.nseg - 1) {
                if (lane == 0) __hip_atomic_store(&p.rowticket[cur.tix], 0u, __ATOMIC_RELAXED, __HIP_MEMORY_SCOPE_AGENT);
                if (lane < GW) {
                    double ys = 0.0;
                    for (uint32_t q = 0; q < cur.nseg; q++)
                        ys += __hip_atomic_load(&p.segpart[(size_t)(cur.sbase + q) * GW + c.t], __ATOMIC_RELAXED, __HIP_MEMORY_SCOPE_AGENT);
                    finish_row<GW>(c, lrow, ys, xo, od, p.hubsum + (size_t)cur.tix * 2 * GW);
                }
            }
        }
        cur = nxt;
        nxt = nn;
    }
}

template <int GW, bool TS>
__device__ __forceinline__ void quad_rows(SweepCtx<GW, TS>& c, const WorkItem* __restrict__ work, uint32_t i0, uint32_t i1) {
    constexpr int NS = 64 / GW;
    const PrParams& p = c.p;
    if (i0 >= i1) return;
    const uint32_t myq = (uint32_t)c.t * NS + (uint32_t)c.slot;
    auto bounds = [&](const WorkItem& w, bool live, uint32_t& bv, uint32_t& ev, uint32_t& ov) __attribute__((always_inline)) {
        const bool have = live && myq < w.count;
        const uint32_t rq = live ? w.row + (have ? myq : 0u) : 0u;
        const uint32_t b = p.in_ptr[rq], e = p.in_ptr[rq + 1];
        bv = b;
        ev = have ? e : b;
        ov = rq < p.sl_nd ? NT_LOAD(&p.outdeg[rq]) : 1u;
    };
    WorkItem cur = work[i0], nxt = work[i0 + 1];
    uint32_t cb, ce, co, nb, ne, no;
    bounds(cur, true, cb, ce, co);
    bounds(nxt, i0 + 1 < i1, nb, ne, no);
    uint32_t it = i0, q = 0, ch = 0;
    uint32_t nq = (cur.count + NS - 1) / NS, nch = cur.nseg;
    uint32_t src_n[CH / GW];
    {
        const uint32_t b0 = (uint32_t)__shfl((int)cb, c.gbase, 64), e0 = (uint32_t)__shfl((int)ce, c.gbase, 64);
        idx_turn<GW>(p.in_src, b0, turn_fill(b0, e0), p.zrow, c.t, src_n);
    }
    double acc = 0.0;
    while (it < i1) {
        uint32_t src[CH / GW];
#pragma unroll
        for (int r = 0; r < CH / GW; r++) src[r] = src_n[r];
        uint32_t qn = q, cn = ch + 1;
        bool cross = false;
        if (cn == nch) {
            cn = 0;
            qn = q + 1;
            if (qn == nq) { qn = 0; cross = true; }
        }
        const bool live_n = !cross || it + 1 < i1;
        {
            const uint32_t b_n = (uint32_t)__shfl((int)(cross ? nb : cb), c.gbase + (int)qn, 64);
            const uint32_t e_n = (uint32_t)__shfl((int)(cross ? ne : ce), c.gbase + (int)qn, 64);
            const uint32_t ep = b_n + cn * CH;
            idx_turn<GW>(p.in_src, ep, live_n ? turn_fill(ep, e_n) : 0u, p.zrow, c.t, src_n);
        }
        const bool ends = ch + 1 == nch;
        const uint32_t lrow = cur.row + q * NS + (uint32_t)c.slot;
        const bool valid = q * NS + (uint32_t)c.slot < cur.count;
        double xo = 0.0;
        if (ends) xo = NT_LOAD(&p.x[(size_t)(valid ? lrow : cur.row) * GW + c.t]);
        double v[CH];
        gather_turn<GW>(c.T, src, c.t, c.gbase, v);
#pragma unroll
        for (int j = 0; j < CH; j++) acc += v[j];
        if (ends) {
            const uint32_t od = (uint32_t)__shfl((int)co, c.gbase + (int)q, 64);
            if (valid) finish_row<GW>(c, lrow, acc, xo, od);
            acc = 0.0;
        }
        q = qn;
        ch = cn;
        if (cross) {
            it++;
            cur = nxt;
            cb = nb; ce = ne; co = no;
            nq = (cur.count + NS - 1) / NS;
            nch = cur.nseg;
            nxt = work[it + 1];
            bounds(nxt, it + 1 < i1, nb, ne, no);
        }
    }
}

template <int GW, int R, bool TS>
__device__ __forceinline__ void deg_rows(SweepCtx<GW, TS>& c, const WorkItem* __restrict__ work, uint32_t i0, uint32_t i1) {
    constexpr int NS = 64 / GW;
    constexpr int DM = CH / R;
    constexpr int IR = CH / GW;
    const PrParams& p = c.p;
    if (i0 >= i1) return;
    auto idx = [&](const WorkItem& w, bool live, uint32_t turn, uint32_t (&src)[IR]) __attribute__((always_inline)) {
        const uint32_t rb = (turn * NS + (uint32_t)c.slot) * R;
#pragma unroll
        for (int r = 0; r < IR; r++) {
            const uint32_t j = (uint32_t)(r * GW + c.t);
            const uint32_t rr = rb + j / DM, u = j % DM;
            const bool ok = live && u < w.nseg && rr < w.count;
            const uint32_t raw = NT_LOAD(&p.in_src[ok ? w.beg + rr * w.nseg + u : 0u]);
            src[r] = ok ? (raw & SRC_MASK) : p.zrow;
        }
    };
    WorkItem cur = work[i0], nxt = work[i0 + 1];
    uint32_t src_n[IR];
    idx(cur, true, 0, src_n);
    for (uint32_t it = i0; it < i1; it++) {
        const WorkItem nn = work[it + 2];
        const uint32_t row0 = cur.row, count = cur.count;
        const uint32_t turns = (count + NS * R - 1) / (NS * R);
        for (uint32_t i = 0; i < turns; i++) {
            uint32_t src[IR];
#pragma unroll
            for (int r = 0; r < IR; r++) src[r] = src_n[r];
            if (i + 1 < turns) idx(cur, true, i + 1, src_n);
            else idx(nxt, it + 1 < i1, 0, src_n);
            const uint32_t rb = (i * NS + (uint32_t)c.slot) * R;
            double xo[R];
#pragma unroll
            for (int r = 0; r < R; r++) xo[r] = NT_LOAD(&p.x[(size_t)(row0 + (rb + r < count ? rb + r : 0u)) * GW + c.t]);
            const uint32_t myr = row0 + (rb + (uint32_t)c.t < count ? rb + (uint32_t)c.t : 0u);
            const uint32_t odv = (c.t < R && myr < p.sl_nd) ? NT_LOAD(&p.outdeg[myr]) : 1u;
            double v[CH];
            gather_turn<GW>(c.T, src, c.t, c.gbase, v);
#pragma unroll
            for (int r = 0; r < R; r++) {
                double y = 0.0;
#pragma unroll
                for (int u = 0; u < DM; u++) y += v[r * DM + u];
                const uint32_t od = (uint32_t)__shfl((int)odv, c.gbase + r, 64);
                if (rb + r < count) finish_row<GW>(c, row0 + rb + r, y, xo[r], od);
            }
        }
        cur = nxt;
        nxt = nn;
    }
}

#ifndef SS_PR_MINW
#define SS_PR_MINW 1
#endif
#ifdef SS_PR_WAVETIME
__device__ unsigned long long g_pr_wt[65536][2];
#endif
template <int GW, bool TS>
__global__ __launch_bounds__(TPB, SS_PR_MINW) void k_pr_sweep(PrParams p) {
    constexpr int NS = 64 / GW;
    PrCtl* ctl = p.ctl;
    if (ctl->n_active == 0) return;
#ifdef SS_PR_WAVETIME
    unsigned long long wt0;
    asm volatile("s_memrealtime %0\n\ts_waitcnt lgkmcnt(0)" : "=s"(wt0));
#endif
    const int sweep = ctl->sweep;
    const int lane = threadIdx.x & 63;
    const uint32_t wave = (uint32_t)__builtin_amdgcn_readfirstlane((int)(threadIdx.x >> 6));
    SweepCtx<GW, TS> c{p, p.tab_rd[sweep & 1], p.tab_wr[sweep & 1], 0.0, 0.0, false, lane % GW, lane - lane % GW, lane / GW, 0.0, 0.0};
    c.S = ctl->S[c.t];
    c.act = ctl->active[c.t] != 0;
    c.x0 = sweep == 0 ? p.x0[c.t] : 0.0;

    if constexpr (!TS) {
        if (p.n_shared) {
            const double xz_out = c.act ? zero_row_rank(p, sweep, c.S, p.x0[c.t]) : ctl->xz[c.t];
            const uint32_t nel = p.n_shared * (uint32_t)GW;
            for (uint32_t i = blockIdx.x * TPB + threadIdx.x; i < nel; i += gridDim.x * TPB)
                c.Tw[(size_t)(p.zrow + 1) * GW + i] = p.d * xz_out / (double)p.sh_deg[i / GW];
        }
    }

    const uint32_t* __restrict__ off = p.woff + (size_t)(blockIdx.x * WAVES + wave) * 8;
    int rot = p.stagger_div ? (int)((blockIdx.x / p.stagger_div) % 6u) : 0;
    if (p.stagger_code) {
        uint32_t cdv = p.stagger_code;
        for (uint32_t r = blockIdx.x / p.stagger_div; r > 0; r--) cdv /= 6u;
        rot = (int)(cdv % 6u);
    }
    for (int s6 = 0; s6 < 6; s6++) {
    const int cls = (int)((p.class_order >> (3 * ((s6 + rot) % 6))) & 7u);
    {
        int ln = lane;
        asm volatile("" : "+v"(ln));
        c.t = ln % GW;
        c.gbase = ln - ln % GW;
        c.slot = ln / GW;
    }
    switch (cls) {
    case 0: long_rows<GW>(c, p.work, off[0], off[1], lane); break;
    case 1: quad_rows<GW>(c, p.work, off[1], off[2]); break;
    case 2: deg_rows<GW, 2>(c, p.work, off[2], off[3]); break;
    case 3: deg_rows<GW, 4>(c, p.work, off[3], off[4]); break;
    case 4: deg_rows<GW, 8>(c, p.work, off[4], off[5]); break;
    default:
    for (uint32_t item = off[5]; item < off[6]; item++) {
        const WorkItem w = p.work[item];
        const bool store = TS || !p.share;
        const bool ts = TS && p.memb && ((p.ts_mask >> c.t) & 1u);
        const double xz_out = c.act ? (ts ? zero_row_rank_ts(p, sweep, c.S, p.x0[c.t], 0.0) : zero_row_rank(p, sweep, c.S, p.x0[c.t])) : ctl->xz[c.t];
        const double xz_inn = ts ? (c.act ? zero_row_rank_ts(p, sweep, c.S, p.x0[c.t], p.tin[c.t]) : ctl->xz_in[c.t]) : xz_out;
        uint32_t od[16];
#pragma unroll
        for (int i = 0; i < 16; i++) {
            const uint32_t rr = (uint32_t)(i * NS + c.slot);
            od[i] = NT_LOAD(&p.outdeg[w.row + (rr < w.count ? rr : 0u)]);
        }
#pragma unroll
        for (int i = 0; i < 16; i++) {
            const uint32_t rr = (uint32_t)(i * NS + c.slot);
            if (rr < w.count) {
                const uint32_t lrow = w.row + rr;
                const double xz = ts && ((p.memb[lrow] >> c.t) & 1u) ? xz_inn : xz_out;
                const double cc = p.d * xz / (double)od[i];
                if (store) NT_STORE(cc, &c.Tw[(size_t)lrow * GW + c.t]);
                c.csum += cc;
            }
        }
    }
    break;
    }
    }
#ifdef SS_PR_WAVETIME
    {
        unsigned long long wt1;
        asm volatile("s_waitcnt vmcnt(0)\n\ts_memrealtime %0\n\ts_waitcnt lgkmcnt(0)" : "=s"(wt1));
        const uint32_t wid = (blockIdx.x * WAVES + wave) & 65535u;
        if (lane == 0) { g_pr_wt[wid][0] = wt0; g_pr_wt[wid][1] = wt1; }
    }
#endif
    block_reduce_and_publish<GW>(p, c.dsum, c.csum, c.Tw, false);
}

template __device__ void begin_caller_context<8, 16>(const PrParams&, double*);

}

namespace ss {
void pr_sweep_launch(ss_pr* pr, hipStream_t st) {
    const bool ts = pr->prm.memb != nullptr;
    if (pr->gw == 8) {
        if (ts) hipLaunchKernelGGL((k_pr_sweep<8, true>), dim3(pr->nblocks), dim3(TPB), 0, st, pr->prm);
        else hipLaunchKernelGGL((k_pr_sweep<8, false>), dim3(pr->nblocks), dim3(TPB), 0, st, pr->prm);
    } else {
        if (ts) hipLaunchKernelGGL((k_pr_sweep<16, true>), dim3(pr->nblocks), dim3(TPB), 0, st, pr->prm);
        else hipLaunchKernelGGL((k_pr_sweep<16, false>), dim3(pr->nblocks), dim3(TPB), 0, st, pr->prm);
    }
}
int pr_sweep_occupancy(int gw) {
    int per_cu = 8;
    if (gw == 8) (void)hipOccupancyMaxActiveBlocksPerMultiprocessor(&per_cu, k_pr_sweep<8, false>, TPB, 0);
    else (void)hipOccupancyMaxActiveBlocksPerMultiprocessor(&per_cu, k_pr_sweep<16, false>, TPB, 0);
    return per_cu;
}

#ifdef SS_PR_WAVETIME
void pr_dump_wave_times(const ss_pr* pr) {
    if (pr->gw < 8) return;
    (void)hipDeviceSynchronize();
    const uint32_t nwv = std::min<uint32_t>(65536u, pr->nblocks * WAVES);
    std::vector<unsigned long long> h((size_t)nwv * 2);
    if (hipMemcpyFromSymbol(h.data(), HIP_SYMBOL(g_pr_wt), h.size() * sizeof(unsigned long long)) != hipSuccess || !nwv) return;
    unsigned long long t0 = ~0ull;
    for (uint32_t w = 0; w < nwv; w++) t0 = std::min(t0, h[2 * w]);
    std::vector<double> st(nwv), en(nwv);
    for (uint32_t w = 0; w < nwv; w++) { st[w] = (double)(h[2 * w] - t0) / 100.0; en[w] = (double)(h[2 * w + 1] - t0) / 100.0; }
    std::sort(st.begin(), st.end()); std::sort(en.begin(), en.end());
    if (FILE* f = open_dump("pr_wt.csv")) {
        fprintf(f, "wave,start_us,end_us\n");
        for (uint32_t w = 0; w < nwv; w++) fprintf(f, "%u,%.2f,%.2f\n", w, (double)(h[2 * w] - t0) / 100.0, (double)(h[2 * w + 1] - t0) / 100.0);
        fclose(f);
    }
    fprintf(stderr, "[pr wavetime] %u waves: start us median %.1f max %.1f | out of items us min %.1f p10 %.1f median %.1f p90 %.1f p99 %.1f max %.1f\n", nwv,
            st[nwv / 2], st[nwv - 1], en[0], en[nwv / 10], en[nwv / 2], en[nwv * 9 / 10], en[(size_t)nwv * 99 / 100], en[nwv - 1]);
}
#endif
}
```

spaghettisearch_amd/engine.py:

```python
from __future__ import annotations

import ctypes as C
from typing import Optional, Sequence

import numpy as np

from . import _lib
from ._lib import SsGraphInfo, SsHit, SsPassage, SsTermMatch, check

HIT_DTYPE = np.dtype([("doc", "<u4"), ("_pad", "<u4"), ("title", "<f8"), ("body", "<f8"),
                      ("pagerank", "<f8"), ("final", "<f8")])

TERM_MATCH_DTYPE = np.dtype([("title_w", "<f4"), ("body_w", "<f4"), ("flags", "<u4"), ("body_pos", "<f4")])

PASSAGE_DTYPE = np.dtype([("start", "<f4"), ("last", "<f4"), ("n_distinct", "<u4"), ("n_occ", "<u4"), ("token_mask", "<u8")])

DOC_RANGE_DTYPE = np.dtype([("field", "<i4"), ("_pad", "<i4"), ("lo", "<i8"), ("hi", "<i8")])

VEC_HIT_DTYPE = np.dtype([("doc", "<u4"), ("score", "<i4")])

FUSED_DTYPE = np.dtype([("score", "<f8"), ("vec_score", "<i4"), ("lex_rank", "<u2"), ("vec_rank", "<u2")])
FUSE_RRF, FUSE_WEIGHTED = 0, 1

_NP2T = {"uint64": "int64", "uint32": "int32"}
# ... 1 lines not shown

def _is_torch(x) -> bool:
    return type(x).__module__.startswith("torch")


def _as(x, dtype: str):
    if x is None:
        return None
    if _is_torch(x):
        import torch
        want = getattr(torch, _NP2T.get(dtype, dtype))
        if x.dtype != want:
            raise TypeError(f"torch tensor has dtype {x.dtype}, expected {want}")
        return x.contiguous()
    return np.ascontiguousarray(x, dtype=np.dtype(dtype))


def _ptr(x) -> Optional[int]:
    if x is None:
        return None
    if _is_torch(x):
        return x.data_ptr()
    return x.ctypes.data


class Context:

    def __init__(self, device_id: int = 0):
        self.lib = _lib.load()
        h = C.c_void_p()
        check(self.lib.ss_init(device_id, C.byref(h)))
        self.h = h
        self.device_id = device_id
        self._options = {}

    def set_stream(self, hip_stream: Optional[int]) -> None:
        check(self.lib.ss_set_stream(self.h, C.c_void_p(hip_stream)), self.h)
        self._shared_stream = bool(hip_stream)

    def ready(self, *arrays) -> None:
        if getattr(self, "_shared_stream", False):
            return
        for a in arrays:
            if a is not None and _is_torch(a) and a.is_cuda:
                import torch
                torch.cuda.current_stream(a.device).synchronize()
                return

    def merge_hits(self, parts, n_hits, k: int, doc_base=None, out=None):
        n_hits = _as(n_hits, "int32")
        n_parts, n_q = int(n_hits.shape[0]), int(n_hits.shape[1])
        doc_base = _as(doc_base, "uint32")
        if _is_torch(parts):
            parts = parts.contiguous()
            have = parts.numel() * parts.element_size()
        else:
            parts = np.ascontiguousarray(parts, dtype=HIT_DTYPE)
            have = parts.nbytes
        if have != n_parts * n_q * k * HIT_DTYPE.itemsize:
            raise ValueError("parts does not hold n_parts*n_q*k hits")
        if out is not None:
            hits, n_out = out
            if hits.numel() * hits.element_size() < n_q * k * HIT_DTYPE.itemsize or n_out.numel() < n_q:
                raise ValueError("output buffers too small")
        else:
            hits = np.zeros((n_q, k), dtype=HIT_DTYPE)
            n_out = np.zeros(n_q, dtype=np.int32)
        self.ready(parts, n_hits, doc_base)
        check(self.lib.ss_merge_hits(self.h, n_q, n_parts, k, _ptr(parts), _ptr(n_hits), _ptr(doc_base), _ptr(hits), _ptr(n_out)), self.h)
        return hits, n_out

    def synchronize(self) -> None:
        check(self.lib.ss_synchronize(self.h), self.h)

    def set_option(self, name: str, value: Optional[int]) -> None:
        check(self.lib.ss_set_option(self.h, name.encode(), -(1 << 63) if value is None else int(value)), self.h)
        if value is None:
            self._options.pop(name, None)
        else:
            self._options[name] = int(value)

    def options(self, **kv):
        ctx = self

        class _Scope:
            def __enter__(self_inner):
                self_inner.before = {k.replace("__", "."): ctx._options.get(k.replace("__", ".")) for k in kv}
                for k, v in kv.items():
                    ctx.set_option(k.replace("__", "."), v)

            def __exit__(self_inner, *exc):
                for name, old in self_inner.before.items():
                    ctx.set_option(name, old)
                return False
        return _Scope()

    @staticmethod
    def comm_unique_id() -> bytes:
        buf = C.create_string_buffer(_lib.SS_COMM_ID_BYTES)
        check(_lib.load().ss_comm_unique_id(buf))
        return buf.raw

    def comm_init(self, uid: bytes, rank: int, world: int) -> None:
        if len(uid) != _lib.SS_COMM_ID_BYTES:
            raise ValueError("communicator id must be SS_COMM_ID_BYTES long")
        check(self.lib.ss_comm_init(self.h, C.c_char_p(uid), rank, world), self.h)

    def comm_split(self, color: int, key: int) -> None:
        check(self.lib.ss_comm_split(self.h, color, key), self.h)

    def comm_destroy(self) -> None:
        check(self.lib.ss_comm_destroy(self.h), self.h)

    def comm_info(self):
        r, w = C.c_int32(), C.c_int32()
        check(self.lib.ss_comm_info(self.h, C.byref(r), C.byref(w)), self.h)
        return r.value, w.value

    def comm_allreduce_u64(self, buf) -> None:
        buf = _as(buf, "uint64")
        self.ready(buf)
        check(self.lib.ss_comm_allreduce_u64(self.h, _ptr(buf), int(buf.shape[0])), self.h)

    def comm_allgather(self, send, recv, bytes_per_rank: int) -> None:
        self.ready(send, recv)
        check(self.lib.ss_comm_allgather(self.h, _ptr(send), _ptr(recv), int(bytes_per_rank)), self.h)

    def last_kernel_ms(self, kind: int) -> float:
        ms = C.c_float(0)
        check(self.lib.ss_last_kernel_ms(self.h, kind, C.byref(ms)), self.h)
        return float(ms.value)

    def close(self) -> None:
        if self.h:
            self.lib.ss_shutdown(self.h)
            self.h = None


class Graph:

    def __init__(self, ctx: Context, n_nodes: int, out_ptr, out_dst, rank: int = 0, world: int = 1):
        self.ctx = ctx
        self.n = int(n_nodes)
        out_ptr = _as(out_ptr, "uint64")
        out_dst = _as(out_dst, "uint32")
        self.e = int(out_dst.shape[0]) if out_dst is not None else 0
        if out_ptr.shape[0] != self.n + 1:
            raise ValueError("out_ptr must have n_nodes+1 entries")
        ctx.ready(out_ptr, out_dst)
        h = C.c_void_p()
        check(ctx.lib.ss_graph_create(ctx.h, self.n, self.e, _ptr(out_ptr), _ptr(out_dst), rank, world, C.byref(h)), ctx.h)
        self.h = h
        self.rank, self.world = rank, world

    def apply_delta(self, n_nodes_new: int, changed, new_ptr, new_children) -> None:
        changed = _as(changed, "uint32")
        new_ptr = _as(new_ptr, "uint64")
        new_children = _as(new_children, "uint32")
        self.ctx.ready(changed, new_ptr, new_children)
        check(self.ctx.lib.ss_graph_apply_delta(self.h, int(n_nodes_new), int(changed.shape[0]), _ptr(changed), _ptr(new_ptr), _ptr(new_children)),
              self.ctx.h)
        self.n = int(n_nodes_new)

    def info(self) -> SsGraphInfo:
        gi = SsGraphInfo()
        check(self.ctx.lib.ss_graph_get_info(self.h, C.byref(gi)), self.ctx.h)
        return gi

    def pagerank_sharded(self, damping: float, eps: float, n_topic: Sequence[int], max_iter: int = 0, allreduce: bool = False, out=None):
        n_topic = np.ascontiguousarray(np.atleast_1d(n_topic), dtype=np.int32)
        K = len(n_topic)
        rows = int(self.info().n_rows_local)
        if out is not None:
            ids, rank = _as(out[0], "uint32"), _as(out[1], "float64")
            count = lambda a: a.numel() if _is_torch(a) else a.size
            if count(ids) < rows or count(rank) < K * rows:
                raise ValueError("out arrays too small")
        else:
            ids = np.zeros(rows, dtype=np.uint32)
            rank = np.zeros((K, rows), dtype=np.float64)
        iters = np.zeros(K, dtype=np.int32)
        check(self.ctx.lib.ss_pagerank_run_sharded(self.h, damping, eps, max_iter, K, _ptr(n_topic), 1 if allreduce else 0,
                                                   _ptr(ids), _ptr(rank), _ptr(iters)), self.ctx.h)
        return ids, rank, iters

    def pagerank(self, damping: float, eps: float, n_topic: Sequence[int], max_iter: int = 0):
        n_topic = np.ascontiguousarray(np.atleast_1d(n_topic), dtype=np.int32)
        K = len(n_topic)
        rank = np.zeros((K, self.n), dtype=np.float64)
        iters = np.zeros(K, dtype=np.int32)
        check(self.ctx.lib.ss_pagerank_run(self.h, damping, eps, max_iter, K, _ptr(n_topic), _ptr(rank), _ptr(iters)),
              self.ctx.h)
        return rank, iters

    @staticmethod
    def pagerank_group(shards, damping: float, eps: float, n_topic: Sequence[int], max_iter: int = 0):
        n_topic = np.ascontiguousarray(np.atleast_1d(n_topic), dtype=np.int32)
        K = len(n_topic)
        ctx = shards[0].ctx
        hs = (C.c_void_p * len(shards))(*[g.h for g in shards])
        rank = np.zeros((K, shards[0].n), dtype=np.float64)
        iters = np.zeros(K, dtype=np.int32)
        check(ctx.lib.ss_pagerank_run_group(hs, len(shards), damping, eps, max_iter, K, _ptr(n_topic), _ptr(rank), _ptr(iters)), ctx.h)
        return rank, iters

    def pagerank_dev(self, damping: float, eps: float, n_topic: Sequence[int], rank_out, max_iter: int = 0):
        n_topic = np.ascontiguousarray(np.atleast_1d(n_topic), dtype=np.int32)
        K = len(n_topic)
        rank_out = _as(rank_out, "float64")
        if rank_out.numel() < K * self.n:
            raise ValueError("rank_out too small")
        iters = np.zeros(K, dtype=np.int32)
        check(self.ctx.lib.ss_pagerank_run(self.h, damping, eps, max_iter, K, _ptr(n_topic), _ptr(rank_out), _ptr(iters)),
              self.ctx.h)
        return iters

    def set_link_key(self, key) -> None:
        if key is None:
            check(self.ctx.lib.ss_graph_set_link_key(self.h, None), self.ctx.h)
            return
        key = _as(key, "float64")
        if (key.numel() if _is_torch(key) else key.size) < self.n:
            raise ValueError("key must hold n_nodes values")
        self.ctx.ready(key)
        check(self.ctx.lib.ss_graph_set_link_key(self.h, _ptr(key)), self.ctx.h)

    def _links_out(self, rows: int, m: int, want_degree: bool, out):
        count = lambda a: a.numel() if _is_torch(a) else a.size
        if out is not None:
            links, n_out, degree = _as(out[0], "uint32"), _as(out[1], "int32"), _as(out[2], "uint32") if len(out) > 2 else None
            if count(links) < rows * m or count(n_out) < rows or (degree is not None and count(degree) < rows):
                raise ValueError("output buffers too small")
            return links, n_out, degree
        return np.zeros(rows * m, dtype=np.uint32), np.zeros(rows, dtype=np.int32), np.zeros(rows, dtype=np.uint32) if want_degree else None

    def top_links(self, nodes, direction: int, m: int = 5, want_degree: bool = True, out=None):
        nodes = _as(nodes, "uint32")
        n = int(nodes.numel() if _is_torch(nodes) else nodes.size)
        links, n_out, degree = self._links_out(n, int(m), want_degree, out)
        self.ctx.ready(nodes, links, n_out, degree)
        check(self.ctx.lib.ss_graph_top_links(self.h, int(direction), n, _ptr(nodes), int(m), _ptr(links), _ptr(n_out), _ptr(degree)), self.ctx.h)
        if out is None:
            links = links.reshape(n, int(m))
        elif any(_is_torch(a) for a in (links, n_out, degree)) and not getattr(self.ctx, "_shared_stream", False):
            self.ctx.synchronize()
        return links, n_out, degree

    def hit_links(self, hits, n_hits, direction: int, m: int = 5, want_degree: bool = True, out=None, k: Optional[int] = None):
        n_hits = _as(n_hits, "int32")
        n_q = int(n_hits.numel() if _is_torch(n_hits) else n_hits.size)
        nbytes = lambda a: a.numel() * a.element_size() if _is_torch(a) else a.nbytes
        hits = hits.contiguous() if _is_torch(hits) else np.ascontiguousarray(hits, dtype=HIT_DTYPE)
        if k is None:
            if n_q > 0 and nbytes(hits) % (n_q * HIT_DTYPE.itemsize):
                raise ValueError("hits does not hold n_q rows of whole ss_hit")
            k = nbytes(hits) // (n_q * HIT_DTYPE.itemsize) if n_q > 0 else 1
        elif nbytes(hits) < n_q * int(k) * HIT_DTYPE.itemsize:
            raise ValueError("hits too small")
        k = int(k)
        links, n_out, degree = self._links_out(n_q * k, int(m), want_degree, out)
        self.ctx.ready(hits, n_hits, links, n_out, degree)
        check(self.ctx.lib.ss_graph_hit_links(self.h, int(direction), n_q, k, _ptr(hits), _ptr(n_hits), int(m), _ptr(links), _ptr(n_out),
                                              _ptr(degree)), self.ctx.h)
        if out is None:
            links, n_out = links.reshape(n_q, k, int(m)), n_out.reshape(n_q, k)
            degree = degree.reshape(n_q, k) if degree is not None else None
        elif any(_is_torch(a) for a in (links, n_out, degree)) and not getattr(self.ctx, "_shared_stream", False):
            self.ctx.synchronize()
        return links, n_out, degree

    def close(self) -> None:
        if self.h:
            self.ctx.lib.ss_graph_destroy(self.h)
            self.h = None


class PageRankState:

    def __init__(self, graph: Graph, damping: float, eps: float, n_topic: Sequence[int], max_iter: int = 0):
        self.g = graph
        self.ctx = graph.ctx
        n_topic = np.ascontiguousarray(np.atleast_1d(n_topic), dtype=np.int32)
        self.k = len(n_topic)
        h = C.c_void_p()
        check(self.ctx.lib.ss_pr_create(graph.h, damping, eps, max_iter, self.k, _ptr(n_topic), C.byref(h)), self.ctx.h)
        self.h = h

    def set_teleport(self, sets) -> None:
        if sets is None:
            check(self.ctx.lib.ss_pr_set_teleport(self.h, None, None), self.ctx.h)
            return
        if len(sets) != self.k:
            raise ValueError("one teleport set per topic")
        ptr = np.zeros(self.k + 1, dtype=np.uint64)
        ptr[1:] = np.cumsum([len(x) for x in sets])
        nodes = np.ascontiguousarray(np.concatenate([np.asarray(x, dtype=np.uint32) for x in sets]) if int(ptr[-1]) else np.zeros(0, np.uint32))
        check(self.ctx.lib.ss_pr_set_teleport(self.h, _ptr(ptr), _ptr(nodes)), self.ctx.h)

    def begin(self) -> None:
        check(self.ctx.lib.ss_pr_begin(self.h), self.ctx.h)

    def step(self, n_steps: int = 1) -> None:
        check(self.ctx.lib.ss_pr_step(self.h, n_steps), self.ctx.h)

    def finalize(self) -> None:
        check(self.ctx.lib.ss_pr_finalize(self.h), self.ctx.h)

    def exchange(self, allreduce: bool = False) -> None:
        check(self.ctx.lib.ss_pr_exchange(self.h, 1 if allreduce else 0), self.ctx.h)

    def exchange_buffers(self):
        sp, rp = C.c_void_p(), C.c_void_p()
        sb, rb = C.c_uint64(), C.c_uint64()
        check(self.ctx.lib.ss_pr_exchange_buffers(self.h, C.byref(sp), C.byref(sb), C.byref(rp), C.byref(rb)), self.ctx.h)
        return sp.value, sb.value, rp.value, rb.value

    def status(self):
        iters = np.zeros(self.k, dtype=np.int32)
        delta = np.zeros(self.k, dtype=np.float64)
        total = np.zeros(self.k, dtype=np.float64)
        na, sw = C.c_int32(), C.c_int32()
        check(self.ctx.lib.ss_pr_status(self.h, _ptr(iters), C.byref(na), C.byref(sw), _ptr(delta), _ptr(total)), self.ctx.h)
        return {"iters": iters, "n_active": na.value, "sweeps": sw.value, "delta": delta, "total": total}

    def probe(self, mode: int = 0, n_reps: int = 5) -> float:
        ms = C.c_float(0)
        check(self.ctx.lib.ss_pr_probe(self.h, mode, n_reps, C.byref(ms)), self.ctx.h)
        return float(ms.value)

    def read(self) -> np.ndarray:
        out = np.zeros((self.k, self.g.n), dtype=np.float64)
        check(self.ctx.lib.ss_pr_read(self.h, _ptr(out)), self.ctx.h)
        return out

    def read_local(self):
        n_rows = int(self.g.info().n_rows_local)
        ids = np.zeros(n_rows, dtype=np.uint32)
        out = np.zeros((self.k, n_rows), dtype=np.float64)
        check(self.ctx.lib.ss_pr_read_local(self.h, _ptr(ids), _ptr(out)), self.ctx.h)
        return ids, out

    def close(self) -> None:
        if self.h:
            self.ctx.lib.ss_pr_destroy(self.h)
            self.h = None


class InvertedIndex:

    def __init__(self, ctx: Context, n_docs: int, term_ptr, post_doc, post_tf):
        self.ctx = ctx
        self.n_docs = int(n_docs)
        term_ptr = _as(term_ptr, "uint64")
        post_doc = _as(post_doc, "uint32")
        post_tf = _as(post_tf, "float32")
        self.n_terms = int(term_ptr.shape[0]) - 1
        self.n_post = int(post_doc.shape[0])
        ctx.ready(term_ptr, post_doc, post_tf)
        h = C.c_void_p()
        check(ctx.lib.ss_index_create(ctx.h, self.n_docs, self.n_terms, _ptr(term_ptr), _ptr(post_doc), _ptr(post_tf),
                                      C.byref(h)), ctx.h)
        self.h = h

    def tfidf_build(self, total_docs: int, want_w: bool = True, want_mag: bool = True, want_idf: bool = True):
        w = np.zeros(self.n_post, dtype=np.float32) if want_w else None
        mag = np.zeros(self.n_docs, dtype=np.float64) if want_mag else None
        idf = np.zeros(self.n_terms, dtype=np.float32) if want_idf else None
        check(self.ctx.lib.ss_tfidf_build(self.h, int(total_docs), _ptr(w), _ptr(mag), _ptr(idf)), self.ctx.h)
        return w, mag, idf

    def apply_delta(self, del_docs=None, del_pairs=None, add=None, add_pos=None) -> None:
        dd = _as(del_docs if del_docs is not None else np.zeros(0, np.uint32), "uint32")
        dt, dp = (_as(del_pairs[0], "uint32"), _as(del_pairs[1], "uint32")) if del_pairs is not None else (np.zeros(0, np.uint32),) * 2
        at, ad, aw = (_as(add[0], "uint32"), _as(add[1], "uint32"), _as(add[2], "float32")) if add is not None else \
            (np.zeros(0, np.uint32), np.zeros(0, np.uint32), np.zeros(0, np.float32))
        pp, pv = (_as(add_pos[0], "uint64"), _as(add_pos[1], "float32")) if add_pos is not None else (None, None)
        self.ctx.ready(dd, dt, dp, at, ad, aw, pp, pv)
        check(self.ctx.lib.ss_index_apply_delta_pos(self.h, int(dd.shape[0]), _ptr(dd), int(dt.shape[0]), _ptr(dt), _ptr(dp),
                                                    int(at.shape[0]), _ptr(at), _ptr(ad), _ptr(aw), _ptr(pp), _ptr(pv)), self.ctx.h)
        n_post = C.c_uint64()
        check(self.ctx.lib.ss_index_get_info(self.h, None, None, C.byref(n_post)), self.ctx.h)
        self.n_post = int(n_post.value)

    def resize(self, n_docs: int, n_terms: int) -> None:
        check(self.ctx.lib.ss_index_resize(self.h, int(n_docs), int(n_terms)), self.ctx.h)
        self.n_docs, self.n_terms = int(n_docs), int(n_terms)

    def read_magnitudes(self, docs) -> np.ndarray:
        docs = _as(docs, "uint32")
        out = np.zeros(int(docs.shape[0]), dtype=np.float64)
        check(self.ctx.lib.ss_index_read_magnitudes(self.h, int(docs.shape[0]), _ptr(docs), _ptr(out)), self.ctx.h)
        return out

    def read_positions(self):
        pp = np.zeros(self.n_post + 1, dtype=np.uint64)
        check(self.ctx.lib.ss_index_read_positions(self.h, _ptr(pp), None), self.ctx.h)
        pv = np.zeros(int(pp[-1]), dtype=np.float32)
        check(self.ctx.lib.ss_index_read_positions(self.h, None, _ptr(pv)), self.ctx.h)
        return pp, pv

    def refresh_magnitudes(self) -> np.ndarray:
        mag = np.zeros(self.n_docs, dtype=np.float64)
        check(self.ctx.lib.ss_index_refresh_magnitudes(self.h, _ptr(mag)), self.ctx.h)
        return mag

    def read(self):
        tp = np.zeros(self.n_terms + 1, dtype=np.uint64)
        pd = np.zeros(self.n_post, dtype=np.uint32)
        pw = np.zeros(self.n_post, dtype=np.float32)
        check(self.ctx.lib.ss_index_read(self.h, _ptr(tp), _ptr(pd), _ptr(pw)), self.ctx.h)
        return tp, pd, pw

    def build_doc_view(self) -> None:
        check(self.ctx.lib.ss_index_build_doc_view(self.h), self.ctx.h)

    def drop_doc_view(self) -> None:
        check(self.ctx.lib.ss_index_drop_doc_view(self.h), self.ctx.h)

    def read_doc_view(self):
        dp = np.zeros(self.n_docs + 1, dtype=np.uint64)
        check(self.ctx.lib.ss_index_read_doc_view(self.h, _ptr(dp), None, None), self.ctx.h)
        dt = np.zeros(int(dp[-1]), dtype=np.uint32)
        dw = np.zeros(int(dp[-1]), dtype=np.float32)
        check(self.ctx.lib.ss_index_read_doc_view(self.h, None, _ptr(dt), _ptr(dw)), self.ctx.h)
        return dp, dt, dw

    def doc_top_terms(self, docs, m: int, want_w: bool = True, out=None):
        docs = _as(docs, "uint32")
        n = int(docs.shape[0])
        if out is not None:
            terms, w, n_out = _as(out[0], "uint32"), _as(out[1], "float32"), _as(out[2], "int32")
            count = lambda a: a.numel() if _is_torch(a) else a.size
            if count(terms) < n * m or (w is not None and count(w) < n * m) or count(n_out) < n:
                raise ValueError("output buffers too small")
        else:
            terms = np.zeros((n, m), dtype=np.uint32)
            w = np.zeros((n, m), dtype=np.float32) if want_w else None
            n_out = np.zeros(n, dtype=np.int32)
        self.ctx.ready(docs, terms, w, n_out)
        check(self.ctx.lib.ss_index_doc_top_terms(self.h, n, _ptr(docs), int(m), _ptr(terms), _ptr(w), _ptr(n_out)), self.ctx.h)
        return terms, w, n_out

    def build_signatures(self, n_slots: int = 16) -> None:
        check(self.ctx.lib.ss_index_build_signatures(self.h, int(n_slots)), self.ctx.h)

    def drop_signatures(self) -> None:
        check(self.ctx.lib.ss_index_drop_signatures(self.h), self.ctx.h)

    def read_signatures(self, docs, out=None):
        docs = _as(docs, "uint32")
        n = int(docs.numel() if _is_torch(docs) else docs.size)
        n_slots = C.c_int32(0)
        check(self.ctx.lib.ss_index_read_signatures(self.h, 0, None, None, C.byref(n_slots)), self.ctx.h)
        if out is None:
            out = np.zeros((n, n_slots.value), dtype=np.uint32)
        else:
            out = _as(out, "uint32")
            if (out.numel() if _is_torch(out) else out.size) < n * n_slots.value:
                raise ValueError("output buffer too small")
        self.ctx.ready(docs, out)
        check(self.ctx.lib.ss_index_read_signatures(self.h, n, _ptr(docs), _ptr(out), None), self.ctx.h)
        return out

    def set_doc_freq(self, df) -> None:
        df = _as(df, "uint64")
        if df is not None and int(df.shape[0]) != self.n_terms:
            raise ValueError("df must hold one entry per term")
        self.ctx.ready(df)
        check(self.ctx.lib.ss_index_set_doc_freq(self.h, _ptr(df)), self.ctx.h)

    def set_positions(self, pos_ptr, pos) -> None:
        pos_ptr = _as(pos_ptr, "uint64")
        pos = _as(pos, "float32")
        self.ctx.ready(pos_ptr, pos)
        check(self.ctx.lib.ss_index_set_positions(self.h, _ptr(pos_ptr), _ptr(pos)), self.ctx.h)

    def set_weighted(self, mag) -> None:
        mag = _as(mag, "float64")
        self.ctx.ready(mag)
        check(self.ctx.lib.ss_index_set_weighted(self.h, _ptr(mag)), self.ctx.h)

    def close(self) -> None:
        if self.h:
            check(self.ctx.lib.ss_index_destroy(self.h), self.ctx.h)
            self.h = None


def pack_doc_masks(sets, n_docs: int) -> np.ndarray:
    n_words = (int(n_docs) + 31) // 32
    if isinstance(sets, np.ndarray) and sets.dtype == np.bool_:
        if sets.ndim != 2 or sets.shape[1] != n_docs:
            raise ValueError(f"bool masks must have shape [n_masks][{n_docs}], got {sets.shape}")
        bits = np.zeros((sets.shape[0], n_words * 32), dtype=np.bool_)
        bits[:, :n_docs] = sets
    else:
        bits = np.zeros((len(sets), n_words * 32), dtype=np.bool_)
        for i, docs in enumerate(sets):
            docs = np.asarray(docs, dtype=np.int64).ravel()
            if docs.size and (docs.min() < 0 or docs.max() >= n_docs):
                raise ValueError(f"mask {i}: doc id outside 0 .. {n_docs - 1}")
            bits[i, docs] = True
    return np.packbits(bits, axis=1, bitorder="little").view("<u4").reshape(bits.shape[0], n_words).astype(np.uint32)


def pack_doc_ranges(sets):
    ptr = np.zeros(len(sets) + 1, dtype=np.uint32)
    ptr[1:] = np.cumsum([len(c) for c in sets])
    rng = np.zeros(int(ptr[-1]), dtype=DOC_RANGE_DTYPE)
    flat = [c for cs in sets for c in cs]
    rng["field"] = [c[0] for c in flat]
    rng["lo"] = [c[1] for c in flat]
    rng["hi"] = [c[2] for c in flat]
    return ptr, rng


class Scorer:

    def __init__(self, ctx: Context, title: InvertedIndex, body: InvertedIndex):
        self.ctx = ctx
        self.title, self.body = title, body
        h = C.c_void_p()
        check(ctx.lib.ss_scorer_create(ctx.h, title.h, body.h, C.byref(h)), ctx.h)
        self.h = h
        self.k_topics = 0
        self.n_fields = 0
        self.vec_dim = 0
        self.n_vec_lists = 0

    def set_prior(self, rank) -> None:
        if rank is None:
            check(self.ctx.lib.ss_scorer_set_prior(self.h, 0, None), self.ctx.h)
            self.k_topics = 0
            return
        rank = _as(rank, "float64")
        self.k_topics = int(rank.shape[0])
        self.ctx.ready(rank)
        check(self.ctx.lib.ss_scorer_set_prior(self.h, self.k_topics, _ptr(rank)), self.ctx.h)

    def set_doc_masks(self, masks) -> None:
        if masks is None or len(masks) == 0:
            check(self.ctx.lib.ss_scorer_set_doc_masks(self.h, 0, None), self.ctx.h)
            return
        masks = _as(masks, "uint32")
        self.ctx.ready(masks)
        check(self.ctx.lib.ss_scorer_set_doc_masks(self.h, int(masks.shape[0]), _ptr(masks)), self.ctx.h)

    def score_topk_masked(self, q_ptr, q_terms, mask_id, k: int, p_ptr=None, p_terms=None, query_len=None, topic_probs=None, out=None):
        q_ptr = _as(q_ptr, "uint32")
        q_terms = _as(q_terms, "uint32")
        mask_id = _as(mask_id, "int32")
        p_ptr = _as(p_ptr, "uint32")
        p_terms = _as(p_terms, "uint32")
        query_len = _as(query_len, "int32")
        topic_probs = _as(topic_probs, "float64")
        n_q = int(q_ptr.shape[0]) - 1
        self.ctx.ready(q_ptr, q_terms, mask_id, p_ptr, p_terms, query_len, topic_probs)
        if out is not None:
            hits, n_hits = out
            if hits.numel() * hits.element_size() < n_q * k * HIT_DTYPE.itemsize or n_hits.numel() < n_q:
                raise ValueError("output buffers too small")
        else:
            hits, n_hits = np.zeros((n_q, k), dtype=HIT_DTYPE), np.zeros(n_q, dtype=np.int32)
        check(self.ctx.lib.ss_score_topk_masked(self.h, n_q, _ptr(q_ptr), _ptr(q_terms), _ptr(p_ptr), _ptr(p_terms), _ptr(query_len),
                                                _ptr(topic_probs), _ptr(mask_id), k, _ptr(hits), _ptr(n_hits)), self.ctx.h)
        if out is not None and not getattr(self.ctx, "_shared_stream", False):
            self.ctx.synchronize()
        return hits, n_hits

    def score_topk_constrained(self, q_ptr, q_terms, k: int, req=None, exc=None, mask_id=None, p_ptr=None, p_terms=None,
                               query_len=None, topic_probs=None, out=None):
        q_ptr = _as(q_ptr, "uint32")
        q_terms = _as(q_terms, "uint32")
        req_ptr, req_terms = (None, None) if req is None else (_as(req[0], "uint32"), _as(req[1], "uint32"))
        exc_ptr, exc_terms = (None, None) if exc is None else (_as(exc[0], "uint32"), _as(exc[1], "uint32"))
        mask_id = _as(mask_id, "int32")
        p_ptr = _as(p_ptr, "uint32")
        p_terms = _as(p_terms, "uint32")
        query_len = _as(query_len, "int32")
        topic_probs = _as(topic_probs, "float64")
        n_q = int(q_ptr.shape[0]) - 1
        self.ctx.ready(q_ptr, q_terms, req_ptr, req_terms, exc_ptr, exc_terms, mask_id, p_ptr, p_terms, query_len, topic_probs)
        if out is not None:
            hits, n_hits = out
            if hits.numel() * hits.element_size() < n_q * k * HIT_DTYPE.itemsize or n_hits.numel() < n_q:
                raise ValueError("output buffers too small")
        else:
            hits, n_hits = np.zeros((n_q, k), dtype=HIT_DTYPE), np.zeros(n_q, dtype=np.int32)
        check(self.ctx.lib.ss_score_topk_constrained(self.h, n_q, _ptr(q_ptr), _ptr(q_terms), _ptr(p_ptr), _ptr(p_terms), _ptr(query_len),
                                                     _ptr(topic_probs), _ptr(mask_id), _ptr(req_ptr), _ptr(req_terms), _ptr(exc_ptr),
                                                     _ptr(exc_terms), k, _ptr(hits), _ptr(n_hits)), self.ctx.h)
        if out is not None and not getattr(self.ctx, "_shared_stream", False):
            self.ctx.synchronize()
        return hits, n_hits

    def score_topk_phrase(self, q_ptr, q_terms, p_ptr, p_terms, k: int, query_len=None, topic_probs=None):
        q_ptr = _as(q_ptr, "uint32")
        q_terms = _as(q_terms, "uint32")
        p_ptr = _as(p_ptr, "uint32")
        p_terms = _as(p_terms, "uint32")
        query_len = _as(query_len, "int32")
        topic_probs = _as(topic_probs, "float64")
        n_q = int(q_ptr.shape[0]) - 1
        self.ctx.ready(q_ptr, q_terms, p_ptr, p_terms, query_len, topic_probs)
        hits = np.zeros((n_q, k), dtype=HIT_DTYPE)
        n_hits = np.zeros(n_q, dtype=np.int32)
        check(self.ctx.lib.ss_score_topk_phrase(self.h, n_q, _ptr(q_ptr), _ptr(q_terms), _ptr(p_ptr), _ptr(p_terms),
# ... 664 lines not shown
```

Measured before the change: 18200.

## Add lean PageRank sweeps that skip x writes and deltas for fixed-iteration runs

When eps is negative (fixed iteration count), no teleport sets, single device and a non-affine sweep, all but the last two sweeps in a batch run a lean kernel variant. It skips loading and storing the rank vector x and the delta reduction, and only writes the contribution table. It also uses a filtered work list holding only rows with out-degree (row < sl_nd). This cuts memory traffic per sweep. The cost is extra planning work and device buffers at create time, plus extra template instantiations.

```diff
diff --git a/include/spaghetti_rank.h b/include/spaghetti_rank.h
--- a/include/spaghetti_rank.h
+++ b/include/spaghetti_rank.h
@@ -98,6 +98,7 @@
 int32_t ss_pr_set_teleport(ss_pr* pr, const uint64_t* set_ptr , const uint32_t* set_nodes);
 int32_t ss_pr_begin(ss_pr* pr);
 int32_t ss_pr_step(ss_pr* pr, int32_t n_steps);
+int32_t ss_pr_lean_sweeps(ss_pr* pr, int64_t* n_out);
 int32_t ss_pr_finalize(ss_pr* pr);
 int32_t ss_pr_exchange_buffers(ss_pr* pr, void** send_dev, uint64_t* send_bytes,
                                void** recv_dev, uint64_t* recv_bytes);
diff --git a/spaghettisearch_amd/_lib.py b/spaghettisearch_amd/_lib.py
--- a/spaghettisearch_amd/_lib.py
+++ b/spaghettisearch_amd/_lib.py
@@ -110,6 +110,7 @@
     "ss_pr_set_teleport": (_i32, [_vp, _vp, _vp]),
     "ss_pr_begin": (_i32, [_vp]),
     "ss_pr_step": (_i32, [_vp, _i32]),
+    "ss_pr_lean_sweeps": (_i32, [_vp, C.POINTER(C.c_int64)]),
     "ss_pr_finalize": (_i32, [_vp]),
     "ss_pr_exchange_buffers": (_i32, [_vp, C.POINTER(_vp), C.POINTER(_u64), C.POINTER(_vp), C.POINTER(_u64)]),
     "ss_pr_exchange": (_i32, [_vp, _i32]),
diff --git a/spaghettisearch_amd/csrc/ctx.hip b/spaghettisearch_amd/csrc/ctx.hip
--- a/spaghettisearch_amd/csrc/ctx.hip
+++ b/spaghettisearch_amd/csrc/ctx.hip
@@ -280,6 +280,7 @@
     "pr.stagger",
     "pr.deal_global",
     "pr.share_zero_rows",
+    "pr.lean_sweeps",
     "pr.item_turns",
     "graph.late_free",
     "graph.readback_runs",
diff --git a/spaghettisearch_amd/csrc/pagerank.hip b/spaghettisearch_amd/csrc/pagerank.hip
--- a/spaghettisearch_amd/csrc/pagerank.hip
+++ b/spaghettisearch_amd/csrc/pagerank.hip
@@ -272,10 +272,10 @@
 namespace ss {
 unsigned begin_blocks(const ss_pr* pr) { return std::max(1u, std::min(2048u, ss::div_up((size_t)pr->g->n_local() * pr->gw, TPB))); }
 void pr_launch_begin(ss_pr* pr, hipStream_t st, unsigned nb) { SS_GW_DISPATCH(pr->gw, launch_begin, pr, st, nb); }
-void pr_launch_step(ss_pr* pr, hipStream_t st) {
+void pr_launch_step(ss_pr* pr, hipStream_t st, bool lean) {
     switch (pr->kernel) {
         case PR_STEP: pr_step_launch(pr, st); break;
-        case PR_SWEEP: pr_sweep_launch(pr, st); break;
+        case PR_SWEEP: pr_sweep_launch(pr, st, lean); break;
         case PR_SWEEP_N: pr_sweep_n_launch(pr, st); break;
     }
 }
@@ -371,6 +371,7 @@
     p.stagger_code = opt.stagger >= 10 ? (uint32_t)(opt.stagger - 10) : 0u;
     p.class_order = pack_class_order(opt.class_order);
     p.n_order = pack_n_order(opt.n_class_order);
+    p.woff_lean = pr->lean ? pr->woff_lean.p : nullptr;
 }
 
 uint64_t fnv1a(const void* q, size_t n, uint64_t h = 0xcbf29ce484222325ull) {
@@ -510,6 +511,17 @@
         if (trace) fprintf(stderr, "[pr trace]   deal: placement %.3f ms\n", t_ms(td1, t_now()));
     }
     const std::vector<WorkItem>& items = cut.items;
+    pr->lean = pr->kernel == PR_SWEEP && g->world == 1 && ctx->opt("pr.affine", 0) == 0 && ctx->opt("pr.lean_sweeps", 1) != 0;
+    static const std::vector<WorkItem> no_items;
+    const std::vector<WorkItem>* lean_items = &no_items;
+    const std::vector<uint32_t>* lean_woff = &no_woff;
+    if (pr->lean) {
+        const auto tl0 = t_now();
+        const LeanPlan lp = plan_lean_items(items, *woff, pr->nblocks * WAVES, g->sl_nd, (uint32_t)items.size());
+        lean_items = &lp.items;
+        lean_woff = &lp.woff;
+        if (trace) fprintf(stderr, "[pr trace]   lean walk: %zu of %zu items, %.3f ms\n", lp.items.size() - 2, items.size() - 2, t_ms(tl0, t_now()));
+    }
 
     g->settle();
     const auto tc2 = t_now();
@@ -538,10 +550,16 @@
     SS_HIP(ctx, hipMemsetAsync(pr->rowticket.p, 0, pr->rowticket.bytes(), st));
     SS_HIP(ctx, pr->woff.alloc(std::max<size_t>(woff->size(), 8)));
     if (!woff->empty()) SS_HIP(ctx, hipMemcpyAsync(pr->woff.p, woff->data(), woff->size() * sizeof(uint32_t), hipMemcpyHostToDevice, st));
-    SS_HIP(ctx, pr->work.alloc(items.size()));
+    const size_t n_work = items.size() + lean_items->size();
+    SS_HIP(ctx, pr->work.alloc(n_work));
     SS_HIP(ctx, hipMemcpyAsync(pr->work.p, items.data(), items.size() * sizeof(WorkItem), hipMemcpyHostToDevice, st));
+    if (pr->lean) {
+        SS_HIP(ctx, hipMemcpyAsync(pr->work.p + items.size(), lean_items->data(), lean_items->size() * sizeof(WorkItem), hipMemcpyHostToDevice, st));
+        SS_HIP(ctx, pr->woff_lean.alloc(std::max<size_t>(lean_woff->size(), 8)));
+        SS_HIP(ctx, hipMemcpyAsync(pr->woff_lean.p, lean_woff->data(), lean_woff->size() * sizeof(uint32_t), hipMemcpyHostToDevice, st));
+    }
     if (vitems)
-        hipLaunchKernelGGL(k_pr_item_ranges, dim3(ss::div_up(items.size(), TPB)), dim3(TPB), 0, st, pr->work.p, (uint32_t)items.size(), (const uint32_t*)g->in_ptr.p);
+        hipLaunchKernelGGL(k_pr_item_ranges, dim3(ss::div_up(n_work, TPB)), dim3(TPB), 0, st, pr->work.p, (uint32_t)n_work, (const uint32_t*)g->in_ptr.p);
     SS_HIP(ctx, pr->ctl.alloc(1));
     SS_HIP(ctx, hipMemsetAsync(pr->ctl.p, 0, sizeof(PrCtl), st));
     double h_x0[MAXK];
@@ -672,6 +690,7 @@
     ss::pr_launch_begin(pr, ctx->stream, ss::begin_blocks(pr));
     SS_HIP(ctx, hipGetLastError());
     pr->begun = true;
+    pr->sweeps_enq = 0;
     if (pr->g->world > 1) {
         pr->need_finalize = true;
         pr->finalize_is_begin = true;
@@ -681,6 +700,19 @@
 
 int32_t ss_pr_step(ss_pr* pr, int32_t n_steps) {
     if (!pr) return SS_ERR_INVALID;
+    return ss::pr_step(pr, n_steps, 2);
+}
+
+int32_t ss_pr_lean_sweeps(ss_pr* pr, int64_t* n_out) {
+    if (!pr || !n_out) return SS_ERR_INVALID;
+    std::lock_guard<std::recursive_mutex> lk(pr->g->ctx->mu);
+    *n_out = pr->n_lean;
+    return SS_OK;
+}
+
+}
+
+int32_t ss::pr_step(ss_pr* pr, int32_t n_steps, int32_t full_tail) {
     ss_ctx* ctx = pr->g->ctx;
     std::lock_guard<std::recursive_mutex> lk(ctx->mu);
     SS_HIP(ctx, hipSetDevice(ctx->device));
@@ -692,8 +724,15 @@
     if (pr->persist && !pr->prm.memb && !pr->prm.aff) {
         ss::pr_multi_n_launch(pr, ctx->stream, (int)n_steps);
     } else {
-        for (int i = 0; i < n_steps; i++) ss::pr_launch_step(pr, ctx->stream);
-    }
+        const PrParams& p = pr->prm;
+        const bool lean_ok = pr->lean && p.eps < 0.0 && !p.memb && !p.aff;
+        for (int i = 0; i < n_steps; i++) {
+            const int64_t s = pr->sweeps_enq + 1 + i;
+            const bool lean = lean_ok && i + full_tail < n_steps && (p.max_iter <= 0 || s + 2 <= p.max_iter);
+            ss::pr_launch_step(pr, ctx->stream, lean);
+        }
+    }
+    pr->sweeps_enq += n_steps;
     SS_HIP(ctx, hipEventRecord(ctx->ev[0][1], ctx->stream));
     ctx->ev_valid[0] = true;
     SS_HIP(ctx, hipGetLastError());
@@ -703,6 +742,8 @@
     }
     return SS_OK;
 }
+
+extern "C" {
 
 int32_t ss_pr_finalize(ss_pr* pr) {
     if (!pr) return SS_ERR_INVALID;
diff --git a/spaghettisearch_amd/csrc/pagerank_run.hip b/spaghettisearch_amd/csrc/pagerank_run.hip
--- a/spaghettisearch_amd/csrc/pagerank_run.hip
+++ b/spaghettisearch_amd/csrc/pagerank_run.hip
@@ -692,7 +692,7 @@
         while (rc == SS_OK && n_active > 0) {
             int todo = BATCH;
             if (max_iter > 0) todo = std::min(BATCH, std::max(1, max_iter - sweeps));
-            rc = ss_pr_step(pr, todo);
+            rc = ss::pr_step(pr, todo, eps < 0.0 ? 0 : 2);
             if (rc == SS_OK) rc = ss_pr_status(pr, iters_out ? iters_out + k0 : nullptr, &n_active, &sweeps, nullptr, nullptr);
         }
         if (rc == SS_OK) rc = ss_pr_read(pr, rank_out + (size_t)k0 * g->n);
diff --git a/spaghettisearch_amd/csrc/pr_plan.hpp b/spaghettisearch_amd/csrc/pr_plan.hpp
--- a/spaghettisearch_amd/csrc/pr_plan.hpp
+++ b/spaghettisearch_amd/csrc/pr_plan.hpp
@@ -52,6 +52,8 @@
     std::vector<double> cost, load;
     std::vector<uint32_t> owner, by_load, idx, order, bucket, woff, cnt;
     std::vector<std::pair<double, uint32_t>> key;
+    std::vector<WorkItem> lean_items;
+    std::vector<uint32_t> lean_woff;
 };
 inline PlanScratch& plan_scratch() {
     static thread_local PlanScratch s;
@@ -301,6 +303,28 @@
     return woff;
 }
 
+struct LeanPlan {
+    const std::vector<WorkItem>& items;
+    const std::vector<uint32_t>& woff;
+};
+inline LeanPlan plan_lean_items(const std::vector<WorkItem>& dealt, const std::vector<uint32_t>& woff, uint32_t nw, uint32_t sl_nd, uint32_t base) {
+    PlanScratch& s = plan_scratch();
+    auto& items = s.lean_items;
+    auto& loff = s.lean_woff;
+    items.clear();
+    loff.assign((size_t)nw * 8, base);
+    const size_t n = dealt.size() >= 2 ? dealt.size() - 2 : 0;
+    for (size_t j = 0; j < (size_t)nw * 8 && j < woff.size(); j++) {
+        loff[j] = base + (uint32_t)items.size();
+        const size_t lo = std::min<size_t>(woff[j], n), hi = j + 1 < woff.size() ? std::min<size_t>(woff[j + 1], n) : n;
+        for (size_t i = lo; i < hi; i++)
+            if (dealt[i].row < sl_nd) items.push_back(dealt[i]);
+    }
+    items.push_back({V_ZERO, 0, 0, 0, 0, 0, 0, 0});
+    items.push_back({V_ZERO, 0, 0, 0, 0, 0, 0, 0});
+    return {items, loff};
+}
+
 inline uint32_t pack_class_order(int64_t code) {
     uint32_t packed = 0, seen = 0;
     for (int pos = 5; pos >= 0; pos--) {
diff --git a/spaghettisearch_amd/csrc/pr_state.hpp b/spaghettisearch_amd/csrc/pr_state.hpp
--- a/spaghettisearch_amd/csrc/pr_state.hpp
+++ b/spaghettisearch_amd/csrc/pr_state.hpp
@@ -76,6 +76,7 @@
     uint32_t n_shared;
     uint32_t share;
     uint32_t tab_rows;
+    const uint32_t* woff_lean;
 };
 
 }
@@ -105,6 +106,10 @@
     ss::DevBuf<uint32_t> woff;
     ss::DevBuf<uint32_t> src_shared;
     ss::DevBuf<uint32_t> sh_deg;
+    ss::DevBuf<uint32_t> woff_lean;
+    bool lean = false;
+    int64_t sweeps_enq = 0;
+    int64_t n_lean = 0;
     ss::DevBuf<PrCtl> ctl;
     bool begun = false;
     bool need_finalize = false;
@@ -115,9 +120,10 @@
 namespace ss {
 unsigned begin_blocks(const ss_pr* pr);
 void pr_launch_begin(ss_pr* pr, hipStream_t st, unsigned nb);
-void pr_launch_step(ss_pr* pr, hipStream_t st);
+void pr_launch_step(ss_pr* pr, hipStream_t st, bool lean = false);
+int32_t pr_step(ss_pr* pr, int32_t n_steps, int32_t full_tail);
 void pr_launch_finalize(ss_pr* pr, hipStream_t st, int is_begin);
-void pr_sweep_launch(ss_pr* pr, hipStream_t st);
+void pr_sweep_launch(ss_pr* pr, hipStream_t st, bool lean);
 int pr_sweep_occupancy(int gw);
 void pr_sweep_n_launch(ss_pr* pr, hipStream_t st);
 int pr_sweep_n_occupancy(int gw);
diff --git a/spaghettisearch_amd/csrc/pr_sweep.hip b/spaghettisearch_amd/csrc/pr_sweep.hip
--- a/spaghettisearch_amd/csrc/pr_sweep.hip
+++ b/spaghettisearch_amd/csrc/pr_sweep.hip
@@ -10,7 +10,7 @@
 }
 
 
-template <int GW, bool TS>
+template <int GW, bool TS, bool LEAN>
 struct SweepCtx {
     const PrParams& p;
     const double* __restrict__ T;
@@ -43,14 +43,22 @@
     }
 }
 
-template <int GW, bool TS>
-__device__ __forceinline__ void finish_row(SweepCtx<GW, TS>& c, uint32_t lrow, double y, double xo, uint32_t od, double* hub = nullptr) {
+template <int GW, bool TS, bool LEAN>
+__device__ __forceinline__ void finish_row(SweepCtx<GW, TS, LEAN>& c, uint32_t lrow, double y, double xo, uint32_t od, double* hub = nullptr) {
     const PrParams& p = c.p;
     y += c.x0;
     const size_t xi = (size_t)lrow * GW + c.t;
     double tele = p.teleport;
     if constexpr (TS) tele = teleport_of(p, lrow, c.t);
     double xn = (y + tele) / c.S;
+    if constexpr (LEAN) {
+        if (!c.act) xn = 0.0;
+        const double cc = p.d * xn / (double)od;
+        NT_STORE(cc, &c.Tw[xi]);
+        if (hub) __hip_atomic_store(&hub[GW + c.t], cc, __ATOMIC_RELAXED, __HIP_MEMORY_SCOPE_AGENT);
+        else c.csum += cc;
+        return;
+    }
     if (c.act) {
         NT_STORE(xn, &p.x[xi]);
         if (!hub) c.dsum += fabs(xn - xo);
@@ -69,8 +77,8 @@
     }
 }
 
-template <int GW, bool TS>
-__device__ __forceinline__ void long_rows(SweepCtx<GW, TS>& c, const WorkItem* __restrict__ work, uint32_t i0, uint32_t i1, int lane) {
+template <int GW, bool TS, bool LEAN>
+__device__ __forceinline__ void long_rows(SweepCtx<GW, TS, LEAN>& c, const WorkItem* __restrict__ work, uint32_t i0, uint32_t i1, int lane) {
     constexpr int NS = 64 / GW;
     constexpr uint32_t TW = NS * CH;
     const PrParams& p = c.p;
@@ -84,7 +92,8 @@
     for (uint32_t it = i0; it < i1; it++) {
         const WorkItem nn = work[it + 2];
         const uint32_t lrow = cur.row;
-        const double xo = NT_LOAD(&p.x[(size_t)lrow * GW + c.t]);
+        double xo = 0.0;
+        if constexpr (!LEAN) xo = NT_LOAD(&p.x[(size_t)lrow * GW + c.t]);
         const uint32_t od = lrow < p.sl_nd ? NT_LOAD(&p.outdeg[lrow]) : 1u;
         const uint32_t turns = (cur.end - cur.beg + TW - 1) / TW;
         const bool more = it + 1 < i1;
@@ -126,8 +135,8 @@
     }
 }
 
-template <int GW, bool TS>
-__device__ __forceinline__ void quad_rows(SweepCtx<GW, TS>& c, const WorkItem* __restrict__ work, uint32_t i0, uint32_t i1) {
+template <int GW, bool TS, bool LEAN>
+__device__ __forceinline__ void quad_rows(SweepCtx<GW, TS, LEAN>& c, const WorkItem* __restrict__ work, uint32_t i0, uint32_t i1) {
     constexpr int NS = 64 / GW;
     const PrParams& p = c.p;
     if (i0 >= i1) return;
@@ -174,7 +183,8 @@
         const uint32_t lrow = cur.row + q * NS + (uint32_t)c.slot;
         const bool valid = q * NS + (uint32_t)c.slot < cur.count;
         double xo = 0.0;
-        if (ends) xo = NT_LOAD(&p.x[(size_t)(valid ? lrow : cur.row) * GW + c.t]);
+        if constexpr (!LEAN)
+            if (ends) xo = NT_LOAD(&p.x[(size_t)(valid ? lrow : cur.row) * GW + c.t]);
         double v[CH];
         gather_turn<GW>(c.T, src, c.t, c.gbase, v);
 #pragma unroll
@@ -198,8 +208,8 @@
     }
 }
 
-template <int GW, int R, bool TS>
-__device__ __forceinline__ void deg_rows(SweepCtx<GW, TS>& c, const WorkItem* __restrict__ work, uint32_t i0, uint32_t i1) {
+template <int GW, int R, bool TS, bool LEAN>
+__device__ __forceinline__ void deg_rows(SweepCtx<GW, TS, LEAN>& c, const WorkItem* __restrict__ work, uint32_t i0, uint32_t i1) {
     constexpr int NS = 64 / GW;
     constexpr int DM = CH / R;
     constexpr int IR = CH / GW;
@@ -232,7 +242,10 @@
             const uint32_t rb = (i * NS + (uint32_t)c.slot) * R;
             double xo[R];
 #pragma unroll
-            for (int r = 0; r < R; r++) xo[r] = NT_LOAD(&p.x[(size_t)(row0 + (rb + r < count ? rb + r : 0u)) * GW + c.t]);
+            for (int r = 0; r < R; r++) {
+                xo[r] = 0.0;
+                if constexpr (!LEAN) xo[r] = NT_LOAD(&p.x[(size_t)(row0 + (rb + r < count ? rb + r : 0u)) * GW + c.t]);
+            }
             const uint32_t myr = row0 + (rb + (uint32_t)c.t < count ? rb + (uint32_t)c.t : 0u);
             const uint32_t odv = (c.t < R && myr < p.sl_nd) ? NT_LOAD(&p.outdeg[myr]) : 1u;
             double v[CH];
@@ -257,8 +270,9 @@
 #ifdef SS_PR_WAVETIME
 __device__ unsigned long long g_pr_wt[65536][2];
 #endif
-template <int GW, bool TS>
+template <int GW, bool TS, bool LEAN>
 __global__ __launch_bounds__(TPB, SS_PR_MINW) void k_pr_sweep(PrParams p) {
+    static_assert(!(TS && LEAN), "the lean sweep exists without teleport sets only");
     constexpr int NS = 64 / GW;
     PrCtl* ctl = p.ctl;
     if (ctl->n_active == 0) return;
@@ -269,7 +283,7 @@
     const int sweep = ctl->sweep;
     const int lane = threadIdx.x & 63;
     const uint32_t wave = (uint32_t)__builtin_amdgcn_readfirstlane((int)(threadIdx.x >> 6));
-    SweepCtx<GW, TS> c{p, p.tab_rd[sweep & 1], p.tab_wr[sweep & 1], 0.0, 0.0, false, lane % GW, lane - lane % GW, lane / GW, 0.0, 0.0};
+    SweepCtx<GW, TS, LEAN> c{p, p.tab_rd[sweep & 1], p.tab_wr[sweep & 1], 0.0, 0.0, false, lane % GW, lane - lane % GW, lane / GW, 0.0, 0.0};
     c.S = ctl->S[c.t];
     c.act = ctl->active[c.t] != 0;
     c.x0 = sweep == 0 ? p.x0[c.t] : 0.0;
@@ -283,7 +297,7 @@
         }
     }
 
-    const uint32_t* __restrict__ off = p.woff + (size_t)(blockIdx.x * WAVES + wave) * 8;
+    const uint32_t* __restrict__ off = (LEAN ? p.woff_lean : p.woff) + (size_t)(blockIdx.x * WAVES + wave) * 8;
     int rot = p.stagger_div ? (int)((blockIdx.x / p.stagger_div) % 6u) : 0;
     if (p.stagger_code) {
         uint32_t cdv = p.stagger_code;
@@ -341,7 +355,7 @@
         if (lane == 0) { g_pr_wt[wid][0] = wt0; g_pr_wt[wid][1] = wt1; }
     }
 #endif
-    block_reduce_and_publish<GW>(p, c.dsum, c.csum, c.Tw, false);
+    block_reduce_and_publish<GW>(p, LEAN ? 0.0 : c.dsum, c.csum, c.Tw, false);
 }
 
 template __device__ void begin_caller_context<8, 16>(const PrParams&, double*);
@@ -349,20 +363,24 @@
 }
 
 namespace ss {
-void pr_sweep_launch(ss_pr* pr, hipStream_t st) {
+void pr_sweep_launch(ss_pr* pr, hipStream_t st, bool lean) {
     const bool ts = pr->prm.memb != nullptr;
+    lean = lean && !ts && pr->prm.woff_lean;
+    if (lean) pr->n_lean++;
     if (pr->gw == 8) {
-        if (ts) hipLaunchKernelGGL((k_pr_sweep<8, true>), dim3(pr->nblocks), dim3(TPB), 0, st, pr->prm);
-        else hipLaunchKernelGGL((k_pr_sweep<8, false>), dim3(pr->nblocks), dim3(TPB), 0, st, pr->prm);
+        if (ts) hipLaunchKernelGGL((k_pr_sweep<8, true, false>), dim3(pr->nblocks), dim3(TPB), 0, st, pr->prm);
+        else if (lean) hipLaunchKernelGGL((k_pr_sweep<8, false, true>), dim3(pr->nblocks), dim3(TPB), 0, st, pr->prm);
+        else hipLaunchKernelGGL((k_pr_sweep<8, false, false>), dim3(pr->nblocks), dim3(TPB), 0, st, pr->prm);
     } else {
-        if (ts) hipLaunchKernelGGL((k_pr_sweep<16, true>), dim3(pr->nblocks), dim3(TPB), 0, st, pr->prm);
-        else hipLaunchKernelGGL((k_pr_sweep<16, false>), dim3(pr->nblocks), dim3(TPB), 0, st, pr->prm);
+        if (ts) hipLaunchKernelGGL((k_pr_sweep<16, true, false>), dim3(pr->nblocks), dim3(TPB), 0, st, pr->prm);
+        else if (lean) hipLaunchKernelGGL((k_pr_sweep<16, false, true>), dim3(pr->nblocks), dim3(TPB), 0, st, pr->prm);
+        else hipLaunchKernelGGL((k_pr_sweep<16, false, false>), dim3(pr->nblocks), dim3(TPB), 0, st, pr->prm);
     }
 }
 int pr_sweep_occupancy(int gw) {
     int per_cu = 8;
-    if (gw == 8) (void)hipOccupancyMaxActiveBlocksPerMultiprocessor(&per_cu, k_pr_sweep<8, false>, TPB, 0);
-    else (void)hipOccupancyMaxActiveBlocksPerMultiprocessor(&per_cu, k_pr_sweep<16, false>, TPB, 0);
+    if (gw == 8) (void)hipOccupancyMaxActiveBlocksPerMultiprocessor(&per_cu, k_pr_sweep<8, false, false>, TPB, 0);
+    else (void)hipOccupancyMaxActiveBlocksPerMultiprocessor(&per_cu, k_pr_sweep<16, false, false>, TPB, 0);
     return per_cu;
 }
 
diff --git a/spaghettisearch_amd/engine.py b/spaghettisearch_amd/engine.py
--- a/spaghettisearch_amd/engine.py
+++ b/spaghettisearch_amd/engine.py
@@ -327,6 +327,11 @@
 
     def step(self, n_steps: int = 1) -> None:
         check(self.ctx.lib.ss_pr_step(self.h, n_steps), self.ctx.h)
+
+    def lean_sweeps(self) -> int:
+        n = C.c_int64(0)
+        check(self.ctx.lib.ss_pr_lean_sweeps(self.h, C.byref(n)), self.ctx.h)
+        return int(n.value)
 
     def finalize(self) -> None:
         check(self.ctx.lib.ss_pr_finalize(self.h), self.ctx.h)
```

Measured after the change: 21060 (median of 6 runs). 15.7% higher.
